# lyclyc52/SANeRF-HQ

Hardware: AMD Instinct MI355X
Metric: rays/s full render (800x800, hashgrid L=16 + 2x64 MLP) (higher is better)
Workload: dtype f32 arithmetic / f16 tables

## Files before the change

include/sanerf_hip.h:

```cpp
#ifndef SANERF_HIP_H
#define SANERF_HIP_H

#include <stddef.h>
#include <stdint.h>

#ifdef __cplusplus
extern "C" {
#endif

#define SN_MAX_LEVELS 32
#define SN_MAX_LAYERS 8
#define SN_MAX_STAGES 4
#define SN_ABI_VERSION 12

typedef void *sn_stream_t;

typedef enum {
    SN_OK = 0,
    SN_ERR_INVALID = -1,
    SN_ERR_UNSUPPORTED = -2,
    SN_ERR_HIP = -3,
    SN_ERR_WORKSPACE = -4,
    SN_ERR_WINDOW = -5
} sn_status;
// ... 111 lines not shown

int sn_rm_mask_eval_accumulate(const float *logits, const int64_t *labels, uint32_t N, uint32_t K, uint32_t C, float eps, sn_eval_record *record,
                               void *workspace, sn_stream_t stream);

int sn_rm_image_sqerr_accumulate(const float *pred, uint32_t pred_stride, const float *truth, uint32_t truth_stride, uint32_t N,
                                 sn_eval_record *record, void *workspace, sn_stream_t stream);

typedef struct sn_ssim_record {
    double ssim_sum;
    double last;
    uint64_t images;
} sn_ssim_record;

#define SN_SSIM_WORKSPACE_BYTES 8192

int sn_rm_image_ssim_accumulate(const float *pred, uint32_t pred_stride, const float *truth, uint32_t truth_stride, uint32_t H, uint32_t W,
                                float data_range , sn_ssim_record *record, void *workspace, sn_stream_t stream);

#define SN_DISTILL_WORKSPACE_FIXED_BYTES 8256
size_t sn_rm_feature_distill_workspace_bytes(uint32_t h, uint32_t w, uint32_t C, uint32_t Ho, uint32_t Wo);
int sn_rm_feature_distill_loss(const float *feat, uint32_t feat_stride, uint32_t h, uint32_t w, uint32_t C, const float *target, uint32_t Ho,
                               uint32_t Wo, float scale, const float *scale_dev, float *loss, float *grad_feat, float *resized, void *workspace,
                               size_t workspace_bytes, sn_stream_t stream);
int sn_rm_feature_map(const float *feat, uint32_t feat_stride, uint32_t h, uint32_t w, uint32_t C, uint32_t Ho, uint32_t Wo, float *out,
                      sn_stream_t stream);

typedef struct sn_rgb_loss_record { float total, mse, entropy, reserved; } sn_rgb_loss_record;
#define SN_RGB_LOSS_MAX_WORKGROUPS 512
#define SN_RGB_LOSS_WORKSPACE_BYTES 8256
int sn_rm_rgb_loss(const float *image, uint32_t image_stride, const float *weights_sum, const float *truth, uint32_t truth_stride,
                   uint32_t truth_channels, uint32_t N, float bg_value, const float *bg, uint32_t bg_rows, int image_has_bg,
                   float lambda_entropy, const float *extra0, float coef0, const float *extra1, float coef1, float *pred_rgb, float *gt_rgb,
                   sn_rgb_loss_record *record, float *grad_image, float *grad_weights_sum, void *workspace, sn_stream_t stream);

#define SN_PROMPT_MAX_POINTS 1024

int sn_rm_points_lift(const int32_t *pixels, uint32_t M, const float *rays_o, const float *rays_d, const float *depth, uint32_t depth_stride,
                      uint32_t H, uint32_t W, float *point_3d, sn_stream_t stream);

int sn_rm_point_store_update(float *xyz, int32_t *labels, int32_t *crucial, int32_t *count, uint32_t cap, const float *point, const int32_t *label,
                             float dist_thresh, int32_t *status, sn_stream_t stream);

int sn_rm_points_project(const float *points, const int32_t *labels, const int32_t *crucial, uint32_t N, const int32_t *n_points, const float *poses,
                         uint32_t V, const float *intrinsics, uint32_t n_intr, const float *depth, uint32_t depth_stride, uint32_t H, uint32_t W,
                         float depth_tol, int32_t crucial_count, int32_t valid_threshold, double resize_ratio ,
                         int32_t *coords, int32_t *labels_out, int32_t *kept_index, int32_t *sam_coords, int32_t *overlay_coords, float *cam,
                         float *uv, int32_t *state, int32_t *counts, sn_stream_t stream);

int sn_rm_prompt_overlay(const float *image, uint32_t image_stride, uint32_t H, uint32_t W, const uint8_t *masks, uint32_t M, const float *scores,
                         int32_t mask_index, const int32_t *coords, const int32_t *labels, uint32_t N, const int32_t *count, int32_t radius, double alpha,
                         float *rgb, uint8_t *rgb8, uint8_t *pred_mask, int32_t *selected, sn_stream_t stream);

#define SN_DRAW_MAX_CELLS 65536

int sn_rm_weighted_draw(const float *weights, const float *expo, uint32_t R, uint32_t C, uint32_t n, const float *row_u, const int64_t *row_index,
                        uint32_t M, int64_t *out, int32_t *status, sn_stream_t stream);

enum { SN_COLLATE_UNIFORM = 0, SN_COLLATE_ERROR_MAP = 1 };
typedef struct sn_collate_desc {
    const float   *poses, *intrinsics;
    const uint8_t *images;
    const void    *masks;
    const float   *error_map, *cam_near_far;
    uint32_t       M, n_intrinsics, H, W, image_channels, mask_channels, mask_elem_bytes, S, coarse_size;
    uint32_t       N;
    int32_t        mode, index;
    const int64_t *index_dev;
    const float   *u;
    const int64_t *cells;
    uint32_t       L, p;
    const float   *ul;
    const int64_t *centres;
    float         *rays_o, *rays_d;
    int64_t       *index_out, *i_out, *j_out, *inds_coarse;
    float         *images_out;
    void          *masks_out;
    float         *error_maps_out, *cam_near_far_out, *poses_out, *intrinsics_out;
    uint32_t       rays_o_stride, rays_d_stride, index_stride, i_stride, j_stride, inds_coarse_stride, images_stride, masks_stride,
                   error_maps_stride, cam_near_far_stride, poses_stride, intrinsics_stride;
} sn_collate_desc;
int sn_rm_collate_gather(const sn_collate_desc *desc, sn_stream_t stream);

int sn_rm_sample_positions(const float *rays_o, const float *rays_d, const float *nears, const float *fars, const float *bins,
                           uint32_t N, uint32_t T, int contract, float *real_bins, float *rays_t, float *xyzs, sn_stream_t stream);

int sn_rm_sample_positions_ex(const float *rays_o, const float *rays_d, const float *nears, const float *fars, const float *bins,
                              uint32_t N, uint32_t T, int contract, float grid_bound, float *real_bins, float *rays_t, float *xyzs,
                              sn_stream_t stream);

int sn_rm_jitter(const float *uniform, uint32_t N, uint32_t T, int kind, float *out, sn_stream_t stream);

int sn_rm_jitter_tables(uint64_t *state, uint32_t N, uint32_t ray_base, uint32_t num_stages, const uint32_t *num_steps, float *bins0,
                        float *const *u, int32_t advance, sn_stream_t stream);

int sn_rm_ray_composite(const float *weights, const float *rays_t, const float *raw, const float *rays_d, uint32_t N, uint32_t T,
                        float *weights_sum, float *depth, float *f_image, sn_stream_t stream);
int sn_rm_ray_composite_backward(const float *weights, const float *rays_t, const float *raw, const float *rays_d, const float *grad_weights_sum,
                                 const float *grad_depth, const float *grad_f_image, uint32_t N, uint32_t T, float *grad_weights, float *grad_raw,
                                 sn_stream_t stream);

int sn_rm_proposal_loss_scaled(const float *bins, const float *weights, const float *ref_bins, const float *ref_weights, uint32_t N, uint32_t T,
                               uint32_t Tr, float scale, const float *scale_dev, float *loss_per_ray, float *grad_weights, sn_stream_t stream);

size_t sn_rm_proposal_loss_workspace_bytes(uint32_t N, uint32_t T, uint32_t Tr, int backward);
int sn_rm_proposal_loss_long(const float *bins, const float *weights, const float *ref_bins, const float *ref_weights, uint32_t N, uint32_t T,
                             uint32_t Tr, float scale, const float *scale_dev, float *loss_per_ray, float *grad_weights, void *workspace,
                             size_t workspace_bytes, sn_stream_t stream);

int sn_zero(void *ptr, size_t bytes, sn_stream_t stream);

int sn_rm_composite(const float *weights, const float *values, uint32_t N, uint32_t T, uint32_t K,
                    float *out, sn_stream_t stream);
int sn_rm_composite_backward(const float *weights, const float *grad_out, uint32_t N, uint32_t T, uint32_t K,
                             float *grad_values, sn_stream_t stream);

typedef struct sn_grid_desc {
    const void *embeddings;
    int32_t     table_dtype;
    int32_t     offsets[SN_MAX_LEVELS + 1];
    uint32_t    D, C, L;
    float       S;
    uint32_t    H;
    uint32_t    gridtype, align_corners, interp;
} sn_grid_desc;

typedef struct sn_mlp_desc {
    const float *weight[SN_MAX_LAYERS];
    const float *bias[SN_MAX_LAYERS];
    uint32_t     dims[SN_MAX_LAYERS + 1];
    uint32_t     num_layers;
    uint32_t     activation;
    uint32_t     skip_mask;
} sn_mlp_desc;

enum { SN_MLP_AUTO = 0, SN_MLP_F16X3 = 1, SN_MLP_MFMA32 = 2, SN_MLP_VALU = 3, SN_MLP_F16X1 = 5 };
enum { SN_EXP_NONE = 0, SN_EXP_ROLE_SPLIT = 1, SN_EXP_LDS_LEVEL0 = 2, SN_EXP_FINAL_ONE_WG = 3,
       SN_EXP_MATRIX_CLUMPED = 4,
       SN_EXP_GATHER_CANONICAL = 5    };
typedef struct sn_render_tuning {
    int32_t mlp_mode;
    int32_t per_sample_form;
    int32_t densify;
    int32_t linear_tile_order;
    int32_t prop_sp_max_rays;
    int32_t final_sp_max_rays;
    int32_t feat_levels;
    int32_t band_streams;
    int32_t exact_early_out;
    int32_t wave_tile;
    int32_t prop_sp_lanes;
    int32_t feat_patch;
    int32_t prop_pair;
    int32_t experiment;
} sn_render_tuning;

typedef struct sn_render_cfg {
    uint32_t     num_stages;
    uint32_t     num_steps[SN_MAX_STAGES];
    sn_grid_desc prop_grid[SN_MAX_STAGES];
    sn_mlp_desc  prop_mlp[SN_MAX_STAGES];
    sn_grid_desc grid;
    sn_mlp_desc  grid_mlp;
    sn_mlp_desc  view_mlp;
    uint32_t     sh_degree;
    float        aabb[6];
    float        min_near;
    float        bound;
    int32_t      contract;
    int32_t      last_sample_opaque;
    float        bg_color;
    sn_grid_desc feat_grid;
    int32_t      with_feat;
    float        early_stop_eps;
    int32_t      mlp_exact_fp32;
    int32_t      compact_live;
    sn_render_tuning tuning;
} sn_render_cfg;

typedef struct sn_render_io {
    const float *rays_o, *rays_d;
    const float *cam_near_far;
    uint32_t     N;
    uint32_t     tile_w;
    const float *bins0_table;
    const float *u_table[SN_MAX_STAGES];
    uint32_t     bins0_ray_stride;
    uint32_t     u_ray_stride[SN_MAX_STAGES];
    int32_t      skip_final;
    float       *image;
    float       *depth;
    float       *weights_sum;
    uint32_t     out_stride;
    float       *bins[SN_MAX_STAGES];
    float       *weights[SN_MAX_STAGES];
    float       *sigmas[SN_MAX_STAGES];
    int32_t     *inds[SN_MAX_STAGES];
    float       *xyzs_last;
    float       *geo_feat_last;
    float       *f_image;
    float       *f_feat;
    uint32_t     head_stride;
    int32_t      pack_valid;
    void        *workspace;
    size_t       workspace_bytes;
} sn_render_io;

#define SN_PACK_VALID 0x50414b31

size_t sn_rm_render_workspace_bytes(const sn_render_cfg *cfg, uint32_t N, uint32_t tile_w);
int sn_rm_render_rays(const sn_render_cfg *cfg, const sn_render_io *io, sn_stream_t stream);
typedef struct sn_launch_info {
    char     final_kernel[64];
    uint32_t workgroups, lds_bytes, dense_levels, gathers_per_wave_sample, launches;
} sn_launch_info;
int sn_rm_last_launch_info(sn_launch_info *info);
int sn_rm_render_route_info(const sn_render_cfg *cfg, const sn_render_io *io, sn_launch_info *out);

typedef struct sn_tile_order_info {
    uint32_t workgroups, tile_id, tile_w, tile_h;
    int32_t  x[4], y[4];
} sn_tile_order_info;
int sn_rm_tile_order_info(uint32_t W, uint32_t rows, int32_t wave_tile, int32_t order, uint32_t workgroup, sn_tile_order_info *out);

int sn_rm_grid_composite(const float *xyzs, const float *weights, uint32_t N, uint32_t T, float bound,
                         const sn_grid_desc *grid, uint32_t tile_w, float *out, sn_stream_t stream);

size_t sn_mlp_wide_workspace_bytes(const sn_mlp_desc *mlp);
int sn_mlp_wide_overflow(int32_t *flag);
int sn_mlp_wide_forward(const sn_mlp_desc *mlp, const float *ln_weight, const float *ln_bias, float ln_eps,
                        const float *x, uint32_t N, float *out, void *workspace, size_t workspace_bytes,
                        sn_stream_t stream);

size_t sn_rm_mask_head_workspace_bytes(const sn_mlp_desc *mlp);
int sn_rm_mask_head(const float *xyzs, const float *extra, const float *weights, uint32_t N, uint32_t T, uint32_t E,
                    float bound, const sn_grid_desc *grid, const sn_mlp_desc *mlp, float *out,
                    void *workspace, size_t workspace_bytes, sn_stream_t stream);

int sn_rm_mask_point_labels(const float *xyzs, const float *extra, const float *live, uint32_t N, uint32_t T, uint32_t E,
                            float bound, const sn_grid_desc *grid, const sn_mlp_desc *mlp, uint8_t *labels, float *logits,
                            void *workspace, size_t workspace_bytes, sn_stream_t stream);
int sn_rm_object_composite(const uint8_t *labels, const float *sigmas, const float *real_bins, const float *geo_feat, const float *rays_d,
                           uint32_t N, uint32_t T, uint32_t keep_mask, int32_t invert, int32_t last_sample_opaque, float *weights_sum,
                           float *depth, float *f_image, float *weights, sn_stream_t stream);

int sn_rm_vertex_probe_points(const float *vertices, const float *normals, uint32_t V_total, uint32_t first, uint32_t count, uint32_t K,
                              float h, int32_t contract, float *xyz, float *dirs, sn_stream_t stream);
int sn_rm_vertex_probe_composite(const uint8_t *labels, const float *sigmas, const float *geo_feat, const float *dirs, uint32_t V, uint32_t K,
                                 float h, uint32_t keep_mask, int32_t invert, float *f, float *coverage, uint8_t *vertex_label,
                                 sn_stream_t stream);

int sn_rm_lattice_points(const float *origin, const float *step, uint32_t nx, uint32_t ny, uint32_t nz, uint32_t first, uint32_t count,
                         int32_t contract, float *xyz, sn_stream_t stream);
size_t sn_rm_isosurface_workspace_bytes(uint32_t nx, uint32_t ny, uint32_t nz);
int sn_rm_isosurface_count(const float *volume, uint32_t nx, uint32_t ny, uint32_t nz, float iso, void *workspace, size_t workspace_bytes,
                           uint32_t *counts, sn_stream_t stream);
int sn_rm_isosurface_emit(const float *volume, uint32_t nx, uint32_t ny, uint32_t nz, float iso, const float *origin, const float *step,
                          const void *workspace, size_t workspace_bytes, float *vertices, float *normals, int32_t *triangles,
                          uint32_t cap_v, uint32_t cap_t, sn_stream_t stream);

size_t sn_rm_mesh_clean_workspace_bytes(uint32_t V, uint32_t T);
int sn_rm_mesh_components_init(uint32_t V, int32_t *labels, sn_stream_t stream);
int sn_rm_mesh_components_sweep(const int32_t *triangles, uint32_t T, uint32_t V, int32_t *labels, uint32_t rounds, uint32_t *changed,
                                sn_stream_t stream);
int sn_rm_mesh_component_stats(const int32_t *triangles, uint32_t T, uint32_t V, const int32_t *labels, int32_t *triangle_counts,
                               int32_t *vertex_counts, uint32_t *counts, sn_stream_t stream);
int sn_rm_mesh_filter_count(const int32_t *triangles, uint32_t T, uint32_t V, const int32_t *labels, const int32_t *triangle_counts,
                            uint32_t min_triangles, const uint64_t *min_key, void *workspace, size_t workspace_bytes, uint32_t *counts,
                            sn_stream_t stream);
int sn_rm_mesh_filter_emit(const int32_t *triangles, uint32_t T, uint32_t V, const float *vertices, const float *normals,
                           const void *workspace, size_t workspace_bytes, float *out_vertices, float *out_normals, int32_t *out_triangles,
                           int32_t *source_vertex, uint32_t cap_v, uint32_t cap_t, sn_stream_t stream);

#define SN_MESH_SPLIT_PARTS 33
size_t sn_rm_mesh_split_workspace_bytes(uint32_t V, uint32_t T);
int sn_rm_mesh_split_count(const int32_t *triangles, uint32_t T, uint32_t V, const uint8_t *vertex_labels, void *workspace,
                           size_t workspace_bytes, int32_t *part_triangle_offsets, int32_t *part_vertex_offsets, uint32_t *counts,
                           sn_stream_t stream);
int sn_rm_mesh_split_emit(const int32_t *triangles, uint32_t T, uint32_t V, const float *vertices, const float *normals, void *workspace,
                          size_t workspace_bytes, float *out_vertices, float *out_normals, int32_t *out_triangles, int32_t *source_vertex,
                          int32_t *source_triangle, uint32_t cap_v, uint32_t cap_t, sn_stream_t stream);

size_t sn_rm_mesh_simplify_workspace_bytes(uint32_t V, uint32_t T, uint32_t cells);
int sn_rm_mesh_simplify_count(const float *vertices, const float *normals, const int32_t *triangles, uint32_t V, uint32_t T,
                              const float *origin, const float *cell, const uint32_t *dims, void *workspace, size_t workspace_bytes,
                              uint32_t *counts, sn_stream_t stream);
int sn_rm_mesh_simplify_emit(const float *vertices, const float *normals, const int32_t *triangles, uint32_t V, uint32_t T,
                             const float *origin, const float *cell, const uint32_t *dims, const void *workspace, size_t workspace_bytes,
                             float *out_vertices, float *out_normals, int32_t *out_triangles, int32_t *vertex_cluster, uint32_t cap_v,
                             uint32_t cap_t, sn_stream_t stream);

size_t sn_rm_mesh_smooth_workspace_bytes(uint32_t V, uint32_t T);
int sn_rm_mesh_smooth_build(const float *vertices, const int32_t *triangles, uint32_t V, uint32_t T, const float *origin, float quantum,
                            void *workspace, size_t workspace_bytes, sn_stream_t stream);
int sn_rm_mesh_smooth_steps(uint32_t V, uint32_t T, uint32_t iterations, float lambda, float mu, int pin_open, void *workspace,
                            size_t workspace_bytes, sn_stream_t stream);
int sn_rm_mesh_smooth_emit(const float *vertices, uint32_t V, uint32_t T, const float *origin, float quantum, const void *workspace,
                           size_t workspace_bytes, float *out_vertices, float *out_normals, uint8_t *vertex_flags, sn_stream_t stream);

size_t sn_rm_mesh_raster_workspace_bytes(uint32_t V, uint32_t T, uint32_t H, uint32_t W);
int sn_rm_mesh_raster_project(const float *vertices, uint32_t V, uint32_t T, const float *pose, const float *intrinsics, uint32_t H, uint32_t W,
                              float near_plane, void *workspace, size_t workspace_bytes, int32_t *counts, sn_stream_t stream);
int sn_rm_mesh_raster_draw(const int32_t *triangles, uint32_t V, uint32_t T, uint32_t H, uint32_t W, int cull, uint32_t small_max_pixels,
                           void *workspace, size_t workspace_bytes, int32_t *counts, sn_stream_t stream);
int sn_rm_mesh_raster_resolve(const int32_t *triangles, uint32_t V, uint32_t T, uint32_t H, uint32_t W, const float *colors,
                              const float *normals, const uint8_t *labels, float bg_color, const void *workspace, size_t workspace_bytes,
                              int32_t *triangle_id, float *depth, uint8_t *mask, float *image, float *normal, uint8_t *label,
                              sn_stream_t stream);
int sn_rm_mesh_raster_draw_clip(const float *vertices, const int32_t *triangles, uint32_t V, uint32_t T, const float *pose, const float *intrinsics,
                                uint32_t H, uint32_t W, float near_plane, int cull, uint32_t small_max_pixels, void *workspace,
                                size_t workspace_bytes, int32_t *counts, int32_t *clip_counts, sn_stream_t stream);
int sn_rm_mesh_raster_resolve_clip(const float *vertices, const int32_t *triangles, uint32_t V, uint32_t T, const float *pose,
                                   const float *intrinsics, uint32_t H, uint32_t W, float near_plane, const float *colors, const float *normals,
                                   const uint8_t *labels, float bg_color, const void *workspace, size_t workspace_bytes, int32_t *triangle_id,
                                   float *depth, uint8_t *mask, float *image, float *normal, uint8_t *label, sn_stream_t stream);

int sn_mlp_wide_forward_train(const sn_mlp_desc *mlp, const float *x, uint32_t N, float *const *hidden, float *out, sn_stream_t stream);

int sn_mlp_wide_forward_train_f16x3(const sn_mlp_desc *mlp, const float *x, uint32_t N, float *const *hidden, uint32_t *const *sign_bits,
                                    float *out, void *workspace, size_t workspace_bytes, sn_stream_t stream);

size_t sn_mlp_wide_backward_workspace_bytes(const sn_mlp_desc *mlp);
int sn_mlp_wide_backward_bits(const sn_mlp_desc *mlp, const float *grad_out, const uint32_t *const *sign_bits, uint32_t N,
                              float *grad_in, float *const *grad_hidden, void *workspace, size_t workspace_bytes, sn_stream_t stream);
int sn_mlp_wide_backward(const sn_mlp_desc *mlp, const float *grad_out, const float *const *hidden, uint32_t N,
                         float *grad_in, float *const *grad_hidden, void *workspace, size_t workspace_bytes, sn_stream_t stream);

enum { SN_SMALL_ACT_NONE = 0, SN_SMALL_ACT_TRUNC_EXP0 = 1, SN_SMALL_ACT_SIGMOID_BG = 2 };
int sn_mlp_small_supported(const sn_mlp_desc *mlp);
int sn_mlp_small_forward_train(const sn_mlp_desc *mlp, const float *x, uint32_t N, float *const *hidden, float *out, int32_t act,
                               const float *aux_in, float bg, float *aux_out, sn_stream_t stream);
int sn_mlp_small_backward(const sn_mlp_desc *mlp, const float *grad_out, const float *grad_aux, int32_t act, const float *out_raw, float bg,
                          const float *const *hidden, uint32_t N, float *grad_in, float *const *grad_hidden, float *grad_last, float *grad_aux_in,
                          sn_stream_t stream);

int sn_gemm_f32(const float *a, int64_t a_row, int64_t a_col, const float *b, int64_t b_row, int64_t b_col, const float *bias, int32_t act,
                uint32_t M, uint32_t N, uint32_t K, float *c, int64_t c_row, sn_stream_t stream);

size_t sn_linear_wgrad_workspace_bytes(uint32_t M, uint32_t K, uint32_t N);
int sn_linear_wgrad(const float *x, const float *dy, uint32_t M, uint32_t K, uint32_t N, float *dw,
                    void *workspace, size_t workspace_bytes, sn_stream_t stream);

#define SN_ADAM_ZERO_GRAD 1
#define SN_ADAM_LAZY 2
int sn_adam_step(float *param, float *grad, float *exp_avg, float *exp_avg_sq, uint64_t n, double lr, double beta1, double beta2,
                 double eps, double weight_decay, uint32_t step, const float *step_device, int maximize, int flags, sn_stream_t stream);

#define SN_ADAM_MULTI_MAX_TENSORS 32
#define SN_ADAM_MULTI_MAX_GROUPS 8
typedef struct sn_adam_tensor {
    float *param, *grad, *exp_avg, *exp_avg_sq;
    uint64_t n;
    float *step_device;
    uint32_t step;
    uint32_t group;
} sn_adam_tensor;
typedef struct sn_adam_group {
    double lr, beta1, beta2, eps, weight_decay;
    int32_t maximize;
    int32_t flags;
} sn_adam_group;
int sn_adam_step_multi(const sn_adam_tensor *tensors, uint32_t n_tensors, const sn_adam_group *groups, uint32_t n_groups,
                       const float *lr_scale_device, uint32_t *ticket, sn_stream_t stream);

#define SN_EMA_MULTI_MAX_TENSORS 32
#define SN_EMA_ADVANCE 1
typedef struct sn_ema_tensor {
    float *shadow;
    const float *param;
    uint64_t n;
// ... 15 lines not shown
```

sanerf-hq_amd/_lib.py:

```python
from __future__ import annotations

import ctypes as C
import os
import subprocess
from typing import Optional

import torch

_PKG = os.path.dirname(os.path.abspath(__file__))
LIB_PATH = os.environ.get("SN_LIB") or os.path.join(_PKG, "libsanerf_hip.so")
CSRC = os.path.join(_PKG, "csrc")

MAX_LEVELS, MAX_LAYERS, MAX_STAGES = 32, 8, 4
SN_F32, SN_F16 = 0, 1
LAYOUT_LBC, LAYOUT_BLC = 0, 1


class GridDesc(C.Structure):
    _fields_ = [("embeddings", C.c_void_p), ("table_dtype", C.c_int32), ("offsets", C.c_int32 * (MAX_LEVELS + 1)),
                ("D", C.c_uint32), ("C", C.c_uint32), ("L", C.c_uint32), ("S", C.c_float), ("H", C.c_uint32),
                ("gridtype", C.c_uint32), ("align_corners", C.c_uint32), ("interp", C.c_uint32)]


class MlpDesc(C.Structure):
    _fields_ = [("weight", C.c_void_p * MAX_LAYERS), ("bias", C.c_void_p * MAX_LAYERS),
                ("dims", C.c_uint32 * (MAX_LAYERS + 1)), ("num_layers", C.c_uint32),
                ("activation", C.c_uint32), ("skip_mask", C.c_uint32)]


MLP_AUTO, MLP_F16X3, MLP_MFMA32, MLP_VALU, MLP_F16X1 = 0, 1, 2, 3, 5
EXP_NONE, EXP_ROLE_SPLIT, EXP_LDS_LEVEL0, EXP_FINAL_ONE_WG, EXP_MATRIX_CLUMPED, EXP_GATHER_CANONICAL = 0, 1, 2, 3, 4, 5
BUILD_EXPERIMENTS, BUILD_POISON_LDS = 1, 2
ADAM_ZERO_GRAD, ADAM_LAZY = 1, 2
ADAM_MULTI_MAX_TENSORS, ADAM_MULTI_MAX_GROUPS = 32, 8
EMA_MULTI_MAX_TENSORS, EMA_ADVANCE = 32, 1
MASK_MAX_CLASSES, MASK_EVAL_WORKSPACE_BYTES = 32, 8192
MASK_OUT_MODES = {"none": 0, "heatmap": 1, "composition": 2, "mask": 3}
SSIM_WORKSPACE_BYTES, SSIM_MAX_STRIDE, SSIM_WINDOW = 8192, 64, 11
DISTILL_WORKSPACE_FIXED_BYTES = 8256
RGB_LOSS_WORKSPACE_BYTES, RGB_LOSS_MAX_WORKGROUPS = 8256, 512
PROMPT_MAX_POINTS = 1024
DRAW_MAX_CELLS = 65536
COLLATE_UNIFORM, COLLATE_ERROR_MAP = 0, 1


class AdamTensor(C.Structure):
    _fields_ = [("param", C.c_void_p), ("grad", C.c_void_p), ("exp_avg", C.c_void_p), ("exp_avg_sq", C.c_void_p), ("n", C.c_uint64),
                ("step_device", C.c_void_p), ("step", C.c_uint32), ("group", C.c_uint32)]


class AdamGroup(C.Structure):
    _fields_ = [("lr", C.c_double), ("beta1", C.c_double), ("beta2", C.c_double), ("eps", C.c_double), ("weight_decay", C.c_double),
                ("maximize", C.c_int32), ("flags", C.c_int32)]


class EmaTensor(C.Structure):
    _fields_ = [("shadow", C.c_void_p), ("param", C.c_void_p), ("n", C.c_uint64)]


class EvalRecord(C.Structure):
    _fields_ = [("nll_mean_sum", C.c_double), ("miou_sum", C.c_double), ("mse_sum", C.c_double), ("psnr_sum", C.c_double),
                ("images", C.c_uint64), ("rgb_images", C.c_uint64), ("inter", C.c_uint64 * MASK_MAX_CLASSES),
                ("pred", C.c_uint64 * MASK_MAX_CLASSES), ("truth", C.c_uint64 * MASK_MAX_CLASSES)]


class SsimRecord(C.Structure):
    _fields_ = [("ssim_sum", C.c_double), ("last", C.c_double), ("images", C.c_uint64)]


class CollateDesc(C.Structure):
    _fields_ = ([(n, C.c_void_p) for n in ("poses", "intrinsics", "images", "masks", "error_map", "cam_near_far")]
                + [(n, C.c_uint32) for n in ("M", "n_intrinsics", "H", "W", "image_channels", "mask_channels", "mask_elem_bytes", "S", "coarse_size", "N")]
                + [("mode", C.c_int32), ("index", C.c_int32), ("index_dev", C.c_void_p), ("u", C.c_void_p), ("cells", C.c_void_p),
                   ("L", C.c_uint32), ("p", C.c_uint32), ("ul", C.c_void_p), ("centres", C.c_void_p)]
                + [(n, C.c_void_p) for n in ("rays_o", "rays_d", "index_out", "i_out", "j_out", "inds_coarse", "images_out", "masks_out",
                                             "error_maps_out", "cam_near_far_out", "poses_out", "intrinsics_out")]
                + [(n + "_stride", C.c_uint32) for n in ("rays_o", "rays_d", "index", "i", "j", "inds_coarse", "images", "masks", "error_maps",
                                                         "cam_near_far", "poses", "intrinsics")])


class RenderTuning(C.Structure):
    _fields_ = [("mlp_mode", C.c_int32), ("per_sample_form", C.c_int32), ("densify", C.c_int32), ("linear_tile_order", C.c_int32),
                ("prop_sp_max_rays", C.c_int32), ("final_sp_max_rays", C.c_int32), ("feat_levels", C.c_int32), ("band_streams", C.c_int32), ("exact_early_out", C.c_int32), ("wave_tile", C.c_int32), ("prop_sp_lanes", C.c_int32), ("feat_patch", C.c_int32), ("prop_pair", C.c_int32), ("experiment", C.c_int32)]


class LaunchInfo(C.Structure):
    _fields_ = [("final_kernel", C.c_char * 64), ("workgroups", C.c_uint32), ("lds_bytes", C.c_uint32), ("dense_levels", C.c_uint32),
                ("gathers_per_wave_sample", C.c_uint32), ("launches", C.c_uint32)]


class TileOrderInfo(C.Structure):
    _fields_ = [("workgroups", C.c_uint32), ("tile_id", C.c_uint32), ("tile_w", C.c_uint32), ("tile_h", C.c_uint32),
                ("x", C.c_int32 * 4), ("y", C.c_int32 * 4)]


PACK_VALID = 0x50414B31


class RenderCfg(C.Structure):
    _fields_ = [("num_stages", C.c_uint32), ("num_steps", C.c_uint32 * MAX_STAGES),
                ("prop_grid", GridDesc * MAX_STAGES), ("prop_mlp", MlpDesc * MAX_STAGES),
                ("grid", GridDesc), ("grid_mlp", MlpDesc), ("view_mlp", MlpDesc),
                ("sh_degree", C.c_uint32), ("aabb", C.c_float * 6), ("min_near", C.c_float), ("bound", C.c_float),
                ("contract", C.c_int32), ("last_sample_opaque", C.c_int32), ("bg_color", C.c_float),
                ("feat_grid", GridDesc), ("with_feat", C.c_int32), ("early_stop_eps", C.c_float), ("mlp_exact_fp32", C.c_int32),
                ("compact_live", C.c_int32), ("tuning", RenderTuning)]


class RenderIO(C.Structure):
    _fields_ = [("rays_o", C.c_void_p), ("rays_d", C.c_void_p), ("cam_near_far", C.c_void_p),
                ("N", C.c_uint32), ("tile_w", C.c_uint32),
                ("bins0_table", C.c_void_p), ("u_table", C.c_void_p * MAX_STAGES),
                ("bins0_ray_stride", C.c_uint32), ("u_ray_stride", C.c_uint32 * MAX_STAGES), ("skip_final", C.c_int32),
                ("image", C.c_void_p), ("depth", C.c_void_p), ("weights_sum", C.c_void_p), ("out_stride", C.c_uint32),
                ("bins", C.c_void_p * MAX_STAGES), ("weights", C.c_void_p * MAX_STAGES),
                ("sigmas", C.c_void_p * MAX_STAGES), ("inds", C.c_void_p * MAX_STAGES),
                ("xyzs_last", C.c_void_p), ("geo_feat_last", C.c_void_p), ("f_image", C.c_void_p), ("f_feat", C.c_void_p), ("head_stride", C.c_uint32), ("pack_valid", C.c_int32),
                ("workspace", C.c_void_p), ("workspace_bytes", C.c_size_t)]


_u32, _f32, _i32, _vp, _int = C.c_uint32, C.c_float, C.c_int32, C.c_void_p, C.c_int
ABI_VERSION = 12

_SIGNATURES = {
    "sn_abi_version": (_int, []),
    "sn_build_flags": (_int, []),
    "sn_debug_set": (_int, [C.c_char_p, _int]),
    "sn_last_error": (C.c_char_p, []),
    "sn_device_count": (_int, []),
    "sn_grid_encode_forward": (_int, [_vp, _vp, _int, _vp, _vp, _u32, _u32, _u32, _u32, _u32, _f32, _u32, _vp, _u32, _int, _u32, _int, _vp]),
    "sn_grid_encode_forward_cat": (_int, [_vp, _vp, _int, _vp, _vp, _u32, _vp, _u32, _u32, _u32, _f32, _u32, _u32, _int, _u32, _vp]),
    "sn_grid_encode_backward": (_int, [_vp, _vp, _vp, _int, _vp, _vp, _u32, _u32, _u32, _u32, _u32, _f32, _u32, _vp, _vp, _u32, _int, _u32, _int, _vp]),
    "sn_grid_backward_binned_workspace_bytes": (C.c_size_t, [_u32, _u32, _u32, _u32, _u32, _vp]),
    "sn_grid_encode_backward_binned": (_int, [_vp, _vp, _vp, _vp, _u32, _u32, _u32, _u32, _u32, _f32, _u32, _u32, _int, _u32, _int, _vp, C.c_size_t, _vp]),
    "sn_grid_encode_backward_binned_rows": (_int, [_vp, _u32, _vp, _vp, _vp, _u32, _u32, _u32, _u32, _u32, _f32, _u32, _u32, _int, _u32, _int, _vp, C.c_size_t, _vp]),
    "sn_grad_total_variation": (_int, [_vp, _vp, _vp, _vp, _f32, _u32, _u32, _u32, _u32, _f32, _u32, _u32, _int, _vp]),
    "sn_grad_weight_decay": (_int, [_vp, _vp, _vp, _f32, _u32, _u32, _u32, _vp]),
    "sn_sh_encode_forward": (_int, [_vp, _vp, _u32, _u32, _u32, _vp, _vp]),
    "sn_sh_encode_backward": (_int, [_vp, _vp, _u32, _u32, _u32, _vp, _vp, _vp]),
    "sn_freq_encode_forward": (_int, [_vp, _u32, _u32, _u32, _u32, _vp, _vp]),
    "sn_freq_encode_backward": (_int, [_vp, _vp, _u32, _u32, _u32, _u32, _vp, _vp]),
    "sn_rm_generate_rays": (_int, [_vp, _f32, _f32, _f32, _f32, _u32, _u32, _u32, _u32, _vp, _vp, _vp]),
    "sn_rm_rays_from_pixels": (_int, [_vp, _u32, _vp, _u32, _vp, _u32, _u32, _vp, _vp, _vp]),
    "sn_rm_near_far_from_aabb": (_int, [_vp, _vp, _vp, _f32, _u32, _vp, _vp, _vp]),
    "sn_rm_contract": (_int, [_vp, _u32, _vp, _vp]),
    "sn_rm_sample_pdf": (_int, [_vp, _vp, _u32, _u32, _u32, _vp, _u32, _vp, _vp, _vp]),
    "sn_rm_weights_from_sigma": (_int, [_vp, _vp, _u32, _u32, _int, _vp, _vp]),
    "sn_rm_weights_from_sigma_backward": (_int, [_vp, _vp, _vp, _u32, _u32, _int, _vp, _vp]),
    "sn_rm_distort_loss": (_int, [_vp, _vp, _u32, _u32, _vp, _vp, _vp]),
    "sn_rm_proposal_loss": (_int, [_vp, _vp, _vp, _vp, _u32, _u32, _u32, _vp, _vp, _vp]),
    "sn_rm_sample_positions": (_int, [_vp, _vp, _vp, _vp, _vp, _u32, _u32, _int, _vp, _vp, _vp, _vp]),
    "sn_rm_sample_positions_ex": (_int, [_vp, _vp, _vp, _vp, _vp, _u32, _u32, _int, _f32, _vp, _vp, _vp, _vp]),
    "sn_rm_jitter": (_int, [_vp, _u32, _u32, _int, _vp, _vp]),
    "sn_rm_jitter_tables": (_int, [_vp, _u32, _u32, _u32, C.POINTER(_u32), _vp, C.POINTER(_vp), _i32, _vp]),
    "sn_rm_ray_composite": (_int, [_vp, _vp, _vp, _vp, _u32, _u32, _vp, _vp, _vp, _vp]),
    "sn_rm_ray_composite_backward": (_int, [_vp, _vp, _vp, _vp, _vp, _vp, _vp, _u32, _u32, _vp, _vp, _vp]),
    "sn_rm_proposal_loss_scaled": (_int, [_vp, _vp, _vp, _vp, _u32, _u32, _u32, _f32, _vp, _vp, _vp, _vp]),
    "sn_gemm_f32": (_int, [_vp, C.c_int64, C.c_int64, _vp, C.c_int64, C.c_int64, _vp, C.c_int32, _u32, _u32, _u32, _vp, C.c_int64, _vp]),
    "sn_rm_proposal_loss_workspace_bytes": (C.c_size_t, [_u32, _u32, _u32, _int]),
    "sn_rm_proposal_loss_long": (_int, [_vp, _vp, _vp, _vp, _u32, _u32, _u32, _f32, _vp, _vp, _vp, _vp, C.c_size_t, _vp]),
    "sn_zero": (_int, [_vp, C.c_size_t, _vp]),
    "sn_mlp_small_supported": (_int, [C.POINTER(MlpDesc)]),
    "sn_mlp_small_forward_train": (_int, [C.POINTER(MlpDesc), _vp, _u32, _vp, _vp, _i32, _vp, _f32, _vp, _vp]),
    "sn_mlp_small_backward": (_int, [C.POINTER(MlpDesc), _vp, _vp, _i32, _vp, _f32, _vp, _u32, _vp, _vp, _vp, _vp, _vp]),
    "sn_rm_composite": (_int, [_vp, _vp, _u32, _u32, _u32, _vp, _vp]),
    "sn_rm_composite_backward": (_int, [_vp, _vp, _u32, _u32, _u32, _vp, _vp]),
    "sn_rm_grid_composite": (_int, [_vp, _vp, _u32, _u32, _f32, C.POINTER(GridDesc), _u32, _vp, _vp]),
    "sn_mlp_wide_workspace_bytes": (C.c_size_t, [C.POINTER(MlpDesc)]),
    "sn_mlp_wide_forward": (_int, [C.POINTER(MlpDesc), _vp, _vp, _f32, _vp, _u32, _vp, _vp, C.c_size_t, _vp]),
    "sn_mlp_wide_overflow": (_int, [_vp]),
    "sn_mlp_wide_forward_train": (_int, [C.POINTER(MlpDesc), _vp, _u32, _vp, _vp, _vp]),
    "sn_mlp_wide_forward_train_f16x3": (_int, [C.POINTER(MlpDesc), _vp, _u32, _vp, _vp, _vp, _vp, C.c_size_t, _vp]),
    "sn_mlp_wide_backward_bits": (_int, [C.POINTER(MlpDesc), _vp, _vp, _u32, _vp, _vp, _vp, C.c_size_t, _vp]),
    "sn_mlp_wide_backward_workspace_bytes": (C.c_size_t, [C.POINTER(MlpDesc)]),
    "sn_mlp_wide_backward": (_int, [C.POINTER(MlpDesc), _vp, _vp, _u32, _vp, _vp, _vp, C.c_size_t, _vp]),
    "sn_rm_mask_head_workspace_bytes": (C.c_size_t, [C.POINTER(MlpDesc)]),
    "sn_rm_mask_head": (_int, [_vp, _vp, _vp, _u32, _u32, _u32, _f32, C.POINTER(GridDesc), C.POINTER(MlpDesc), _vp, _vp, C.c_size_t, _vp]),
    "sn_rm_mask_point_labels": (_int, [_vp, _vp, _vp, _u32, _u32, _u32, _f32, C.POINTER(GridDesc), C.POINTER(MlpDesc), _vp, _vp, _vp, C.c_size_t, _vp]),
    "sn_rm_object_composite": (_int, [_vp, _vp, _vp, _vp, _vp, _u32, _u32, _u32, _i32, _i32, _vp, _vp, _vp, _vp, _vp]),
    "sn_rm_vertex_probe_points": (_int, [_vp, _vp, _u32, _u32, _u32, _u32, _f32, _i32, _vp, _vp, _vp]),
    "sn_rm_vertex_probe_composite": (_int, [_vp, _vp, _vp, _vp, _u32, _u32, _f32, _u32, _i32, _vp, _vp, _vp, _vp]),
    "sn_rm_lattice_points": (_int, [C.POINTER(_f32), C.POINTER(_f32), _u32, _u32, _u32, _u32, _u32, _i32, _vp, _vp]),
    "sn_rm_isosurface_workspace_bytes": (C.c_size_t, [_u32, _u32, _u32]),
    "sn_rm_isosurface_count": (_int, [_vp, _u32, _u32, _u32, _f32, _vp, C.c_size_t, _vp, _vp]),
    "sn_rm_isosurface_emit": (_int, [_vp, _u32, _u32, _u32, _f32, C.POINTER(_f32), C.POINTER(_f32), _vp, C.c_size_t, _vp, _vp, _vp, _u32, _u32, _vp]),
    "sn_rm_mesh_clean_workspace_bytes": (C.c_size_t, [_u32, _u32]),
    "sn_rm_mesh_components_init": (_int, [_u32, _vp, _vp]),
    "sn_rm_mesh_components_sweep": (_int, [_vp, _u32, _u32, _vp, _u32, _vp, _vp]),
    "sn_rm_mesh_component_stats": (_int, [_vp, _u32, _u32, _vp, _vp, _vp, _vp, _vp]),
    "sn_rm_mesh_filter_count": (_int, [_vp, _u32, _u32, _vp, _vp, _u32, _vp, _vp, C.c_size_t, _vp, _vp]),
    "sn_rm_mesh_filter_emit": (_int, [_vp, _u32, _u32, _vp, _vp, _vp, C.c_size_t, _vp, _vp, _vp, _vp, _u32, _u32, _vp]),
    "sn_rm_mesh_split_workspace_bytes": (C.c_size_t, [_u32, _u32]),
    "sn_rm_mesh_split_count": (_int, [_vp, _u32, _u32, _vp, _vp, C.c_size_t, _vp, _vp, _vp, _vp]),
    "sn_rm_mesh_split_emit": (_int, [_vp, _u32, _u32, _vp, _vp, _vp, C.c_size_t, _vp, _vp, _vp, _vp, _vp, _u32, _u32, _vp]),
    "sn_rm_mesh_simplify_workspace_bytes": (C.c_size_t, [_u32, _u32, _u32]),
    "sn_rm_mesh_simplify_count": (_int, [_vp, _vp, _vp, _u32, _u32, _vp, _vp, _vp, _vp, C.c_size_t, _vp, _vp]),
    "sn_rm_mesh_simplify_emit": (_int, [_vp, _vp, _vp, _u32, _u32, _vp, _vp, _vp, _vp, C.c_size_t, _vp, _vp, _vp, _vp, _u32, _u32, _vp]),
    "sn_rm_mesh_smooth_workspace_bytes": (C.c_size_t, [_u32, _u32]),
    "sn_rm_mesh_smooth_build": (_int, [_vp, _vp, _u32, _u32, C.POINTER(_f32), _f32, _vp, C.c_size_t, _vp]),
    "sn_rm_mesh_smooth_steps": (_int, [_u32, _u32, _u32, _f32, _f32, _i32, _vp, C.c_size_t, _vp]),
    "sn_rm_mesh_smooth_emit": (_int, [_vp, _u32, _u32, C.POINTER(_f32), _f32, _vp, C.c_size_t, _vp, _vp, _vp, _vp]),
    "sn_rm_mesh_raster_workspace_bytes": (C.c_size_t, [_u32, _u32, _u32, _u32]),
    "sn_rm_mesh_raster_project": (_int, [_vp, _u32, _u32, _vp, _vp, _u32, _u32, _f32, _vp, C.c_size_t, _vp, _vp]),
    "sn_rm_mesh_raster_draw": (_int, [_vp, _u32, _u32, _u32, _u32, _i32, _u32, _vp, C.c_size_t, _vp, _vp]),
    "sn_rm_mesh_raster_resolve": (_int, [_vp, _u32, _u32, _u32, _u32, _vp, _vp, _vp, _f32, _vp, C.c_size_t, _vp, _vp, _vp, _vp, _vp, _vp, _vp]),
    "sn_rm_mesh_raster_draw_clip": (_int, [_vp, _vp, _u32, _u32, _vp, _vp, _u32, _u32, _f32, _i32, _u32, _vp, C.c_size_t, _vp, _vp, _vp]),
    "sn_rm_mesh_raster_resolve_clip": (_int, [_vp, _vp, _u32, _u32, _vp, _vp, _u32, _u32, _f32, _vp, _vp, _vp, _f32, _vp, C.c_size_t, _vp, _vp, _vp,
                                              _vp, _vp, _vp, _vp]),
    "sn_adam_step": (_int, [_vp, _vp, _vp, _vp, C.c_uint64, C.c_double, C.c_double, C.c_double, C.c_double, C.c_double, _u32, _vp, _int, _int, _vp]),
    "sn_adam_step_multi": (_int, [C.POINTER(AdamTensor), _u32, C.POINTER(AdamGroup), _u32, _vp, _vp, _vp]),
    "sn_ema_update_multi": (_int, [C.POINTER(EmaTensor), _u32, C.c_double, _vp, _vp, _int, _vp]),
    "sn_linear_wgrad_workspace_bytes": (C.c_size_t, [_u32, _u32, _u32]),
    "sn_linear_wgrad": (_int, [_vp, _vp, _u32, _u32, _u32, _vp, _vp, C.c_size_t, _vp]),
    "sn_rm_render_workspace_bytes": (C.c_size_t, [C.POINTER(RenderCfg), _u32, _u32]),
    "sn_rm_render_rays": (_int, [C.POINTER(RenderCfg), C.POINTER(RenderIO), _vp]),
    "sn_rm_profile_enable": (None, [_int]),
    "sn_rm_profile_read": (_int, [_vp, _vp, _int]),
    "sn_rm_profile_shader_clock": (_int, [_vp, _vp]),
    "sn_rm_mask_nll": (_int, [_vp, _vp, _u32, _u32, _f32, _vp, _vp, _vp]),
    "sn_rm_ray_pair_select": (_int, [_vp, _vp, _u32, _u32, _u32, _vp, _vp]),
    "sn_rm_ray_pair_rgb_loss": (_int, [_vp, _vp, _int, _vp, _u32, _u32, _u32, _u32, _f32, _f32, _f32, _int, _f32, _vp, _vp, _vp, _vp, _vp]),
    "sn_rm_mask_error": (_int, [_vp, _int, _vp, _u32, _u32, _f32, _f32, _vp, _vp]),
    "sn_rm_error_map_update": (_int, [_vp, _int, _vp, _vp, _u32, _vp, _u32, _u32, _f32, _f32, _u32, _u32, _vp, _vp, _vp, _vp]),
    "sn_rm_mask_output": (_int, [_vp, _u32, _u32, _vp, _u32, _vp, _u32, _int, _int, _f32, _vp, _vp, _vp, _vp, _vp, _vp, _vp]),
    "sn_rm_mask_eval_accumulate": (_int, [_vp, _vp, _u32, _u32, _u32, _f32, _vp, _vp, _vp]),
    "sn_rm_image_sqerr_accumulate": (_int, [_vp, _u32, _vp, _u32, _u32, _vp, _vp, _vp]),
    "sn_rm_image_ssim_accumulate": (_int, [_vp, _u32, _vp, _u32, _u32, _u32, _f32, _vp, _vp, _vp]),
    "sn_rm_feature_distill_workspace_bytes": (C.c_size_t, [_u32, _u32, _u32, _u32, _u32]),
    "sn_rm_feature_distill_loss": (_int, [_vp, _u32, _u32, _u32, _u32, _vp, _u32, _u32, _f32, _vp, _vp, _vp, _vp, _vp, C.c_size_t, _vp]),
    "sn_rm_feature_map": (_int, [_vp, _u32, _u32, _u32, _u32, _u32, _u32, _vp, _vp]),
    "sn_rm_rgb_loss": (_int, [_vp, _u32, _vp, _vp, _u32, _u32, _u32, _f32, _vp, _u32, _int, _f32, _vp, _f32, _vp, _f32, _vp, _vp, _vp, _vp, _vp, _vp, _vp]),
    "sn_rm_points_lift": (_int, [_vp, _u32, _vp, _vp, _vp, _u32, _u32, _u32, _vp, _vp]),
    "sn_rm_point_store_update": (_int, [_vp, _vp, _vp, _vp, _u32, _vp, _vp, _f32, _vp, _vp]),
    "sn_rm_points_project": (_int, [_vp, _vp, _vp, _u32, _vp, _vp, _u32, _vp, _u32, _vp, _u32, _u32, _u32, _f32, _i32, _i32, C.c_double,
                                    _vp, _vp, _vp, _vp, _vp, _vp, _vp, _vp, _vp, _vp]),
    "sn_rm_prompt_overlay": (_int, [_vp, _u32, _u32, _u32, _vp, _u32, _vp, _i32, _vp, _vp, _u32, _vp, _i32, C.c_double, _vp, _vp, _vp, _vp, _vp]),
    "sn_rm_weighted_draw": (_int, [_vp, _vp, _u32, _u32, _u32, _vp, _vp, _u32, _vp, _vp, _vp]),
    "sn_rm_collate_gather": (_int, [C.POINTER(CollateDesc), _vp]),
    "sn_rm_debug_occupancy": (_int, [_vp, _vp, _int]),
    "sn_rm_last_launch_info": (_int, [_vp]),
    "sn_rm_render_route_info": (_int, [C.POINTER(RenderCfg), C.POINTER(RenderIO), _vp]),
    "sn_rm_tile_order_info": (_int, [_u32, _u32, _i32, _i32, _u32, C.POINTER(TileOrderInfo)]),
    "sn_debug_eval": (_int, [_int, _vp, _vp, _u32, _vp, _vp]),
}

EXPORTED_SYMBOLS = tuple(_SIGNATURES)

_lib = None


def build(force: bool = False) -> str:
    srcs = [os.path.join(CSRC, f) for f in os.listdir(CSRC) if f.endswith((".hip", ".h", ".inc"))]
    srcs.append(os.path.join(os.path.dirname(_PKG), "include", "sanerf_hip.h"))
    stale = force or not os.path.exists(LIB_PATH) or os.path.getmtime(LIB_PATH) < max(os.path.getmtime(s) for s in srcs)
    if stale:
        subprocess.check_call(["make", "-C", CSRC, "-j4"] + (["-B"] if force else []))
    return LIB_PATH


def lib():
    global _lib
    if _lib is None:
        if not os.path.exists(LIB_PATH):
            raise ImportError(
                f"{LIB_PATH} is missing: build it with `python -c 'import __graft_entry__ as g; g.build()'` "
                "(hipcc --offload-arch=gfx950). There is no CPU / eager fallback for these operators.")
        l = C.CDLL(LIB_PATH)
        for name, (res, args) in _SIGNATURES.items():
            try:
                fn = getattr(l, name)
            except AttributeError:
                if os.environ.get("SN_LIB"):
                    continue
                raise ImportError(f"{LIB_PATH} does not export {name}: rebuild it")
            fn.restype, fn.argtypes = res, args
        if l.sn_abi_version() != ABI_VERSION:
            raise ImportError(f"{LIB_PATH} has ABI version {l.sn_abi_version()}, this package expects {ABI_VERSION}: rebuild it")
        _lib = l
    return _lib


def check(rc: int, what: str = "") -> None:
    if rc != 0:
        msg = lib().sn_last_error().decode()
        raise RuntimeError(f"{what}: {msg}" if what else msg)


def stream() -> int:
    return torch.cuda.current_stream().cuda_stream


def dev(t: Optional[torch.Tensor], name: str, dtype=torch.float32):
    if t is None:
        return None
    if not t.is_cuda:
        raise RuntimeError(f"{name} must be a CUDA tensor")
    if not t.is_contiguous():
        raise RuntimeError(f"{name} must be a contiguous tensor")
    if dtype is not None and t.dtype != dtype:
        raise RuntimeError(f"{name} must be a {dtype} tensor, got {t.dtype}")
    return t.data_ptr()


def host_i32(values):
    arr = (C.c_int32 * len(values))(*[int(v) for v in values])
    return arr


def host_f32(values):
    return (C.c_float * len(values))(*[float(v) for v in values])
```

sanerf-hq_amd/csrc/render.hip:

```cpp
#include "sn_common.h"
#include "sh_basis.inc"

#include <float.h>
#include <stdlib.h>
#include <string.h>
#include <cstdio>
#include <map>
#include <mutex>
#include <type_traits>
#include <vector>

namespace sn {

typedef float floatx16 __attribute__((ext_vector_type(16)));

struct RayCommon {
    const float *rays_o, *rays_d, *cnf;
    uint32_t N;
    uint32_t W;
    uint32_t rows;
    uint32_t Npad;
    float aabb[6];
    float min_near, bound;
    int contract, last_opaque;
    float bg;
    int xcd_swizzle;
    uint32_t st_w, st_h;
    uint32_t tlw;
    float inv_den;
};

__host__ __device__ __forceinline__ uint32_t xcd_tile_id(uint32_t b, uint32_t nwg) {
    const uint32_t xcd = b & 7u, q = nwg >> 3, r = nwg & 7u;
    return (xcd < r ? xcd * (q + 1u) : r * (q + 1u) + (xcd - r) * q) + (b >> 3);
}
__device__ __forceinline__ uint32_t tile_id_x(const RayCommon &rc, uint32_t b, uint32_t nwg) { return rc.xcd_swizzle ? xcd_tile_id(b, nwg) : b; }
__device__ __forceinline__ uint32_t tile_id(const RayCommon &rc) { return tile_id_x(rc, blockIdx.x, gridDim.x); }

__host__ __device__ __forceinline__ void wave_tile_of(uint32_t g, uint32_t tx8, uint32_t ty8, uint32_t sw, uint32_t sh, uint32_t &wx, uint32_t &wy) {
    const uint32_t P = ty8 >> 1, pair = 2u * tx8, paired = P * pair;
    if (g >= paired) { wx = g - paired; wy = ty8 & ~1u; return; }
    if (sw == 0u) { const uint32_t p = g / pair, i = g - p * pair; wx = i >> 1; wy = 2u * p + (i & 1u); return; }
    const uint32_t u = g >> 1;
    const uint32_t nsy = (P + sh - 1u) / sh, base = P / nsy, extra = P - base * nsy;
    const uint32_t big = (base + 1u) * tx8;
    uint32_t sy, r0, h, y0;
    if (u < extra * big) { sy = u / big; r0 = u - sy * big; h = base + 1u; y0 = sy * h; }
    else { const uint32_t v = u - extra * big, row = base * tx8, s = v / row; r0 = v - s * row; sy = extra + s; h = base; y0 = extra * (base + 1u) + s * base; }
    const uint32_t full = sw * h, sx = r0 / full, r1 = r0 - sx * full;
    const uint32_t left = tx8 - sx * sw, w = left < sw ? left : sw;
    const uint32_t ry = r1 / w, rx = r1 - ry * w;
    const uint32_t x = sx * sw + rx;
    wx = (sy & 1u) ? tx8 - 1u - x : x;
    wy = 2u * (y0 + ry) + (g & 1u);
}

__device__ __forceinline__ bool ray_of_lane(const RayCommon &rc, uint32_t wg, uint32_t &n) {
    const uint32_t tid = threadIdx.x;
    if (rc.W) {
        const uint32_t tlw = rc.tlw, tlh = 6u - tlw, tw = 1u << tlw, th = 1u << tlh;
        const uint32_t tx8 = (rc.W + tw - 1u) >> tlw, ty8 = (rc.rows + th - 1u) >> tlh;
        const uint32_t wave = __builtin_amdgcn_readfirstlane(tid >> 6), lane = tid & 63u;
        const uint32_t g = wg * 4u + wave;
        uint32_t wx, wy;
        wave_tile_of(g, tx8, ty8, rc.st_w, rc.st_h, wx, wy);
        const uint32_t py = (wy << tlh) + (lane >> tlw);
        const uint32_t px = (wx << tlw) + (lane & (tw - 1u));
        const bool ok = wx < tx8 && px < rc.W && py < rc.rows;
        n = ok ? py * rc.W + px : 0u;
        return ok;
    }
    n = wg * 256u + tid;
    const bool ok = n < rc.N;
    if (!ok) n = 0;
    return ok;
}

struct RaySetup {
    float o[3], d[3];
    float s_near, s_far;
};

__device__ __forceinline__ void setup_ray(const RayCommon &rc, uint32_t n, RaySetup &rs) {
#pragma unroll
    for (int k = 0; k < 3; ++k) { rs.o[k] = rc.rays_o[(size_t)n * 3 + k]; rs.d[k] = rc.rays_d[(size_t)n * 3 + k]; }
    float near, far;
    near_far_one(rs.o, rs.d, rc.aabb, rc.min_near, near, far);
    if (rc.cnf) {
        const float cn = rc.cnf[(size_t)n * 2], cf = rc.cnf[(size_t)n * 2 + 1];
        near = cn > near ? cn : near;
        far = cf < far ? cf : far;
    }
    rs.s_near = spacing_fn(near);
    rs.s_far = spacing_fn(far);
}

__device__ __forceinline__ float real_bin(const RaySetup &rs, float b) {
    const float a = rs.s_near * (1.0f - b);
    const float c = rs.s_far * b;
    return spacing_inv(a + c);
}

__device__ __forceinline__ void sample_x01(const RayCommon &rc, const RaySetup &rs, float tmid, float (&p)[3], float (&x01)[3]) {
#pragma unroll
    for (int k = 0; k < 3; ++k) { const float m = rs.d[k] * tmid; p[k] = rs.o[k] + m; }
    if (rc.contract) contract3(p[0], p[1], p[2]);
    const float den = 2.0f * rc.bound;
    if (rc.inv_den != 0.0f) {
#pragma unroll
        for (int k = 0; k < 3; ++k) x01[k] = (p[k] + rc.bound) * rc.inv_den;
    } else {
#pragma unroll
        for (int k = 0; k < 3; ++k) x01[k] = (p[k] + rc.bound) / den;
    }
}

template <int I, int N, typename F>
__device__ __forceinline__ void static_for(F &&f) {
    if constexpr (I < N) {
        f(std::integral_constant<int, I>{});
        static_for<I + 1, N>(f);
    }
}

template <typename T, int C>
struct Corner { float v[C]; };

template <typename T, int C>
__device__ __forceinline__ void corner_set_half2(Corner<T, C> &c, uint32_t bits) {
    static_assert(C == 2 && sizeof(T) == 2, "packed rows: fp16 tables with two features per level");
    c.v[0] = __uint_as_float(bits); c.v[1] = 0.0f;
}
__device__ __forceinline__ float fma_mix_lo(float w, uint32_t packed, float acc) {
    float d;
    asm("v_fma_mix_f32 %0, %1, %2, %3 op_sel_hi:[0,1,0]" : "=v"(d) : "v"(w), "v"(packed), "v"(acc));
    return d;
}
__device__ __forceinline__ float fma_mix_hi(float w, uint32_t packed, float acc) {
    float d;
    asm("v_fma_mix_f32 %0, %1, %2, %3 op_sel:[0,1,0] op_sel_hi:[0,1,0]" : "=v"(d) : "v"(w), "v"(packed), "v"(acc));
    return d;
}

#ifndef SN_PROP_GROUP
#define SN_PROP_GROUP 2
#endif
#ifndef SN_PROP_GROUP_H
#define SN_PROP_GROUP_H 2
#endif
template <typename T, int KIND, int l>
constexpr bool xswap_level() {
    return KIND == 1 && l >= 0;
}
#ifndef SN_XSWAP_MODE
#define SN_XSWAP_MODE 0
#endif
#ifndef SN_PARITY_FIRST
#define SN_PARITY_FIRST 12
#endif
#ifndef SN_PARITY_AXES
#define SN_PARITY_AXES 2
#endif
template <typename T, int AXIS, int l>
constexpr bool parity_level() {
    return l >= SN_PARITY_FIRST && (AXIS == 2 || (AXIS == 1 && SN_PARITY_AXES == 2));
}
__device__ __forceinline__ float parity_tag(float frac, uint32_t cell) {
    return __uint_as_float(__float_as_uint(frac) | (cell << 31));
}
__device__ __forceinline__ bool parity_of(float tagged) { return (__float_as_uint(tagged) >> 31) != 0u; }
#ifndef SN_PARITY_UNDO
#define SN_PARITY_UNDO 1
#endif
__device__ __forceinline__ void swap_if(bool odd, uint32_t &a, uint32_t &b) {
#if SN_PARITY_UNDO == 1
    const uint64_t m = __builtin_amdgcn_ballot_w64(odd);
    uint64_t sv;
    asm("s_and_saveexec_b64 %[sv], %[m]\n\tv_swap_b32 %[a], %[b]\n\ts_mov_b64 exec, %[sv]" : [a] "+v"(a), [b] "+v"(b), [sv] "=&s"(sv) : [m] "s"(m) : "scc");
#else
    const uint32_t t = a;
    a = odd ? b : a; b = odd ? t : b;
#endif
}
__device__ __forceinline__ void swap_if4(bool odd, uint32_t &a0, uint32_t &b0, uint32_t &a1, uint32_t &b1, uint32_t &a2, uint32_t &b2, uint32_t &a3, uint32_t &b3) {
#if SN_PARITY_UNDO == 1
    const uint64_t m = __builtin_amdgcn_ballot_w64(odd);
    uint64_t sv;
    asm("s_and_saveexec_b64 %[sv], %[m]\n\t"
        "v_swap_b32 %[a0], %[b0]\n\tv_swap_b32 %[a1], %[b1]\n\tv_swap_b32 %[a2], %[b2]\n\tv_swap_b32 %[a3], %[b3]\n\t"
        "s_mov_b64 exec, %[sv]"
        : [a0] "+v"(a0), [b0] "+v"(b0), [a1] "+v"(a1), [b1] "+v"(b1), [a2] "+v"(a2), [b2] "+v"(b2), [a3] "+v"(a3), [b3] "+v"(b3), [sv] "=&s"(sv)
        : [m] "s"(m)
        : "scc");
#else
    uint32_t t;
    t = a0; a0 = odd ? b0 : a0; b0 = odd ? t : b0;
    t = a1; a1 = odd ? b1 : a1; b1 = odd ? t : b1;
    t = a2; a2 = odd ? b2 : a2; b2 = odd ? t : b2;
    t = a3; a3 = odd ? b3 : a3; b3 = odd ? t : b3;
#endif
}

__device__ __forceinline__ void half_wave_swap(uint32_t &a, uint32_t &b) {
#if SN_XSWAP_MODE == 0
    auto r = __builtin_amdgcn_permlane32_swap(a, b, false, false);
    a = r[0]; b = r[1];
#elif SN_XSWAP_MODE == 1
    const uint32_t nb = (uint32_t)__builtin_amdgcn_update_dpp(0, (int)b, 0xB1, 0xF, 0xF, true);
    const uint32_t na = (uint32_t)__builtin_amdgcn_update_dpp(0, (int)a, 0xB1, 0xF, 0xF, true);
    const bool odd = (threadIdx.x & 1u) != 0u;
    a = odd ? nb : a; b = odd ? b : na;
#else
    auto r = __builtin_amdgcn_permlane16_swap(a, b, false, false);
    a = r[0]; b = r[1];
#endif
}

struct PairTab {
    const void *base;
    uint32_t off[8];
};

template <typename T, int C, int KIND, bool PAIRA, bool XSWAP = false>
__device__ __forceinline__ void issue_level(const T *__restrict__ table, const GridLevels &g, int l, const float (&x01)[3],
                                            float (&pos)[3], Corner<T, C> (&cv)[8], const PairTab *pt = nullptr) {
    const uint32_t res = g.res[l], size = g.size[l], mode = g.mode[l];
    const T *tab = table + (size_t)g.off[l] * C;
    uint32_t cell[3], offs[8];
// ... 1270 lines not shown
    return dot32_sum(s01, s23);
}

template <bool SW>
__device__ __forceinline__ void grid_mlp_mfma16_l12_spread(const uint4 *__restrict__ pk, const uint32_t *__restrict__ slab_hi,
                                                           const uint32_t *__restrict__ slab_lo, const float *__restrict__ w3,
                                                           float (&xh)[2][32], float (&part)[2]) {
    const uint32_t lane = threadIdx.x & 63u;
    const uint32_t lo = lane & 31u, hi = lane >> 5;
    const floatx16 zero16 = {0, 0, 0, 0, 0, 0, 0, 0, 0, 0, 0, 0, 0, 0, 0, 0};
    uint4 W[2][2];
    uint4 B[2][2];
    uint32_t bb[4][2][4];
    floatx16 h1[2], h2[2][2];
    float4 ww[2][8];
    f2v s01[2] = {{0.0f, 0.0f}, {0.0f, 0.0f}}, s23[2] = {{0.0f, 0.0f}, {0.0f, 0.0f}};
    const uint32_t oz1 = opaque_zero();
    const uint4 *const pkT[2] = {pk, pk + oz1};
    const float *const w3T[2] = {w3, w3 + oz1};
    auto rdW = [&](int S, int im) { W[S & 1][im] = pkT[S / 12][((S % 12) * 2 + im) * 64 + lane]; };
    auto rdB = [&](int t, int st, int im) {
        const uint32_t off = slab_dword<SW>((uint32_t)t * 32u + lo, 4u * hi + 8u * (uint32_t)st);
        B[st][im] = *reinterpret_cast<const uint4 *>((im ? slab_lo : slab_hi) + off);
    };
    auto rdw3 = [&](int t, int i4) { ww[t][i4] = *reinterpret_cast<const float4 *>(w3T[t] + 4 * i4); };
    auto S_ = [&](int q, int p) {
        const floatx16 &v = h1[q >> 1];
        const int i = 8 * (q & 1) + 2 * p;
        split2(relu_ieee(v[i]), relu_ieee(v[i + 1]), bb[q][0][p], bb[q][1][p]);
    };
    auto X_ = [&](int t, int i4) {
        const floatx16 &v = h2[t][i4 >> 2];
        const int r = 4 * (i4 & 3);
        float (&x)[32] = xh[t];
        x[4 * i4 + 0] = relu_ieee(v[r + 0]); x[4 * i4 + 1] = relu_ieee(v[r + 1]);
        x[4 * i4 + 2] = relu_ieee(v[r + 2]); x[4 * i4 + 3] = relu_ieee(v[r + 3]);
        dot32_step(ww[t][i4], x[4 * i4 + 0], x[4 * i4 + 1], x[4 * i4 + 2], x[4 * i4 + 3], s01[t], s23[t]);
    };
    rdW(0, 1); rdB(0, 0, 0); rdW(0, 0); rdB(0, 0, 1); rdB(0, 1, 0); rdB(0, 1, 1);
    __builtin_amdgcn_sched_barrier(0);
    static_for<0, 2>([&](auto tt) {
        constexpr int t = decltype(tt)::value;
        static_for<0, 36>([&](auto mm) {
            constexpr int m = decltype(mm)::value, s = m / 3, k = m % 3, S = 12 * t + s;
            uint4 bh, bl;
            if constexpr (s < 4) { bh = B[s & 1][0]; bl = B[s & 1][1]; }
            else {
                constexpr int q = s & 3;
                bh = uint4{bb[q][0][0], bb[q][0][1], bb[q][0][2], bb[q][0][3]};
                bl = uint4{bb[q][1][0], bb[q][1][1], bb[q][1][2], bb[q][1][3]};
            }
            floatx16 &acc = s < 4 ? h1[(s >> 1) & 1] : h2[t][s < 4 ? 0 : (s - 4) >> 2];
            if constexpr (k == 0 && (s == 0 || s == 2 || s == 4 || s == 8)) acc = zero16;
            const half8_t Ah = __builtin_bit_cast(half8_t, W[S & 1][0]), Al = __builtin_bit_cast(half8_t, W[S & 1][1]);
            const half8_t Bh = __builtin_bit_cast(half8_t, bh), Bl = __builtin_bit_cast(half8_t, bl);
            if constexpr (k == 0) acc = __builtin_amdgcn_mfma_f32_32x32x16_f16(Al, Bh, acc, 0, 0, 0);
            if constexpr (k == 1) acc = __builtin_amdgcn_mfma_f32_32x32x16_f16(Ah, Bl, acc, 0, 0, 0);
            if constexpr (k == 2) acc = __builtin_amdgcn_mfma_f32_32x32x16_f16(Ah, Bh, acc, 0, 0, 0);
            if constexpr (k == 0 && S + 1 < 24) rdW(S + 1, 1);
            if constexpr (k == 2 && S + 1 < 24) rdW(S + 1, 0);
            if constexpr (t == 1) {
                if constexpr (m == 0) { X_(0, 4); rdw3(0, 5); }
                if constexpr (m == 1) { rdw3(0, 6); rdw3(0, 7); }
                if constexpr (m == 3) X_(0, 5);
                if constexpr (m == 4) X_(0, 6);
                if constexpr (m == 5) { X_(0, 7); part[0] = dot32_sum(s01[0], s23[0]); }
            }
            if constexpr (m >= 6 && m < 14) S_((m - 6) >> 2, (m - 6) & 3);
            if constexpr (m == 14) S_(2, 0);
            if constexpr (m == 15) S_(2, 1);
            if constexpr (m == 16) { S_(2, 2); S_(2, 3); }
            if constexpr (m == 17) S_(3, 0);
            if constexpr (m == 18) S_(3, 1);
            if constexpr (m == 19) { S_(3, 2); S_(3, 3); }
            if constexpr (t == 0) {
                if constexpr (m == 30) rdB(1, 0, 0);
                if constexpr (m == 32) rdB(1, 0, 1);
                if constexpr (m == 33) rdB(1, 1, 0);
                if constexpr (m == 34) rdB(1, 1, 1);
            }
            if constexpr (m == 24) rdw3(t, 0);
            if constexpr (m == 26) rdw3(t, 1);
            if constexpr (m == 28) rdw3(t, 2);
            if constexpr (m == 30) rdw3(t, 3);
            if constexpr (m == 32) rdw3(t, 4);
            if constexpr (m == 26) X_(t, 0);
            if constexpr (m == 28) X_(t, 1);
            if constexpr (m == 30) X_(t, 2);
            if constexpr (m == 32) X_(t, 3);
            if constexpr (t == 1) {
                if constexpr (m == 33) rdw3(1, 5);
                if constexpr (m == 34) rdw3(1, 6);
                if constexpr (m == 35) rdw3(1, 7);
            }
            __builtin_amdgcn_sched_barrier(0);
        });
    });
    X_(1, 4); X_(1, 5); X_(1, 6); X_(1, 7);
    part[1] = dot32_sum(s01[1], s23[1]);
}

template <typename T, int L, int GROUP, int K>
__device__ __forceinline__ void encode_levels_split(const T *__restrict__ table, const GridLevels &g, const float (&x01)[3],
                                                    uint32_t *__restrict__ row_hi, uint32_t *__restrict__ row_lo) {
    const bool oob = encode_grouped<T, L, 2, GROUP, K, false>(table, g, x01, [&](int l, const float (&acc)[2]) {
        uint32_t ph, pl;
        split2(acc[0], acc[1], ph, pl);
        row_hi[l] = ph;
        row_lo[l] = pl;
    });
    if (__builtin_expect(__any(oob), 0)) {
        if (oob) for (int l = 0; l < L; ++l) { row_hi[l] = 0u; row_lo[l] = 0u; }
    }
}

template <int IN, int OUT, int ACT>
__device__ __forceinline__ void dense_lds(const float *__restrict__ W, const float *__restrict__ xin, float *__restrict__ yout, uint32_t stride) {
    float x[IN];
#pragma unroll
    for (int k = 0; k < IN; ++k) x[k] = xin[k * stride];
#pragma unroll 1
    for (int o = 0; o < OUT; ++o) {
        float acc = 0.0f;
#pragma unroll
        for (int k = 0; k < IN; ++k) acc = __builtin_fmaf(W[o * IN + k], x[k], acc);
        if (ACT == 1) acc = relu_ieee(acc);
        yout[o * stride] = acc;
    }
}

template <typename T, int L, int C, int GROUP, int K, bool PAIRX = false>
__device__ __forceinline__ void encode_levels_lds(const T *__restrict__ table, const GridLevels &g, const float (&x01)[3],
                                                  float *__restrict__ fe, uint32_t stride) {
    const bool oob = encode_grouped<T, L, C, GROUP, K, PAIRX>(table, g, x01, [&](int l, const float (&acc)[C]) {
#pragma unroll
        for (int c = 0; c < C; ++c) fe[(l * C + c) * stride] = acc[c];
    });
    if (__builtin_expect(__any(oob), 0)) {
        if (oob) for (int i = 0; i < L * C; ++i) fe[i * stride] = 0.0f;
    }
}

enum { MLP_VALU = 0, MLP_F32 = 1, MLP_F16X3 = 2 };
#ifndef SN_RS_SPANS_H
#define SN_RS_SPANS_H 6
#endif
#ifndef SN_FINAL_WAVES
#ifndef SN_FINAL_SP_MIN_BLOCKS
#define SN_FINAL_SP_MIN_BLOCKS 256u
#endif
#define SN_FINAL_WAVES 2
#endif

template <typename TT, int L, int C, int H1, int H2, int NOUT, int VH, int MODE, int K, bool AUX = false, bool LT = false, bool L0L = false, bool EO = false, int NP = 3, bool PORD = false,
          bool CANON = false>
__global__ __launch_bounds__(256, MODE == MLP_VALU ? 1 : SN_FINAL_WAVES) void k_final_stage(FinalArgs a) {
    SN_POISON_ALL();
    static_assert(NP == 3 || (LT && !L0L && !AUX), "reduced-product MLP forms: plain linear-tail instantiations only");
    static_assert(!LT || (MODE == MLP_F16X3 && K >= 4 && K <= 8), "linear tail: split-fp16 MLP on the FinalLv path");
    static_assert(!L0L || (LT && sizeof(TT) == 2), "LDS-resident level 0: fp16 tables, linear-tail instantiation (80 KiB: 32 packed weights + 4 x 8 swizzled slabs + 16 level 0)");
    constexpr int SLAB_DW = L0L ? 16 : SLAB_STRIDE;
    constexpr bool MFMA = MODE != MLP_VALU;
    constexpr int IN = L * C;
    constexpr int GEO = NOUT - 1;
    constexpr int NSH = 16;
    constexpr int NCOL = GEO + NSH;
    static_assert(!MFMA || (IN == 32 && H1 == 64 && H2 == 64 && NOUT == 16), "MFMA path is the 32-64-64-16 MLP");
    extern __shared__ __attribute__((aligned(16))) float lds[];
    float *fe;
    uint32_t fstride;
    float *actB = nullptr;
    constexpr int VW0 = VH * PadIn<NCOL>::value, VW1 = VH * PadIn<VH>::value;
    float *lds_vw;
    uint32_t *slab_hi = nullptr, *slab_lo = nullptr;
    if constexpr (MODE == MLP_F16X3) {
        static_assert(PACK16_U4 * 4 == PACK_FLOATS, "both packings fill the same 32 KiB");
        for (uint32_t i = threadIdx.x; i < (uint32_t)PACK16_U4; i += 256u)
            reinterpret_cast<uint4 *>(lds)[i] = reinterpret_cast<const uint4 *>(a.mlp_pack)[i];
        if constexpr (LT) { __syncthreads(); stage_w3p(lds + W3P_OFFSET, a.w[2]); }
        constexpr int WAVE_SLAB = 2 * 64 * SLAB_DW;
        float *wave_base = lds + PACK_FLOATS + (threadIdx.x >> 6) * WAVE_SLAB;
        slab_hi = reinterpret_cast<uint32_t *>(wave_base);
        slab_lo = slab_hi + 64 * SLAB_DW;
        if constexpr (L0L) {
            uint32_t *l0w = reinterpret_cast<uint32_t *>(lds + PACK_FLOATS + 4 * WAVE_SLAB);
            const uint32_t rows0 = a.g.res[0] * a.g.res[0] * a.g.res[0];
            const uint32_t *src = reinterpret_cast<const uint32_t *>(a.table) + a.g.off[0];
            for (uint32_t i = threadIdx.x; i < rows0; i += 256u) l0w[i] = src[i];
        }
        fe = wave_base + (threadIdx.x & 63u);
        fstride = 64u;
        lds_vw = lds;
    } else if constexpr (MODE == MLP_F32) {
        for (uint32_t i = threadIdx.x; i < (uint32_t)PACK_FLOATS / 4u; i += 256u)
            reinterpret_cast<float4 *>(lds)[i] = reinterpret_cast<const float4 *>(a.mlp_pack)[i];
        fe = lds + PACK_FLOATS + (threadIdx.x >> 6) * (IN * 64) + (threadIdx.x & 63u);
        fstride = 64u;
        lds_vw = lds;
    } else {
        fe = lds + threadIdx.x;
        actB = lds + 64 * 256 + threadIdx.x;
        fstride = 256u;
        lds_vw = lds + 2 * 64 * 256;
    }
    if constexpr (!MFMA) {
        stage_weights<NCOL, VH>(lds_vw, a.vw[0]);
        stage_weights<VH, VH>(lds_vw + VW0, a.vw[1]);
        stage_weights<VH, 3>(lds_vw + VW0 + VW1, a.vw[2]);
    }
    __syncthreads();
    clock_probe(0);
    const uint32_t *l0tab = reinterpret_cast<const uint32_t *>(lds + PACK_FLOATS + 4 * 2 * 64 * SLAB_DW);

    uint32_t n;
    const uint32_t wg = tile_id(a.rc);
    const bool ok = ray_of_lane(a.rc, wg, n);
    const uint32_t r = wg * 256u + threadIdx.x;
    const uint32_t Npad = a.rc.Npad;
    RaySetup rs;
    setup_ray(a.rc, n, rs);
    const uint32_t T = a.T;
    const float b0step = 1.0f / (float)T;
    auto bin_at = [&](uint32_t j) -> float {
        if (a.bins_in) return a.bins_in[(size_t)j * Npad + r];
        if (a.bins0_tab) return a.bins0_tab[(size_t)n * a.bins0_stride + j];
        return linspace_at(0.0f, 1.0f, b0step, T + 1u, j);
    };

    float dirn[3] = {rs.d[0], rs.d[1], rs.d[2]};
#pragma unroll
    for (int pass = 0; pass < 2; ++pass) {
        const float aa = dirn[0] * dirn[0], bb = dirn[1] * dirn[1], cc = dirn[2] * dirn[2];
        const float nrm = sqrtf((aa + bb) + cc);
        dirn[0] = dirn[0] / nrm; dirn[1] = dirn[1] / nrm; dirn[2] = dirn[2] / nrm;
    }

    float fimg[NCOL];
#pragma unroll
    for (int c = 0; c < NCOL; ++c) fimg[c] = 0.0f;
    float dep = 0.0f;
    double cum = 0.0, wsum = 0.0;
    float tr_seen = 1.0f;
    uint32_t j_stop = a.T;
    const bool per_sample_export = a.dbg_bins || a.dbg_w || a.dbg_sigma || a.dbg_xyz || a.dbg_geo;
    const TT *table = reinterpret_cast<const TT *>(a.table);
    float hacc[LT ? 2 : 1][LT ? 32 : 1];
    if constexpr (LT) {
#pragma unroll
        for (int t = 0; t < 2; ++t)
#pragma unroll
            for (int i = 0; i < 32; ++i) hacc[t][i] = 0.0f;
    }
    const float *w3p = lds + W3P_OFFSET + (threadIdx.x & 32u) * 16u;

    float bprev = bin_at(0);
    float rb_prev = real_bin(rs, bprev);
    if (ok && a.dbg_bins) a.dbg_bins[(size_t)n * (T + 1)] = bprev;
    constexpr int PG = 4;
    constexpr bool LV = MODE == MLP_F16X3 && K >= PG && K <= 8;
    using SP = FinalSpans<LV ? (LT ? (sizeof(TT) == 2 ? SN_FINAL_SPANS_LT_H : SN_FINAL_SPANS_LT) : 0) : 0>;
    constexpr int G0 = LV ? SP::B[1] : PG;
    static_assert(!LV || (L == 16 && SP::B[SP::N] == L && G0 <= K), "spans cover the 16 levels; span 0 is dense");
    GroupRegs<TT, 2, G0> g0;
    float bnext_n = bin_at(1);
    float rb_next_n = real_bin(rs, bnext_n);
    float tmid_n = (rb_next_n + rb_prev) / 2.0f;
    float p_n[3], x01_n[3];
    sample_x01(a.rc, rs, tmid_n, p_n, x01_n);
    bool fast_n = false;
    if constexpr (LV) {
        fast_n = all_interior(a.lv, x01_n);
        if constexpr (L0L) {
            issue_level0_lds<0>(a.lv, l0tab, x01_n, g0.pos[0], g0.cv[0]);
            static_for<1, G0>([&](auto kk) { constexpr int k = decltype(kk)::value; issue_level_lv<TT, true, false, false, k>(a.lv, x01_n, g0.pos[k], g0.cv[k]); });
        } else issue_span_lv<TT, 0, G0, K, false>(a.lv, x01_n, g0);
        __builtin_amdgcn_sched_barrier(0);
    } else if constexpr (MODE == MLP_F16X3) {
        issue_group<TT, 2, PG, K, 0>(table, a.g, x01_n, g0, a.pairs);
        __builtin_amdgcn_sched_barrier(0);
    }
    for (uint32_t j = 0; j < T; ++j) {
        const float bnext = bnext_n;
        const float rb_next = rb_next_n;
        const float tmid = tmid_n;
        float p[3] = {p_n[0], p_n[1], p_n[2]}, x01[3] = {x01_n[0], x01_n[1], x01_n[2]};
        float h[NOUT];
        if constexpr (MODE == MLP_F16X3) {
            const uint32_t lane = threadIdx.x & 63u;
            uint32_t *row_hi = slab_hi + lane * SLAB_STRIDE, *row_lo = slab_lo + lane * SLAB_STRIDE;
            auto emit = [&](int l, const float (&acc)[2]) {
                if constexpr (NP < 3) { row_hi[l] = pack_h2(acc[0], acc[1]); return; }
                uint32_t ph, pl;
                split2(acc[0], acc[1], ph, pl);
                if constexpr (L0L) { const uint32_t o = slab_dword<true>(lane, (uint32_t)l); slab_hi[o] = ph; slab_lo[o] = pl; }
                else { row_hi[l] = ph; row_lo[l] = pl; }
            };
            if constexpr (LV) blend_span<TT, 0, G0, K>(g0, emit);
            else blend_group<TT, 2, PG, K, 0>(g0, emit);
            __builtin_amdgcn_sched_barrier(0);
            auto zero_oob = [&]() {
                const bool oob = (x01[0] < 0.0f || x01[0] > 1.0f) || (x01[1] < 0.0f || x01[1] > 1.0f) || (x01[2] < 0.0f || x01[2] > 1.0f);
                if (__builtin_expect(__any(oob), 0)) {
                    if (oob) for (int l = 0; l < L; ++l) {
                        if constexpr (L0L) { const uint32_t o = slab_dword<true>(lane, (uint32_t)l); slab_hi[o] = 0u; slab_lo[o] = 0u; }
                        else { row_hi[l] = 0u; row_lo[l] = 0u; }
                    }
                }
            };
            if constexpr (LV) {
                auto rest = [&](auto fast_tag) {
                    constexpr bool FAST = decltype(fast_tag)::value;
                    static_for<1, SP::N>([&](auto gg) {
                        constexpr int SPAN = decltype(gg)::value, L0 = SP::B[SPAN], G = SP::B[SPAN + 1] - L0;
                        GroupRegs<TT, 2, G> gr;
                        issue_span_lv<TT, L0, G, K, FAST, !CANON>(a.lv, x01, gr);
                        __builtin_amdgcn_sched_barrier(0);
                        blend_span<TT, L0, G, K, !CANON>(gr, emit);
                        __builtin_amdgcn_sched_barrier(0);
                    });
                };
                if (__builtin_expect(fast_n, 1)) rest(std::true_type{});
                else { rest(std::false_type{}); zero_oob(); }
            } else {
                static_for<1, L / PG>([&](auto gg) {
                    constexpr int GRP = decltype(gg)::value;
                    GroupRegs<TT, 2, PG> gr;
                    issue_group<TT, 2, PG, K, GRP>(table, a.g, x01, gr, a.pairs);
                    __builtin_amdgcn_sched_barrier(0);
                    blend_group<TT, 2, PG, K, GRP>(gr, emit);
                    __builtin_amdgcn_sched_barrier(0);
                });
                zero_oob();
            }
            {
                const uint32_t jn = j + 2u <= T ? j + 2u : T;
                bnext_n = bin_at(jn);
                rb_next_n = real_bin(rs, bnext_n);
                const float rbp = j + 2u <= T ? rb_next : rb_prev;
                tmid_n = (rb_next_n + rbp) / 2.0f;
                sample_x01(a.rc, rs, tmid_n, p_n, x01_n);
                if constexpr (LV) {
                    fast_n = all_interior(a.lv, x01_n);
                    if constexpr (L0L) {
                        issue_level0_lds<0>(a.lv, l0tab, x01_n, g0.pos[0], g0.cv[0]);
                        static_for<1, G0>([&](auto kk) { constexpr int k = decltype(kk)::value; issue_level_lv<TT, true, false, false, k>(a.lv, x01_n, g0.pos[k], g0.cv[k]); });
                    } else issue_span_lv<TT, 0, G0, K, false>(a.lv, x01_n, g0);
                } else {
                    issue_group<TT, 2, PG, K, 0>(table, a.g, x01_n, g0, a.pairs);
                }
                __builtin_amdgcn_sched_barrier(0);
            }
            __builtin_amdgcn_wave_barrier();
            if constexpr (!LT) grid_mlp_mfma16(reinterpret_cast<const uint4 *>(lds) + opaque_zero(), slab_hi, slab_lo, h);
            __builtin_amdgcn_wave_barrier();
        } else if constexpr (MODE == MLP_F32) {
            encode_levels_lds<TT, L, C, 2, K>(table, a.g, x01, fe, fstride);
            __builtin_amdgcn_wave_barrier();
            grid_mlp_mfma(lds + opaque_zero(), fe - (threadIdx.x & 63u), h);
            __builtin_amdgcn_wave_barrier();
        } else {
            encode_levels_lds<TT, L, C, 2, K>(table, a.g, x01, fe, fstride);
            dense_lds<IN, H1, 1>(a.w[0], fe, actB, fstride);
            dense_lds<H1, H2, 1>(a.w[1], actB, fe, fstride);
            dense_lds<H2, NOUT, 0>(a.w[2], fe, actB, fstride);
#pragma unroll
            for (int k = 0; k < NOUT; ++k) h[k] = actB[k * fstride];
        }
        if constexpr (LT && (sizeof(TT) == 2 ? 0 : 0)) {
            const float delta = rb_next - rb_prev;
            const uint32_t oz = opaque_zero();
            const uint32_t my_half = (threadIdx.x >> 5) & 1u;
            static_for<0, 2>([&](auto tt) {
                constexpr int t = decltype(tt)::value;
                float x[32];
                grid_mlp_mfma16_l12<L0L>(reinterpret_cast<const uint4 *>(lds) + oz, slab_hi, slab_lo, t, x);
                const float part = dot32_lds(w3p + oz, x);
                auto pr = __builtin_amdgcn_permlane32_swap(__float_as_uint(part), __float_as_uint(part), false, false);
                const float h0 = __uint_as_float(pr[0]) + __uint_as_float(pr[1]);
                float wv = 0.0f;
                if (my_half == (uint32_t)t) {
                    const float sigma = expf_det(h0);
                    float ds = delta * sigma;
                    if (a.rc.last_opaque && j == T - 1u) ds = __builtin_inff();
                    const float alpha = 1.0f - expf_det(-ds);
                    const float tr = expf_det(-(float)cum);
                    tr_seen = tr;
                    float w = alpha * tr;
                    if (w != w) w = 0.0f;
                    cum += (double)ds;
                    wsum += (double)w;
                    dep = __builtin_fmaf(w, tmid, dep);
                    if constexpr (AUX) { if (a.w_out) a.w_out[(size_t)j * Npad + r] = w; }
                    wv = w;
                }
                auto ww = __builtin_amdgcn_permlane32_swap(__float_as_uint(wv), __float_as_uint(wv), false, false);
                const float wt = __uint_as_float(ww[t]);
#pragma unroll
                for (int i = 0; i < 32; i += 2) {
                    const f2v r = __builtin_elementwise_fma(f2v{wt, wt}, f2v{x[i], x[i + 1]}, f2v{hacc[t][i], hacc[t][i + 1]});
                    hacc[t][i] = r.x; hacc[t][i + 1] = r.y;
                }
                __builtin_amdgcn_sched_barrier(0);
            });
            if constexpr (AUX) { if (a.stop_cum > 0.0f && __all((float)cum > a.stop_cum)) break; }
            if constexpr (EO) { if (!per_sample_export && __all(tr_seen == 0.0f)) { j_stop = j + 1u; break; } }
            rb_prev = rb_next;
            continue;
        }
        float xh[LT ? 2 : 1][LT ? 32 : 1];
        if constexpr (LT) {
            const uint32_t oz = opaque_zero();
            float part[2];
            if constexpr (NP == 3 && !PORD) {
                grid_mlp_mfma16_l12_spread<L0L>(reinterpret_cast<const uint4 *>(lds) + oz, slab_hi, slab_lo, w3p + oz, xh, part);
            } else {
#pragma unroll
                for (int t = 0; t < 2; ++t) {
                    grid_mlp_mfma16_l12<L0L, NP>(reinterpret_cast<const uint4 *>(lds) + oz, slab_hi, slab_lo, t, xh[t]);
                    part[t] = dot32_lds(w3p + oz, xh[t]);
                }
            }
            __builtin_amdgcn_wave_barrier();
            auto pr = __builtin_amdgcn_permlane32_swap(__float_as_uint(part[0]), __float_as_uint(part[1]), false, false);
            h[0] = __uint_as_float(pr[0]) + __uint_as_float(pr[1]);
        }
        const float sigma = expf_det(h[0]);
        const float delta = rb_next - rb_prev;
        float ds = delta * sigma;
        if (a.rc.last_opaque && j == T - 1u) ds = __builtin_inff();
        const float alpha = 1.0f - expf_det(-ds);
        const float tr = expf_det(-(float)cum);
        tr_seen = tr;
        float w = alpha * tr;
        if (w != w) w = 0.0f;
        cum += (double)ds;
        wsum += (double)w;
        dep = __builtin_fmaf(w, tmid, dep);
        if constexpr (LT) {
            auto ww = __builtin_amdgcn_permlane32_swap(__float_as_uint(w), __float_as_uint(w), false, false);
            const float w0 = __uint_as_float(ww[0]), w1 = __uint_as_float(ww[1]);
#pragma unroll
            for (int i = 0; i < 32; i += 2) {
                const f2v r0 = __builtin_elementwise_fma(f2v{w0, w0}, f2v{xh[0][i], xh[0][i + 1]}, f2v{hacc[0][i], hacc[0][i + 1]});
                const f2v r1 = __builtin_elementwise_fma(f2v{w1, w1}, f2v{xh[1][i], xh[1][i + 1]}, f2v{hacc[1][i], hacc[1][i + 1]});
                hacc[0][i] = r0.x; hacc[0][i + 1] = r0.y; hacc[1][i] = r1.x; hacc[1][i + 1] = r1.y;
            }
        } else {
#pragma unroll
            for (int c = 0; c < GEO; ++c) fimg[c] = __builtin_fmaf(w, h[1 + c], fimg[c]);
        }
        if constexpr (AUX) { if (a.w_out) a.w_out[(size_t)j * Npad + r] = w; }
        if constexpr (!LT) if (ok) {
            if (a.dbg_bins) a.dbg_bins[(size_t)n * (T + 1) + j + 1] = bnext;
            if (a.dbg_sigma) a.dbg_sigma[(size_t)n * T + j] = sigma;
            if (a.dbg_w) a.dbg_w[(size_t)n * T + j] = w;
            if (a.dbg_xyz) { float *q = a.dbg_xyz + ((size_t)n * T + j) * 3; q[0] = p[0]; q[1] = p[1]; q[2] = p[2]; }
            if (a.dbg_geo) { float *q = a.dbg_geo + ((size_t)n * T + j) * GEO;
#pragma unroll
                for (int c = 0; c < GEO; ++c) q[c] = h[1 + c]; }
        }
        if constexpr (AUX) { if (a.stop_cum > 0.0f && __all((float)cum > a.stop_cum)) break; }
        if constexpr (EO) { if (!per_sample_export && __all(tr_seen == 0.0f)) { j_stop = j + 1u; break; } }
        rb_prev = rb_next;
        if constexpr (MODE != MLP_F16X3) {
            const uint32_t jn = j + 2u <= T ? j + 2u : T;
            bnext_n = bin_at(jn);
            rb_next_n = real_bin(rs, bnext_n);
            tmid_n = (rb_next_n + (j + 2u <= T ? rb_next : rb_prev)) / 2.0f;
            sample_x01(a.rc, rs, tmid_n, p_n, x01_n);
        }
    }

    clock_probe(1);
    if constexpr (AUX) {
        if (a.w_out) for (uint32_t jj = j_stop; jj < T; ++jj) a.w_out[(size_t)jj * Npad + r] = 0.0f;
    }
    if constexpr (LT) {
#pragma unroll 1
        for (int c = 0; c < GEO; ++c) {
            const float *wr = w3p + (1 + c) * 32;
            const float q0 = dot32_lds(wr, hacc[0]), q1 = dot32_lds(wr, hacc[1]);
            auto qq = __builtin_amdgcn_permlane32_swap(__float_as_uint(q0), __float_as_uint(q1), false, false);
            const float v = __uint_as_float(qq[0]) + __uint_as_float(qq[1]);
            switch (c) {
#define SN_FIMG_CASE(I) case I: fimg[I] = v; break;
                SN_FIMG_CASE(0) SN_FIMG_CASE(1) SN_FIMG_CASE(2) SN_FIMG_CASE(3) SN_FIMG_CASE(4) SN_FIMG_CASE(5) SN_FIMG_CASE(6) SN_FIMG_CASE(7)
                SN_FIMG_CASE(8) SN_FIMG_CASE(9) SN_FIMG_CASE(10) SN_FIMG_CASE(11) SN_FIMG_CASE(12) SN_FIMG_CASE(13) SN_FIMG_CASE(14)
#undef SN_FIMG_CASE
                default: break;
            }
        }
    }
    static_assert(VH <= IN && NCOL <= IN && IN * 64 <= 2 * 64 * SLAB_DW, "view MLP activations reuse the feature column / slab");
    if constexpr (MFMA) {
        __syncthreads();
        stage_weights<NCOL, VH>(lds_vw, a.vw[0]);
        stage_weights<VH, VH>(lds_vw + VW0, a.vw[1]);
        stage_weights<VH, 3>(lds_vw + VW0 + VW1, a.vw[2]);
        __syncthreads();
    }
    __builtin_amdgcn_wave_barrier();
    float rgb[3];
    const float ws = (float)wsum;
    {
        float sh[NSH];
        sh_degree4(dirn[0], dirn[1], dirn[2], sh);
#pragma unroll
        for (int c = 0; c < NSH; ++c) fimg[GEO + c] = sh[c] * ws;
    }
#pragma unroll
    for (int c = 0; c < NCOL; ++c) fe[c * fstride] = fimg[c];
    dense_ldsw_col<NCOL, VH, 1>(lds_vw, fe, fe, fstride);
    dense_ldsw_col<VH, VH, 1>(lds_vw + VW0, fe, fe, fstride);
    {
        float v2[VH];
#pragma unroll
        for (int k = 0; k < VH; ++k) v2[k] = fe[k * fstride];
        dense_ldsw<VH, 3, 0>(lds_vw + VW0 + VW1, v2, rgb);
    }
    if (ok) {
#pragma unroll
        for (int c = 0; c < 3; ++c) {
            const float sg = 1.0f / (1.0f + expf_det(-rgb[c]));
            const float bgm = (1.0f - ws) * a.rc.bg;
            a.image[(size_t)n * a.istride + c] = sg + bgm;
        }
        a.depth[(size_t)n * a.sstride] = dep;
        a.wsum[(size_t)n * a.sstride] = ws;
        if (a.dbg_fimg) {
#pragma unroll
            for (int c = 0; c < NCOL; ++c) a.dbg_fimg[(size_t)n * a.fimg_stride + c] = fimg[c];
        }
        if (a.head_rgbd) {
            float *q = a.head_rgbd + (size_t)n * a.fimg_stride;
#pragma unroll
            for (int c = 0; c < 3; ++c) q[c] = a.image[(size_t)n * a.istride + c];
            q[3] = dep;
        }
    }
}

struct AnyShape {
    uint32_t ng, nv;
    uint32_t dg[5], dv[5];
    const float *wg[4], *wv[4];
    uint32_t rows;
};
constexpr uint32_t ANY_W = 64, ANY_GEO = 31, ANY_LAYERS = 4;

template <int INB>
__device__ __forceinline__ void dense_any_b(const float *__restrict__ W, uint32_t in, uint32_t out, bool relu, const float *xin, float *yout) {
    float x[INB];
#pragma unroll
    for (int k = 0; k < INB; ++k) {
        const float t = xin[(uint32_t)k * 256u];
        x[k] = (uint32_t)k < in ? t : 0.0f;
    }
    for (uint32_t o0 = 0; o0 < out; o0 += 4u) {
        const float *w[4];
        float acc[4] = {0.0f, 0.0f, 0.0f, 0.0f};
#pragma unroll
        for (uint32_t q = 0; q < 4u; ++q) w[q] = W + (size_t)umin(o0 + q, out - 1u) * in;
#pragma unroll
        for (int g = 0; g < INB / 8; ++g) {
            if (8u * (uint32_t)g < in) {
                if (8u * (uint32_t)g + 8u <= in) {
#pragma unroll
                    for (int j = 0; j < 8; ++j)
#pragma unroll
                        for (uint32_t q = 0; q < 4u; ++q) acc[q] = __builtin_fmaf(w[q][8 * g + j], x[8 * g + j], acc[q]);
                } else {
#pragma unroll
                    for (int j = 0; j < 8; ++j) {
                        const uint32_t kk = 8u * (uint32_t)g + (uint32_t)j;
#pragma unroll
                        for (uint32_t q = 0; q < 4u; ++q) {
                            const float wk = w[q][kk < in ? kk : in - 1u];
                            acc[q] = __builtin_fmaf(kk < in ? wk : 0.0f, x[8 * g + j], acc[q]);
                        }
                    }
                }
            }
        }
#pragma unroll
        for (uint32_t q = 0; q < 4u; ++q) {
            if (o0 + q < out) yout[(o0 + q) * 256u] = relu ? relu_ieee(acc[q]) : acc[q];
        }
    }
}
__device__ __forceinline__ void dense_any(const float *__restrict__ W, uint32_t in, uint32_t out, bool relu, const float *xin, float *yout) {
    if (in <= 16u) dense_any_b<16>(W, in, out, relu, xin, yout);
    else if (in <= 32u) dense_any_b<32>(W, in, out, relu, xin, yout);
    else dense_any_b<64>(W, in, out, relu, xin, yout);
}

template <typename TT>
__global__ __launch_bounds__(256) void k_final_stage_any(FinalArgs a, AnyShape s) {
    SN_POISON_ALL();
    extern __shared__ __attribute__((aligned(16))) float lds[];
    const uint32_t rows = s.rows;
    float *bufA = lds + threadIdx.x, *bufB = lds + rows * 256u + threadIdx.x, *accf = lds + 2u * rows * 256u + threadIdx.x;
    uint32_t n;
    const uint32_t wg = tile_id(a.rc);
    const bool ok = ray_of_lane(a.rc, wg, n);
    const uint32_t r = wg * 256u + threadIdx.x;
    const uint32_t Npad = a.rc.Npad;
    RaySetup rs;
    setup_ray(a.rc, n, rs);
    const uint32_t T = a.T, L = a.g.L, GEO = s.dg[s.ng] - 1u, NCOL = GEO + 16u;
    const float b0step = 1.0f / (float)T;
    auto bin_at = [&](uint32_t j) -> float {
        if (a.bins_in) return a.bins_in[(size_t)j * Npad + r];
        if (a.bins0_tab) return a.bins0_tab[(size_t)n * a.bins0_stride + j];
        return linspace_at(0.0f, 1.0f, b0step, T + 1u, j);
    };
    float dirn[3] = {rs.d[0], rs.d[1], rs.d[2]};
#pragma unroll
    for (int pass = 0; pass < 2; ++pass) {
        const float aa = dirn[0] * dirn[0], bb = dirn[1] * dirn[1], cc = dirn[2] * dirn[2];
        const float nrm = sqrtf((aa + bb) + cc);
        dirn[0] = dirn[0] / nrm; dirn[1] = dirn[1] / nrm; dirn[2] = dirn[2] / nrm;
    }
    for (uint32_t c = 0; c < GEO; ++c) accf[c * 256u] = 0.0f;
    float dep = 0.0f;
    double cum = 0.0, wsum = 0.0;
    const TT *table = reinterpret_cast<const TT *>(a.table);
    float bprev = bin_at(0);
    float rb_prev = real_bin(rs, bprev);
    if (ok && a.dbg_bins) a.dbg_bins[(size_t)n * (T + 1)] = bprev;
    for (uint32_t j = 0; j < T; ++j) {
        const float bnext = bin_at(j + 1u);
        const float rb_next = real_bin(rs, bnext);
        const float tmid = (rb_next + rb_prev) / 2.0f;
        float p[3], x01[3];
        sample_x01(a.rc, rs, tmid, p, x01);
        const bool oob = (x01[0] < 0.0f || x01[0] > 1.0f) || (x01[1] < 0.0f || x01[1] > 1.0f) || (x01[2] < 0.0f || x01[2] > 1.0f);
        for (uint32_t l0 = 0; l0 < L; l0 += 4u) {
            float pos[4][3], v[4][8][2];
#pragma unroll
            for (uint32_t gi = 0; gi < 4u; ++gi) {
                const uint32_t l = umin(l0 + gi, L - 1u);
                const uint32_t res = a.g.res[l], size = a.g.size[l], mode = a.g.mode[l];
                const TT *tab = table + (size_t)a.g.off[l] * 2u;
                float deriv[3];
                uint32_t cell[3];
                grid_locate<3>(x01, res, a.g.align_corners != 0, a.g.interp, pos[gi], deriv, cell);
#pragma unroll
                for (uint32_t idx = 0; idx < 8u; ++idx) {
                    uint32_t q[3];
#pragma unroll
                    for (uint32_t d = 0; d < 3u; ++d) q[d] = (idx & (1u << d)) ? umin(cell[d] + 1u, res - 1u) : cell[d];
                    load_row<TT, 2>(tab + (size_t)grid_row<3>(q, res, size, mode) * 2u, v[gi][idx]);
                }
            }
#pragma unroll
            for (uint32_t gi = 0; gi < 4u; ++gi) {
                float acc[2] = {0.0f, 0.0f};
#pragma unroll
                for (uint32_t idx = 0; idx < 8u; ++idx) {
                    float w = 1.0f;
#pragma unroll
                    for (uint32_t d = 0; d < 3u; ++d) w *= (idx & (1u << d)) ? pos[gi][d] : 1.0f - pos[gi][d];
                    acc[0] = __builtin_fmaf(w, v[gi][idx][0], acc[0]);
                    acc[1] = __builtin_fmaf(w, v[gi][idx][1], acc[1]);
                }
                if (l0 + gi < L) {
                    bufA[(2u * (l0 + gi)) * 256u] = oob ? 0.0f : acc[0];
                    bufA[(2u * (l0 + gi) + 1u) * 256u] = oob ? 0.0f : acc[1];
                }
            }
        }
        float *xin = bufA, *xout = bufB;
        for (uint32_t i = 0; i < s.ng; ++i) {
            dense_any(s.wg[i], s.dg[i], s.dg[i + 1u], i + 1u < s.ng, xin, xout);
            float *t = xin; xin = xout; xout = t;
        }
        const float sigma = expf_det(xin[0]);
        const float delta = rb_next - rb_prev;
        float ds = delta * sigma;
        if (a.rc.last_opaque && j == T - 1u) ds = __builtin_inff();
        const float alpha = 1.0f - expf_det(-ds);
        const float tr = expf_det(-(float)cum);
        float w = alpha * tr;
        if (w != w) w = 0.0f;
        cum += (double)ds;
        wsum += (double)w;
        dep = __builtin_fmaf(w, tmid, dep);
        for (uint32_t c = 0; c < GEO; ++c) accf[c * 256u] = __builtin_fmaf(w, xin[(1u + c) * 256u], accf[c * 256u]);
        if (a.w_out) a.w_out[(size_t)j * Npad + r] = w;
        if (ok) {
            if (a.dbg_bins) a.dbg_bins[(size_t)n * (T + 1) + j + 1] = bnext;
            if (a.dbg_sigma) a.dbg_sigma[(size_t)n * T + j] = sigma;
// ... 824 lines not shown
    const auto key = std::make_pair(dev, caller);
    auto it = streams.find(key);
    if (it != streams.end()) return it->second;
    hipStream_t s = nullptr;
    if (hipStreamCreateWithFlags(&s, hipStreamNonBlocking) != hipSuccess) s = nullptr;
    streams[key] = s;
    return s;
}

struct BandFork {
    hipStream_t main_st, side = nullptr;
    hipEvent_t ev_fork = nullptr, ev_join = nullptr;
    BandFork(hipStream_t m, bool want) : main_st(m) {
        if (!want) return;
        hipStream_t s = band_side_stream(m);
        if (!s) return;
        if (hipEventCreateWithFlags(&ev_fork, hipEventDisableTiming) != hipSuccess) { ev_fork = nullptr; return; }
        if (hipEventCreateWithFlags(&ev_join, hipEventDisableTiming) != hipSuccess) { (void)hipEventDestroy(ev_fork); ev_fork = ev_join = nullptr; return; }
        if (hipEventRecord(ev_fork, main_st) != hipSuccess || hipStreamWaitEvent(s, ev_fork, 0) != hipSuccess) {
            (void)hipEventDestroy(ev_fork); (void)hipEventDestroy(ev_join); ev_fork = ev_join = nullptr; return;
        }
        side = s;
    }
    ~BandFork() {
        if (!side) return;
        (void)hipEventRecord(ev_join, side);
        (void)hipStreamWaitEvent(main_st, ev_join, 0);
        (void)hipEventDestroy(ev_fork); (void)hipEventDestroy(ev_join);
    }
};
}

using namespace sn;

extern "C" {

int sn_build_flags(void) {
    int f = 0;
#ifdef SN_EXPERIMENTS
    f |= SN_BUILD_EXPERIMENTS;
#endif
#ifdef SN_POISON_LDS
    f |= SN_BUILD_POISON_LDS;
#endif
    return f;
}

int sn_rm_last_launch_info(sn_launch_info *info) {
    SN_REQUIRE(info, "last_launch_info: NULL output");
    *info = g_launch;
    return SN_OK;
}

void sn_rm_profile_enable(int on) {
    g_prof_on = on != 0;
    {
        const int flag = g_prof_on ? 1 : 0;
        const unsigned long long zero[4] = {0, 0, 0, 0};
        if (g_prof_on) (void)hipMemcpyToSymbol(HIP_SYMBOL(g_clk_buf), zero, sizeof(zero));
        (void)hipMemcpyToSymbol(HIP_SYMBOL(g_clk_on), &flag, sizeof(flag));
    }
    if (!g_prof_on) {
        for (auto &sp : g_prof) { (void)hipEventDestroy(sp.a); (void)hipEventDestroy(sp.b); }
        g_prof.clear();
    }
}

int sn_rm_profile_shader_clock(float *shader_mhz, float *probe_ms) {
    SN_REQUIRE(shader_mhz, "profile_shader_clock: NULL output");
    *shader_mhz = 0.0f;
    if (probe_ms) *probe_ms = 0.0f;
    unsigned long long h[4];
    SN_HIP_OK(hipDeviceSynchronize());
    SN_HIP_OK(hipMemcpyFromSymbol(h, HIP_SYMBOL(g_clk_buf), sizeof(h)));
    int dev = 0, wall_khz = 0;
    SN_HIP_OK(hipGetDevice(&dev));
    SN_HIP_OK(hipDeviceGetAttribute(&wall_khz, hipDeviceAttributeWallClockRate, dev));
    if (h[3] <= h[1] || h[2] <= h[0] || wall_khz <= 0) return SN_OK;
    const double wall_s = (double)(h[3] - h[1]) / ((double)wall_khz * 1e3);
    *shader_mhz = (float)((double)(h[2] - h[0]) / wall_s / 1e6);
    if (probe_ms) *probe_ms = (float)(wall_s * 1e3);
    return SN_OK;
}

int sn_rm_profile_read(float *ms_per_class, int32_t *launches_per_class, int n_classes) {
    SN_REQUIRE(ms_per_class && launches_per_class && n_classes >= PK_CLASSES, "profile_read: need %d classes", (int)PK_CLASSES);
    for (int i = 0; i < n_classes; ++i) { ms_per_class[i] = 0.0f; launches_per_class[i] = 0; }
    for (auto &sp : g_prof) {
        SN_HIP_OK(hipEventSynchronize(sp.b));
        float ms = 0.0f;
        SN_HIP_OK(hipEventElapsedTime(&ms, sp.a, sp.b));
        ms_per_class[sp.cls] += ms; launches_per_class[sp.cls] += 1;
        (void)hipEventDestroy(sp.a); (void)hipEventDestroy(sp.b);
    }
    g_prof.clear();
    return SN_OK;
}

int sn_rm_debug_occupancy(int32_t *out, int32_t *lds, int n) {
    SN_REQUIRE(out && lds && n >= 3, "debug_occupancy: need 3 slots");
    int v = 0;
    SN_HIP_OK(hipOccupancyMaxActiveBlocksPerMultiprocessor(&v, k_prop_stage<float, 5, 2, 16, 3>, 256, 0));
    out[0] = v; lds[0] = 0;
    size_t l1 = (size_t)(PACK_FLOATS + 4 * 2 * 64 * SLAB_STRIDE) * sizeof(float);
    SN_HIP_OK(hipFuncSetAttribute(reinterpret_cast<const void *>(&k_final_stage<float, 16, 2, 64, 64, 16, 32, MLP_F16X3, 5>), hipFuncAttributeMaxDynamicSharedMemorySize, (int)l1));
    SN_HIP_OK(hipOccupancyMaxActiveBlocksPerMultiprocessor(&v, k_final_stage<float, 16, 2, 64, 64, 16, 32, MLP_F16X3, 5>, 256, l1));
    out[1] = v; lds[1] = (int32_t)l1;
    size_t l2 = (size_t)(PACK_FLOATS + 4 * 32 * 64) * sizeof(float);
    SN_HIP_OK(hipFuncSetAttribute(reinterpret_cast<const void *>(&k_final_stage<float, 16, 2, 64, 64, 16, 32, MLP_F32, -1>), hipFuncAttributeMaxDynamicSharedMemorySize, (int)l2));
    SN_HIP_OK(hipOccupancyMaxActiveBlocksPerMultiprocessor(&v, k_final_stage<float, 16, 2, 64, 64, 16, 32, MLP_F32, -1>, 256, l2));
    out[2] = v; lds[2] = (int32_t)l2;
    return SN_OK;
}

}

namespace sn {

constexpr uint64_t DENSIFY_MIN_SAMPLES = 64ull << 20;
constexpr uint64_t DENSIFY_MAX_VERTICES = 6ull << 20;
static int densify_levels(const GridLevels &g, int K, uint64_t samples, bool f16, int mode) {
    if (K != 5 || g.L != 16 || g.C != 2) return K;
    const bool want = mode == 2 || (mode == 0 && samples >= DENSIFY_MIN_SAMPLES && f16);
    if (!want) return K;
    uint64_t v = 0;
    for (int l = 0; l < K + 2; ++l) {
        if ((uint64_t)g.res[l] * g.res[l] * 16u >= (1u << 24)) return K;
        v += (uint64_t)g.res[l] * g.res[l] * g.res[l];
    }
    return v <= DENSIFY_MAX_VERTICES ? K + 2 : K;
}

static size_t pair_floats_of(const sn_grid_desc *d, uint64_t densify_samples = 0, int densify_mode = 1) {
    GridLevels g;
    if (d->D != 3 || d->C != 2 || build_grid_levels(&g, d->offsets, d->D, d->C, d->L, d->S, d->H, d->gridtype, (int)d->align_corners, d->interp) != SN_OK) return 0;
    if (!levels_fast(g)) return 0;
    uint32_t off[8];
    const int K = dense_prefix(g);
    return (size_t)pair_layout(g, densify_samples ? densify_levels(g, K, densify_samples, d->table_dtype == SN_F16, densify_mode) : K, off) * 4u;
}

static bool final_lv_fits(const GridLevels &g, int K, uint32_t row_bytes) {
    FinalLv probe;
    PairTab pt;
    pt.base = &probe;
    for (int l = 0; l < 8; ++l) pt.off[l] = 0;
    return build_final_lv(g, K, pt, &probe, row_bytes, probe);
}


constexpr int VIEW_W = 32 * 32 + 32 * 32 + 3 * 32;
static_assert(VIEW_W <= PACK_FLOATS, "view weights overlay the packed MLP weights");
constexpr size_t LDS_F16X3 = (size_t)(PACK_FLOATS + 4 * 2 * 64 * SLAB_STRIDE) * sizeof(float);
constexpr size_t LDS_F16X3_L0 = (size_t)(PACK_FLOATS + 4 * 2 * 64 * 16 + L0_MAX_ROWS) * sizeof(float);
constexpr size_t LDS_MFMA32 = (size_t)(PACK_FLOATS + 4 * 32 * 64) * sizeof(float);
constexpr size_t LDS_VALU = (size_t)(2 * 64 * 256 + VIEW_W) * sizeof(float);

static int experiment_of(const sn_render_cfg *cfg) {
#ifdef SN_EXPERIMENTS
    return cfg->tuning.experiment;
#else
    (void)cfg;
    return SN_EXP_NONE;
#endif
}

struct FinalRoute {
    enum Family { NONE, ANY, SP, CMP, RS, LT, LT_L0, PER_SAMPLE, MFMA32, VALU };
    Family family = NONE;
    bool f16 = false;
    int K = -1;
    bool aux = false, eo = false;
    int np = 3;
    bool clumped = false;
    bool canon = false;
    uint32_t grid = 0, block = 256;
    size_t lds = 0;
    const char *name = "";
    int dense = 0;
    uint32_t gathers = 0;
    uint32_t lpr_log2 = 0, spl_log2 = 0;
};
struct PropRoute {
    int K = -1;
    bool f16 = false, sp = false, pair = false;
    uint32_t lanes = 32, grid = 0;
};
struct FeatRoute {
    uint32_t C = 0, lg = 2, patch_levels = 0;
    bool f16 = false;
};
struct ChunkRoute {
    uint32_t n = 0, nblk = 0, Npad = 0;
    PropRoute prop[SN_MAX_STAGES];
    FinalRoute fin;
};
struct WorkspacePlan {
    BandPlan bands;
    size_t pair_main = 0, pair_prop[SN_MAX_STAGES] = {};
    size_t pair_floats = 0, slot_floats = 0;
    size_t head_floats() const { return (size_t)PACK_FLOATS + pair_floats; }
    size_t bytes() const { return ((size_t)bands.slots * slot_floats + head_floats()) * sizeof(float); }
};
struct RenderRoute {
    GridLevels gl_prop[SN_MAX_STAGES], gl_main, gl_feat;
    bool is_main = false, is_any = false;
    AnyShape any;
    int mlp_mode = MLP_F16X3, mlp_np = 3;
    bool use_cmp = false;
    int Kmain = -1;
    int Kv_main = 0;
    float stop_cum = 0.0f;
    WorkspacePlan ws;
    FinalRoute fin;
    FeatRoute feat;
    uint32_t chunks = 0;
    ChunkRoute full, last;
};

static WorkspacePlan plan_workspace(const sn_render_cfg *cfg, uint32_t N, uint32_t W) {
    WorkspacePlan w;
    w.bands = band_plan(cfg, N, W);
    const uint32_t nc = w.bands.chunk < N ? w.bands.chunk : N;
    w.slot_floats = stage_scratch_floats(cfg, blocks_for(nc, W, tile_log2w(cfg)) * 256u);
    w.pair_floats = w.pair_main = pair_floats_of(&cfg->grid, (uint64_t)N * cfg->num_steps[cfg->num_stages - 1], cfg->tuning.densify);
    for (uint32_t k = 0; k + 1 < cfg->num_stages; ++k) w.pair_floats += w.pair_prop[k] = pair_floats_of(&cfg->prop_grid[k]);
    return w;
}

static int check_io_pointers(const sn_render_cfg *cfg, const sn_render_io *io) {
    SN_REQUIRE(io->rays_o && io->rays_d, "render_rays: rays must be device pointers");
    if (io->skip_final) SN_REQUIRE(cfg->num_stages >= 2 && (cfg->num_stages > SN_MAX_STAGES  || io->bins[cfg->num_stages - 1]) && !cfg->with_feat,
                                   "render_rays: skip_final needs >= 2 stages, io->bins[last] for the resampled bins, and no feature stage");
    else SN_REQUIRE(io->image && io->depth && io->weights_sum, "render_rays: outputs must be device pointers");
    return SN_OK;
}

static void plan_final(const sn_render_cfg *cfg, const sn_render_io *io, RenderRoute *r) {
    const uint32_t S = cfg->num_stages;
    const bool f16 = cfg->grid.table_dtype == SN_F16;
    const int dp = dense_prefix(r->gl_main);
    const uint64_t main_samples = (uint64_t)io->N * cfg->num_steps[S - 1];
    r->Kv_main = r->is_any ? 0 : dp;
    const bool have_pairs = !r->is_any && dp > 0 && r->ws.pair_main != 0;
    r->Kmain = have_pairs && final_lv_fits(r->gl_main, dp, 2u * (f16 ? 2u : 4u)) ? dp : -1;
    if (cfg->compact_live && r->mlp_mode == MLP_F16X3 && !cfg->with_feat && !io->xyzs_last && !io->geo_feat_last && !io->skip_final &&
        io->bins0_ray_stride == 0) {
        bool any_dbg = false;
        for (uint32_t k = 1; k < S; ++k) any_dbg = any_dbg || io->u_ray_stride[k] != 0;
        for (uint32_t k = 0; k < S; ++k) any_dbg = any_dbg || io->bins[k] || io->weights[k] || io->sigmas[k] || io->inds[k];
        r->use_cmp = !any_dbg && dp == 5 && r->Kmain == 5;
    }
    if (io->skip_final) return;
    const bool dbg_last = io->bins[S - 1] || io->weights[S - 1] || io->sigmas[S - 1] || io->xyzs_last || io->geo_feat_last;
    const bool per_sample_out = dbg_last || cfg->with_feat;
    r->stop_cum = (cfg->early_stop_eps > 0.0f && cfg->early_stop_eps < 1.0f && !per_sample_out) ? -logf(cfg->early_stop_eps) : 0.0f;
    auto lv_gathers = [&](int kd) -> uint32_t { return (uint32_t)kd * (f16 ? 2u : 4u) + (uint32_t)(16 - kd) * 8u; };
    FinalRoute &f = r->fin;
    f.f16 = f16;
    f.aux = cfg->with_feat || r->stop_cum > 0.0f;
    f.eo = cfg->tuning.exact_early_out == 2;
    const int xp = experiment_of(cfg);
    const bool f16x3 = r->mlp_mode == MLP_F16X3;
    f.canon = xp == SN_EXP_GATHER_CANONICAL;
    if (r->is_any) {
        f.family = FinalRoute::ANY; f.name = "k_final_stage_any";
        f.lds = (size_t)(2u * r->any.rows + (r->any.dg[r->any.ng] - 1u)) * 256u * sizeof(float);
        f.dense = 0; f.gathers = cfg->grid.L * 8u;
    } else if (r->use_cmp) {
        f.family = FinalRoute::CMP; f.name = "k_final_stage_cmp"; f.K = 5; f.lds = LDS_F16X3; f.dense = 5; f.gathers = lv_gathers(5);
    } else if (f16x3 && r->Kmain == 5 && !f.aux && !per_sample_out && xp == SN_EXP_ROLE_SPLIT) {
        f.family = FinalRoute::RS; f.name = "k_final_stage_rs"; f.K = 5; f.dense = 5; f.gathers = lv_gathers(5);
    } else if (f16x3 && r->Kmain == 5 && !dbg_last && lt_enabled(cfg)) {
        const bool l0 = f16 && (uint64_t)r->gl_main.res[0] * r->gl_main.res[0] * r->gl_main.res[0] <= (uint64_t)L0_MAX_ROWS && xp == SN_EXP_LDS_LEVEL0;
        if (!f.aux && !cfg->compact_live) r->Kv_main = densify_levels(r->gl_main, 5, main_samples, f16, cfg->tuning.densify);
        const bool dens = r->Kv_main == 7 && !l0 && final_lv_fits(r->gl_main, 7, 2u * (f16 ? 2u : 4u));
        f.family = l0 ? FinalRoute::LT_L0 : FinalRoute::LT;
        f.K = dens ? 7 : 5;
        f.name = l0 ? "k_final_stage<lt,K=5,lds-level0>" : dens ? "k_final_stage<lt,K=7>" : f.aux ? "k_final_stage<lt,K=5,aux>" : "k_final_stage<lt,K=5>";
        f.dense = f.K; f.gathers = lv_gathers(f.K) - (l0 ? 2u : 0u);
        if (f16 && !f.eo && r->mlp_np == 1 && !f.aux && !l0) f.np = 1;
        f.clumped = xp == SN_EXP_MATRIX_CLUMPED && f.np == 3 && !l0;
        f.lds = l0 ? LDS_F16X3_L0 : (xp == SN_EXP_FINAL_ONE_WG && !dens && f.np == 3) ? (size_t)(84 * 1024) : LDS_F16X3;
    } else if (f16x3) {
        f.family = FinalRoute::PER_SAMPLE; f.K = r->Kmain == 5 ? 5 : -1; f.lds = LDS_F16X3;
        f.name = r->Kmain == 5 ? "k_final_stage<per-sample,K=5>" : "k_final_stage<per-sample,generic>";
        f.dense = r->Kmain; f.gathers = r->Kmain == 5 ? lv_gathers(5) : (uint32_t)dp * 4u + (16u - (uint32_t)dp) * 8u;
    } else if (r->mlp_mode == MLP_F32) {
        f.family = FinalRoute::MFMA32; f.name = "k_final_stage<mfma32>"; f.aux = true; f.lds = LDS_MFMA32; f.dense = -1; f.gathers = 16u * 8u;
    } else {
        f.family = FinalRoute::VALU; f.name = "k_final_stage<valu>"; f.aux = true; f.lds = LDS_VALU; f.dense = -1; f.gathers = 16u * 8u;
    }
}

static ChunkRoute plan_chunk(const sn_render_cfg *cfg, const sn_render_io *io, const RenderRoute &r, uint32_t n) {
    const uint32_t S = cfg->num_stages, W = io->tile_w;
    ChunkRoute c;
    c.n = n; c.nblk = blocks_for(n, W, tile_log2w(cfg)); c.Npad = c.nblk * 256u;
    for (uint32_t k = 0; k + 1 < S; ++k) {
        PropRoute &p = c.prop[k];
        const int K = dense_prefix(r.gl_prop[k]);
        p.K = (K == 3 || K == 2) ? K : -1;
        p.f16 = cfg->prop_grid[k].table_dtype != SN_F32;
        p.sp = W == 0 && n <= prop_sp_max_rays(cfg) && cfg->num_steps[k] <= SP_MAX_T;
        p.lanes = 32u;
        if (cfg->tuning.prop_sp_lanes == 8 || cfg->tuning.prop_sp_lanes == 16 || cfg->tuning.prop_sp_lanes == 32) p.lanes = (uint32_t)cfg->tuning.prop_sp_lanes;
        p.pair = cfg->tuning.prop_pair == 2 ||
                 (cfg->tuning.prop_pair == 0 && prop_pair_auto(r.ws.bands.slots == 2u ? blocks_for(io->N, W, tile_log2w(cfg)) : c.nblk));
        p.grid = p.sp ? c.Npad / (256u / p.lanes) : c.nblk;
    }
    c.fin = r.fin;
    FinalRoute &f = c.fin;
    f.grid = c.nblk;
    const uint32_t T = cfg->num_steps[S - 1];
#ifdef SN_EXPERIMENTS
    if (f.family == FinalRoute::RS) {
        f.grid = W ? ((W + 31u) >> 5) * ((n / W + 15u) >> 4) : div_up(n, (uint32_t)(RS_PROD * 64));
        f.block = RS_THREADS; f.lds = (size_t)RS_LDS_FLOATS * sizeof(float);
    }
#endif
    if (f.family != FinalRoute::NONE && f.family != FinalRoute::ANY && W == 0 && r.mlp_mode == MLP_F16X3 && r.stop_cum == 0.0f && !r.use_cmp &&
        n <= final_sp_max_rays(cfg) && T <= 64u * FSP_MAX_SPL) {
        auto lpr_log2_of = [&](uint32_t sl) { const uint32_t need = div_up(T, 1u << sl); uint32_t l2 = 0; while ((1u << l2) < need) ++l2; return l2; };
        uint32_t spl_log2 = 2;
        while (spl_log2 > 0 && div_up(T, 1u << (spl_log2 - 1)) <= 64u && (((size_t)c.Npad << lpr_log2_of(spl_log2)) >> 8) < SN_FINAL_SP_MIN_BLOCKS) --spl_log2;
        FinalRoute sp;
        sp.family = FinalRoute::SP; sp.name = "k_final_stage_sp"; sp.f16 = f.f16; sp.K = r.Kmain == 5 ? 5 : -1;
        sp.spl_log2 = spl_log2; sp.lpr_log2 = lpr_log2_of(spl_log2);
        sp.grid = (uint32_t)(((size_t)c.Npad << sp.lpr_log2) >> 8);
        sp.lds = final_sp_lds_floats(1u << spl_log2) * sizeof(float);
        sp.dense = r.Kmain; sp.gathers = r.Kmain == 5 ? (uint32_t)5 * (f.f16 ? 2u : 4u) + 11u * 8u : 16u * 8u;
        f = sp;
    }
    return c;
}

static void plan_chunks(const sn_render_cfg *cfg, const sn_render_io *io, RenderRoute *r) {
    const uint32_t chunk = r->ws.bands.chunk;
    r->chunks = div_up(io->N, chunk);
    r->full = plan_chunk(cfg, io, *r, io->N < chunk ? io->N : chunk);
    const uint32_t n_last = io->N - (r->chunks - 1u) * chunk;
    r->last = n_last == r->full.n ? r->full : plan_chunk(cfg, io, *r, n_last);
}

static int plan_render(const sn_render_cfg *cfg, const sn_render_io *io, RenderRoute *r) {
    SN_REQUIRE(io->out_stride == 0u || io->out_stride >= 5u, "render_rays: out_stride %u must be 0 (dense outputs) or at least 5 floats (rgb | depth | weights_sum per row)", io->out_stride);
    SN_REQUIRE(io->head_stride == 0u || (io->f_image && io->head_stride >= 31u + 4u && !io->skip_final),
               "render_rays: head_stride %u needs f_image and room for f_image | rgb | depth (>= 35 floats per row)", io->head_stride);
    SN_REQUIRE(cfg->tuning.wave_tile >= 0 && cfg->tuning.wave_tile <= 5, "render_rays: tuning.wave_tile %d outside 0..5", cfg->tuning.wave_tile);
    SN_REQUIRE(!(experiment_of(cfg) == SN_EXP_ROLE_SPLIT && cfg->tuning.wave_tile != 0 && cfg->tuning.wave_tile != 3), "render_rays: the role-split experiment is built for 8x8 wave tiles (tuning.wave_tile 0 or 3)");
    const uint32_t S = cfg->num_stages;
    SN_REQUIRE(S >= 1 && S <= SN_MAX_STAGES, "render_rays: num_stages=%u outside 1..%d", S, SN_MAX_STAGES);
    for (uint32_t k = 0; k < S; ++k) SN_REQUIRE(cfg->num_steps[k] >= 1, "render_rays: num_steps[%u] must be >= 1", k);
    SN_REQUIRE(cfg->sh_degree == 4, "render_rays: fused path is built for SH degree 4 (network.py:97), got %u", cfg->sh_degree);
    if (io->tile_w) SN_REQUIRE(io->N % io->tile_w == 0, "render_rays: N=%u is not a multiple of tile_w=%u", io->N, io->tile_w);
    SN_REQUIRE(io->bins0_ray_stride == 0 || (io->bins0_table && io->bins0_ray_stride >= cfg->num_steps[0] + 1u),
               "render_rays: bins0_ray_stride=%u needs bins0_table and at least num_steps[0]+1=%u values per ray", io->bins0_ray_stride, cfg->num_steps[0] + 1u);
    for (uint32_t k = 1; k < S; ++k)
        SN_REQUIRE(io->u_ray_stride[k] == 0 || (io->u_table[k] && io->u_ray_stride[k] >= cfg->num_steps[k] + 1u),
                   "render_rays: u_ray_stride[%u]=%u needs u_table[%u] and at least num_steps[%u]+1=%u values per ray", k, io->u_ray_stride[k], k, k, cfg->num_steps[k] + 1u);

    static const uint32_t d_prop[3] = {10, 16, 1};
    static const uint32_t d_main[4] = {32, 64, 64, 16};
    static const uint32_t d_view[4] = {31, 32, 32, 3};
    for (uint32_t k = 0; k + 1 < S; ++k) {
        int rc = to_levels(&r->gl_prop[k], &cfg->prop_grid[k]);
        if (rc) return rc;
        if (!(cfg->prop_grid[k].L == 5 && cfg->prop_grid[k].C == 2 && mlp_is(&cfg->prop_mlp[k], 2, d_prop) && levels_fast(r->gl_prop[k]))) {
            set_error("render_rays: proposal stage %u is not the L=5,F=2 grid + 10-16-1 bias-free ReLU MLP this build fuses (network.py:135-143)", k);
            return SN_ERR_UNSUPPORTED;
        }
    }
    {
        int rc = to_levels(&r->gl_main, &cfg->grid);
        if (rc) return rc;
    }
    r->is_main = cfg->grid.L == 16 && cfg->grid.C == 2 && mlp_is(&cfg->grid_mlp, 3, d_main) && mlp_is(&cfg->view_mlp, 3, d_view) && levels_fast(r->gl_main);
    memset(&r->any, 0, sizeof(r->any));
    if (!r->is_main) {
        const sn_mlp_desc *gm = &cfg->grid_mlp, *vm = &cfg->view_mlp;
        auto plain = [](const sn_mlp_desc *m) {
            if (m->num_layers < 1u || m->num_layers > ANY_LAYERS || m->activation != 0u || m->skip_mask != 0u) return false;
            for (uint32_t l = 0; l < m->num_layers; ++l) if (m->bias[l] != nullptr || m->weight[l] == nullptr) return false;
            for (uint32_t l = 0; l <= m->num_layers; ++l) if (m->dims[l] < 1u || m->dims[l] > ANY_W) return false;
            return true;
        };
        r->is_any = cfg->grid.D == 3 && cfg->grid.C == 2 && cfg->grid.L >= 1 && cfg->grid.L * 2u <= ANY_W && plain(gm) && plain(vm) &&
                    gm->dims[0] == cfg->grid.L * 2u && gm->dims[gm->num_layers] >= 2u && gm->dims[gm->num_layers] - 1u <= ANY_GEO &&
                    cfg->sh_degree == 4u && vm->dims[0] == gm->dims[gm->num_layers] - 1u + 16u && vm->dims[vm->num_layers] == 3u;
        if (r->is_any) {
            AnyShape &a = r->any;
            a.ng = gm->num_layers; a.nv = vm->num_layers;
            for (uint32_t l = 0; l <= gm->num_layers; ++l) a.dg[l] = gm->dims[l];
            for (uint32_t l = 0; l <= vm->num_layers; ++l) a.dv[l] = vm->dims[l];
            for (uint32_t l = 0; l < gm->num_layers; ++l) a.wg[l] = gm->weight[l];
            for (uint32_t l = 0; l < vm->num_layers; ++l) a.wv[l] = vm->weight[l];
            uint32_t wmax = 0;
            for (uint32_t l = 0; l <= gm->num_layers; ++l) wmax = gm->dims[l] > wmax ? gm->dims[l] : wmax;
            for (uint32_t l = 0; l <= vm->num_layers; ++l) wmax = vm->dims[l] > wmax ? vm->dims[l] : wmax;
            a.rows = wmax <= 16u ? 16u : wmax <= 32u ? 32u : 64u;
        }
    }
    if (!r->is_main && !r->is_any) {
        set_error("render_rays: the field is neither the L=16,F=2 grid + 32-64-64-16 / 31-32-32-3 MLPs (network.py:93-98) nor of the shape the "
                  "size-agnostic final stage takes (3-D grid with level_dim 2 and <= 32 levels' worth of 64 features, bias-free ReLU MLPs of "
                  "<= 4 layers and <= 64 neurons, <= 31 geometry channels, degree-4 SH)");
        return SN_ERR_UNSUPPORTED;
    }
    if (r->is_any && (cfg->compact_live || cfg->with_feat)) {
        set_error("render_rays: compact_live / the in-render feature stage are instantiated for the reference network's sizes only");
        return SN_ERR_UNSUPPORTED;
    }
    if (cfg->with_feat) {
        SN_REQUIRE(io->f_feat, "render_rays: with_feat is set but io->f_feat is NULL");
        SN_REQUIRE(cfg->feat_grid.embeddings && table_aligned(cfg->feat_grid.embeddings) && table_aligned(io->f_feat),
                   "render_rays: feature grid table / f_feat must be 16-byte aligned device pointers");
        int rc = to_levels(&r->gl_feat, &cfg->feat_grid);
        if (rc) return rc;
        const GridLevels &gf = r->gl_feat;
        if (!levels_fast(gf) || !(gf.C == 2 || gf.C == 4 || gf.C == 8)) {
            set_error("render_rays: feature grid must be a hash grid with level_dim 2/4/8, align_corners=False, linear "
                      "interpolation (network.py:103); use sn_rm_grid_composite for other grids");
            return SN_ERR_UNSUPPORTED;
        }
        int lg = 2;
        if (cfg->tuning.feat_levels) lg = cfg->tuning.feat_levels;
        if (lg != 1 && lg != 2 && lg != 4) lg = 2;
        while (gf.L % (uint32_t)lg) lg >>= 1;
        FeatRoute &ft = r->feat;
        ft.C = gf.C; ft.lg = (uint32_t)lg; ft.f16 = cfg->feat_grid.table_dtype == SN_F16;
        uint32_t n_dense = 0;
        while (n_dense < gf.L && (gf.mode[n_dense] & 1u) == 0u) ++n_dense;
        const uint32_t whole = ((n_dense + ft.lg - 1u) / ft.lg) * ft.lg;
        ft.patch_levels = cfg->tuning.feat_patch != 1 ? 0u : whole > gf.L ? gf.L : whole;
    }
    r->mlp_mode = cfg->mlp_exact_fp32 ? MLP_F32 : MLP_F16X3;
    r->mlp_np = 3;
    switch (cfg->tuning.mlp_mode) {
        case SN_MLP_F16X1: r->mlp_mode = MLP_F16X3; r->mlp_np = 1; break;
        case SN_MLP_AUTO: break;
        case SN_MLP_F16X3: r->mlp_mode = MLP_F16X3; break;
        case SN_MLP_MFMA32: r->mlp_mode = MLP_F32; break;
        case SN_MLP_VALU: r->mlp_mode = MLP_VALU; break;
        default: set_error("render_rays: unknown tuning.mlp_mode=%d", cfg->tuning.mlp_mode); return SN_ERR_INVALID;
    }
    if (cfg->tuning.experiment != SN_EXP_NONE && !(sn_build_flags() & SN_BUILD_EXPERIMENTS)) {
        set_error("render_rays: tuning.experiment=%d needs a library built with -DSN_EXPERIMENTS (make exp)", cfg->tuning.experiment);
        return SN_ERR_UNSUPPORTED;
    }
    r->ws = plan_workspace(cfg, io->N, io->tile_w);
    plan_final(cfg, io, r);
    plan_chunks(cfg, io, r);
    return SN_OK;
}

static void note_final(const FinalRoute &f, sn_launch_info *info) {
    snprintf(info->final_kernel, sizeof(info->final_kernel), "%s", f.name);
    info->workgroups = f.grid; info->lds_bytes = (uint32_t)f.lds; info->dense_levels = (uint32_t)(f.dense < 0 ? 0 : f.dense);
    info->gathers_per_wave_sample = f.gathers; info->launches += 1u;
}

template <typename... P, typename... A>
static int launch(void (*kern)(P...), dim3 grid, dim3 block, size_t lds, hipStream_t st, const A &...args) {
    if (lds) SN_HIP_OK(hipFuncSetAttribute(reinterpret_cast<const void *>(kern), hipFuncAttributeMaxDynamicSharedMemorySize, (int)lds));
    hipLaunchKernelGGL(kern, grid, block, lds, st, args...);
    return SN_OK;
}

using PropKern = void (*)(PropArgs);
template <typename TT, int K> static PropKern prop_kernel_of(const PropRoute &p) {
    if (p.sp) {
        if (p.lanes == 8u) return k_prop_stage_sp<TT, 5, 2, 16, K, 8>;
        if (p.lanes == 16u) return k_prop_stage_sp<TT, 5, 2, 16, K, 16>;
        return k_prop_stage_sp<TT, 5, 2, 16, K, 32>;
    }
    if (p.pair) return k_prop_stage<TT, 5, 2, 16, K, 2>;
    return k_prop_stage<TT, 5, 2, 16, K>;
}
static PropKern prop_kernel(const PropRoute &p) {
    switch (p.K) {
        case 3: return p.f16 ? prop_kernel_of<__half, 3>(p) : prop_kernel_of<float, 3>(p);
        case 2: return p.f16 ? prop_kernel_of<__half, 2>(p) : prop_kernel_of<float, 2>(p);
        default: return p.f16 ? prop_kernel_of<__half, -1>(p) : prop_kernel_of<float, -1>(p);
    }
}

using FinalKern = void (*)(FinalArgs);
template <typename TT, int MODE, int K, bool AUX = false, bool LT = false, bool L0L = false, bool EO = false, int NP = 3, bool PORD = false, bool CANON = false>
static FinalKern fs() { return k_final_stage<TT, 16, 2, 64, 64, 16, 32, MODE, K, AUX, LT, L0L, EO, NP, PORD, CANON>; }
template <typename TT> static FinalKern final_kernel_of(const FinalRoute &f) {
    constexpr bool half = std::is_same<TT, __half>::value;
    switch (f.family) {
#ifdef SN_EXPERIMENTS
        case FinalRoute::CMP: return f.canon ? k_final_stage_cmp<TT, 5, true> : k_final_stage_cmp<TT, 5>;
#else
        case FinalRoute::CMP: return k_final_stage_cmp<TT, 5>;
#endif
#ifdef SN_EXPERIMENTS
        case FinalRoute::RS: return k_final_stage_rs<TT, 5>;
        case FinalRoute::LT_L0:
            if constexpr (half) return f.aux ? fs<__half, MLP_F16X3, 5, true, true, true>() : fs<__half, MLP_F16X3, 5, false, true, true>();
            return nullptr;
#endif
        case FinalRoute::LT:
            if constexpr (half) {
                if (f.np == 1) return f.K == 7 ? fs<__half, MLP_F16X3, 7, false, true, false, false, 1>() : fs<__half, MLP_F16X3, 5, false, true, false, false, 1>();
            }
#ifdef SN_EXPERIMENTS
            if (f.clumped) {
                if (f.K == 7) return f.eo ? fs<TT, MLP_F16X3, 7, false, true, false, true, 3, true>() : fs<TT, MLP_F16X3, 7, false, true, false, false, 3, true>();
                if (f.aux) return f.eo ? fs<TT, MLP_F16X3, 5, true, true, false, true, 3, true>() : fs<TT, MLP_F16X3, 5, true, true, false, false, 3, true>();
                return f.eo ? fs<TT, MLP_F16X3, 5, false, true, false, true, 3, true>() : fs<TT, MLP_F16X3, 5, false, true, false, false, 3, true>();
            }
            if (f.canon && f.np == 3) {
                if (f.K == 7) return f.eo ? fs<TT, MLP_F16X3, 7, false, true, false, true, 3, false, true>() : fs<TT, MLP_F16X3, 7, false, true, false, false, 3, false, true>();
                if (f.aux) return f.eo ? fs<TT, MLP_F16X3, 5, true, true, false, true, 3, false, true>() : fs<TT, MLP_F16X3, 5, true, true, false, false, 3, false, true>();
                return f.eo ? fs<TT, MLP_F16X3, 5, false, true, false, true, 3, false, true>() : fs<TT, MLP_F16X3, 5, false, true, false, false, 3, false, true>();
            }
#endif
            if (f.K == 7) return f.eo ? fs<TT, MLP_F16X3, 7, false, true, false, true>() : fs<TT, MLP_F16X3, 7, false, true, false, false>();
            if (f.aux) return f.eo ? fs<TT, MLP_F16X3, 5, true, true, false, true>() : fs<TT, MLP_F16X3, 5, true, true, false, false>();
            return f.eo ? fs<TT, MLP_F16X3, 5, false, true, false, true>() : fs<TT, MLP_F16X3, 5, false, true, false, false>();
        case FinalRoute::PER_SAMPLE:
#ifdef SN_EXPERIMENTS
            if (f.canon && f.K == 5) return f.aux ? fs<TT, MLP_F16X3, 5, true, false, false, false, 3, false, true>() : fs<TT, MLP_F16X3, 5, false, false, false, false, 3, false, true>();
#endif
            if (f.K == 5) return f.aux ? fs<TT, MLP_F16X3, 5, true>() : fs<TT, MLP_F16X3, 5, false>();
            return f.aux ? fs<TT, MLP_F16X3, -1, true>() : fs<TT, MLP_F16X3, -1, false>();
        case FinalRoute::MFMA32: return fs<TT, MLP_F32, -1, true>();
        case FinalRoute::VALU: return fs<TT, MLP_VALU, -1, true>();
        default: return nullptr;
    }
}

static int launch_final(const FinalRoute &f, hipStream_t st, const FinalArgs &fa, const AnyShape &any) {
    const dim3 grid(f.grid), block(f.block);
    switch (f.family) {
        case FinalRoute::ANY:
            return f.f16 ? launch(k_final_stage_any<__half>, grid, block, f.lds, st, fa, any) : launch(k_final_stage_any<float>, grid, block, f.lds, st, fa, any);
        case FinalRoute::SP:
            if (f.K == 5) return f.f16 ? launch(k_final_stage_sp<__half, 5>, grid, block, f.lds, st, fa, f.lpr_log2, f.spl_log2) : launch(k_final_stage_sp<float, 5>, grid, block, f.lds, st, fa, f.lpr_log2, f.spl_log2);
            return f.f16 ? launch(k_final_stage_sp<__half, -1>, grid, block, f.lds, st, fa, f.lpr_log2, f.spl_log2) : launch(k_final_stage_sp<float, -1>, grid, block, f.lds, st, fa, f.lpr_log2, f.spl_log2);
        default: {
            const FinalKern kern = f.f16 ? final_kernel_of<__half>(f) : final_kernel_of<float>(f);
            if (!kern) { set_error("render_rays: no kernel for the last-stage route %s", f.name); return SN_ERR_UNSUPPORTED; }
            return launch(kern, grid, block, f.lds, st, fa);
        }
    }
}

using FeatKern = void (*)(FeatArgs);
template <typename TT, int C> static FeatKern feat_kernel_of(uint32_t lg, bool patch) {
    if (patch) {
        if (lg == 4u) return k_feat_stage<TT, C, 4, true>;
        if (lg == 2u) return k_feat_stage<TT, C, 2, true>;
        return k_feat_stage<TT, C, 1, true>;
    }
    if (lg == 4u) return k_feat_stage<TT, C, 4>;
    if (lg == 2u) return k_feat_stage<TT, C, 2>;
    return k_feat_stage<TT, C, 1>;
}
static FeatKern feat_kernel(const FeatRoute &ft, bool patch) {
    switch (ft.C) {
        case 8: return ft.f16 ? feat_kernel_of<__half, 8>(ft.lg, patch) : feat_kernel_of<float, 8>(ft.lg, patch);
        case 4: return ft.f16 ? feat_kernel_of<__half, 4>(ft.lg, patch) : feat_kernel_of<float, 4>(ft.lg, patch);
        default: return ft.f16 ? feat_kernel_of<__half, 2>(ft.lg, patch) : feat_kernel_of<float, 2>(ft.lg, patch);
    }
}
}

extern "C" {

size_t sn_rm_render_workspace_bytes(const sn_render_cfg *cfg, uint32_t N, uint32_t tile_w) {
    if (!cfg || N == 0 || cfg->num_stages < 1 || cfg->num_stages > SN_MAX_STAGES) return (size_t)PACK_FLOATS * sizeof(float);
    return plan_workspace(cfg, N, tile_w).bytes();
}

int sn_rm_render_route_info(const sn_render_cfg *cfg, const sn_render_io *io, sn_launch_info *out) {
    SN_REQUIRE(cfg && io && out, "render_route_info: cfg/io/out is NULL");
    *out = sn_launch_info{};
    if (io->N == 0) return SN_OK;
    int rc = check_io_pointers(cfg, io);
    if (rc) return rc;
    RenderRoute route;
    rc = plan_render(cfg, io, &route);
    if (rc) return rc;
    if (io->skip_final) return SN_OK;
    note_final(route.last.fin, out);
    out->launches = route.chunks;
    return SN_OK;
}

static_assert(sizeof(sn_render_io) == 312 && offsetof(sn_render_io, pack_valid) == 292 && offsetof(sn_render_io, workspace) == 296,
              "sn_render_io.pack_valid sits in the padding after head_stride: the struct's layout is ABI 12's");

int sn_rm_tile_order_info(uint32_t W, uint32_t rows, int32_t wave_tile, int32_t order, uint32_t workgroup, sn_tile_order_info *out) {
    SN_REQUIRE(out, "tile_order_info: out is NULL");
    SN_REQUIRE(W >= 1u && rows >= 1u && (uint64_t)W * rows <= 0xffffffffull, "tile_order_info: W=%u rows=%u is not an image of 1..2^32-1 rays", W, rows);
    SN_REQUIRE(wave_tile >= 0 && wave_tile <= 5, "tile_order_info: wave_tile %d outside 0..5", wave_tile);
    const uint32_t tlw = wave_tile ? (uint32_t)wave_tile : 3u, tlh = 6u - tlw, tw = 1u << tlw, th = 1u << tlh;
    const uint32_t nwg = blocks_for(W * rows, W, tlw);
    SN_REQUIRE(workgroup < nwg, "tile_order_info: workgroup %u outside the launch of %u", workgroup, nwg);
    const TileOrder to = tile_order_of(order, tlw);
    const uint32_t tx8 = (W + tw - 1u) >> tlw, ty8 = (rows + th - 1u) >> tlh;
    *out = sn_tile_order_info{};
    out->workgroups = nwg;
    out->tile_id = to.xcd ? xcd_tile_id(workgroup, nwg) : workgroup;
    out->tile_w = tw; out->tile_h = th;
    for (uint32_t wave = 0; wave < 4u; ++wave) {
        uint32_t wx, wy;
        wave_tile_of(out->tile_id * 4u + wave, tx8, ty8, to.st_w, to.st_h, wx, wy);
        const bool ok = wx < tx8 && (wy << tlh) < rows;
        out->x[wave] = ok ? (int32_t)(wx << tlw) : -1;
        out->y[wave] = ok ? (int32_t)(wy << tlh) : -1;
    }
    return SN_OK;
}

int sn_rm_render_rays(const sn_render_cfg *cfg, const sn_render_io *io, sn_stream_t stream) {
    SN_REQUIRE(cfg && io, "render_rays: cfg/io is NULL");
    if (io->N == 0) return SN_OK;
    g_launch = sn_launch_info{};
    int rc = check_io_pointers(cfg, io);
    if (rc) return rc;
    RenderRoute route;
    rc = plan_render(cfg, io, &route);
    if (rc) return rc;
    SN_REQUIRE(io->workspace != nullptr, "render_rays: workspace is NULL");
    SN_REQUIRE(table_aligned(io->workspace), "render_rays: workspace must be 16-byte aligned");
    if (io->workspace_bytes / sizeof(float) < route.ws.bytes() / sizeof(float)) {
        set_error("render_rays: workspace too small (%zu bytes, need %zu)", io->workspace_bytes, route.ws.bytes());
        return SN_ERR_WORKSPACE;
    }
    const uint32_t S = cfg->num_stages, W = io->tile_w;
    const hipStream_t st_main = (hipStream_t)stream;
    const GridLevels &gl_main = route.gl_main;
    float *pack = reinterpret_cast<float *>(io->workspace);
    float *pair_mem = pack + PACK_FLOATS;
    float *scratch = pair_mem + route.ws.pair_floats;

    const bool packed_before = io->pack_valid == SN_PACK_VALID;
    if (route.mlp_mode != MLP_VALU && !route.is_any && !packed_before) {
        ProfScope ps(st_main, PK_PACK);
        if (route.mlp_mode == MLP_F16X3)
            rc = launch(k_pack_grid_mlp_f16, dim3(PACK16_VECS * 64 / 256), dim3(256), 0, st_main, cfg->grid_mlp.weight[0], cfg->grid_mlp.weight[1],
                        cfg->grid_mlp.weight[2], reinterpret_cast<uint4 *>(pack));
        else
            rc = launch(k_pack_grid_mlp, dim3(PACK_FLOATS / 256), dim3(256), 0, st_main, cfg->grid_mlp.weight[0], cfg->grid_mlp.weight[1], cfg->grid_mlp.weight[2], pack);
        if (rc) return rc;
        SN_LAUNCH_CHECK("k_pack_grid_mlp");
    }
    PairTab pairs, prop_pairs[SN_MAX_STAGES];
    {
        float *cursor = pair_mem;
        auto pack_pairs = [&](const sn_grid_desc *d, const GridLevels &gl, PairTab &pt, int Kp, size_t fl) -> int {
            pt.base = nullptr;
            for (int l = 0; l < 8; ++l) pt.off[l] = 0;
            if (fl == 0 || Kp <= 0) return SN_OK;
            pair_layout(gl, Kp, pt.off);
            pt.base = cursor;
            cursor += fl;
            if (packed_before) return SN_OK;
            uint32_t max_rows = 0;
            for (int l = 0; l < Kp; ++l) { const uint32_t r3 = gl.res[l] * gl.res[l] * gl.res[l]; if (r3 > max_rows) max_rows = r3; }
            const dim3 gp(div_up(max_rows, 256), (uint32_t)Kp);
            const int rcl = d->table_dtype == SN_F16 ? launch(k_pack_pairs<__half>, gp, dim3(256), 0, st_main, (const __half *)d->embeddings, gl, pt, (uint32_t)Kp)
                                                     : launch(k_pack_pairs<float>, gp, dim3(256), 0, st_main, (const float *)d->embeddings, gl, pt, (uint32_t)Kp);
            if (rcl) return rcl;
            SN_LAUNCH_CHECK("k_pack_pairs");
            return SN_OK;
        };
        ProfScope ps(st_main, PK_PACK);
        rc = pack_pairs(&cfg->grid, gl_main, pairs, route.Kv_main, route.ws.pair_main);
        if (rc) return rc;
        for (uint32_t k = 0; k + 1 < S; ++k) {
            rc = pack_pairs(&cfg->prop_grid[k], route.gl_prop[k], prop_pairs[k], dense_prefix(route.gl_prop[k]), route.ws.pair_prop[k]);
            if (rc) return rc;
        }
    }

    BandFork fork(st_main, route.ws.bands.slots == 2u);
    if (route.ws.bands.slots == 2u && !fork.side) {
        route.ws.bands.slots = 1u;
        plan_chunks(cfg, io, &route);
    }
    const uint32_t chunk = route.ws.bands.chunk;
    for (uint32_t ci = 0; ci < route.chunks; ++ci) {
        const uint32_t first = ci * chunk;
        const ChunkRoute &cr = ci + 1u < route.chunks ? route.full : route.last;
        const uint32_t n = cr.n, Npad = cr.Npad;
        const uint32_t slot = fork.side ? (ci & 1u) : 0u;
        const hipStream_t st = slot ? fork.side : st_main;
        RayCommon rays;
        rays.rays_o = io->rays_o + (size_t)first * 3; rays.rays_d = io->rays_d + (size_t)first * 3;
        rays.cnf = io->cam_near_far ? io->cam_near_far + (size_t)first * 2 : nullptr;
        rays.N = n; rays.W = W; rays.rows = W ? n / W : 0; rays.Npad = Npad;
        for (int i = 0; i < 6; ++i) rays.aabb[i] = cfg->aabb[i];
        rays.min_near = cfg->min_near; rays.bound = cfg->bound; rays.contract = cfg->contract;
        rays.last_opaque = cfg->last_sample_opaque; rays.bg = cfg->bg_color;
        {
            int e = 0;
            const float m = frexpf(2.0f * cfg->bound, &e);
            rays.inv_den = (m == 0.5f && e > -100 && e < 100) ? 1.0f / (2.0f * cfg->bound) : 0.0f;
        }
        {
            rays.tlw = tile_log2w(cfg);
            const TileOrder to = tile_order_of(cfg->tuning.linear_tile_order, rays.tlw);
            rays.xcd_swizzle = to.xcd; rays.st_w = to.st_w; rays.st_h = to.st_h;
            if (route.use_cmp) rays.xcd_swizzle = 0;
            if (cr.fin.family == FinalRoute::RS) rays.st_w = rays.st_h = 0;
        }

        float *w_scr[SN_MAX_STAGES] = {nullptr}, *b_scr[SN_MAX_STAGES] = {nullptr};
        float *cur = scratch + (size_t)slot * route.ws.slot_floats;
        for (uint32_t k = 0; k + 1 < S; ++k) { w_scr[k] = cur; cur += (size_t)cfg->num_steps[k] * Npad; }
        for (uint32_t k = 1; k < S; ++k) { b_scr[k] = cur; cur += (size_t)(cfg->num_steps[k] + 1) * Npad; }
        if (cfg->with_feat) { w_scr[S - 1] = cur; cur += (size_t)cfg->num_steps[S - 1] * Npad; }

        for (uint32_t k = 0; k + 1 < S; ++k) {
            PropArgs pa;
            pa.rc = rays; pa.g = route.gl_prop[k]; pa.table = cfg->prop_grid[k].embeddings;
            pa.w0 = cfg->prop_mlp[k].weight[0]; pa.w1 = cfg->prop_mlp[k].weight[1];
            pa.T = cfg->num_steps[k]; pa.Tn = cfg->num_steps[k + 1];
            pa.bins_in = b_scr[k];
            pa.bins0_stride = io->bins0_ray_stride; pa.u_stride = io->u_ray_stride[k + 1];
            pa.bins0_tab = (k == 0 && io->bins0_table) ? io->bins0_table + (size_t)first * pa.bins0_stride : nullptr;
            pa.u_tab = io->u_table[k + 1] ? io->u_table[k + 1] + (size_t)first * pa.u_stride : nullptr;
            pa.dbg_bins_next = (io->skip_final && k + 2 == S && io->bins[S - 1]) ? io->bins[S - 1] + (size_t)first * (cfg->num_steps[S - 1] + 1) : nullptr;
            pa.w_scr = w_scr[k]; pa.bins_out = b_scr[k + 1];
            pa.dbg_bins = io->bins[k] ? io->bins[k] + (size_t)first * (pa.T + 1) : nullptr;
            pa.dbg_w = io->weights[k] ? io->weights[k] + (size_t)first * pa.T : nullptr;
            pa.dbg_sigma = io->sigmas[k] ? io->sigmas[k] + (size_t)first * pa.T : nullptr;
            pa.dbg_inds = io->inds[k + 1] ? io->inds[k + 1] + (size_t)first * (pa.Tn + 1) : nullptr;
            pa.pairs = prop_pairs[k];
            pa.skip_miss = route.use_cmp ? 1 : 0;
            {
                ProfScope ps(st, PK_PROP0 + (int)k);
                rc = launch(prop_kernel(cr.prop[k]), dim3(cr.prop[k].grid), dim3(256), 0, st, pa);
                if (rc) return rc;
            }
            SN_LAUNCH_CHECK("k_prop_stage");
        }
        if (io->skip_final) continue;
        const FinalRoute &fr = cr.fin;
        FinalArgs fa;
        fa.rc = rays; fa.g = gl_main; fa.table = cfg->grid.embeddings; fa.mlp_pack = pack;
        for (int l = 0; l < 3; ++l) { fa.w[l] = cfg->grid_mlp.weight[l]; fa.vw[l] = cfg->view_mlp.weight[l]; }
        fa.T = cfg->num_steps[S - 1];
        fa.bins_in = b_scr[S - 1]; fa.bins0_stride = io->bins0_ray_stride;
        fa.bins0_tab = (S == 1 && io->bins0_table) ? io->bins0_table + (size_t)first * fa.bins0_stride : nullptr;
        fa.sh_degree = cfg->sh_degree;
        fa.istride = io->out_stride ? io->out_stride : 3u; fa.sstride = io->out_stride ? io->out_stride : 1u;
        fa.image = io->image + (size_t)first * fa.istride; fa.depth = io->depth + (size_t)first * fa.sstride; fa.wsum = io->weights_sum + (size_t)first * fa.sstride;
        fa.dbg_bins = io->bins[S - 1] ? io->bins[S - 1] + (size_t)first * (fa.T + 1) : nullptr;
        fa.dbg_w = io->weights[S - 1] ? io->weights[S - 1] + (size_t)first * fa.T : nullptr;
        fa.dbg_sigma = io->sigmas[S - 1] ? io->sigmas[S - 1] + (size_t)first * fa.T : nullptr;
        fa.dbg_xyz = io->xyzs_last ? io->xyzs_last + (size_t)first * fa.T * 3 : nullptr;
        const uint32_t geo = route.is_any ? route.any.dg[route.any.ng] - 1u : 15u;
        fa.dbg_geo = io->geo_feat_last ? io->geo_feat_last + (size_t)first * fa.T * geo : nullptr;
        fa.fimg_stride = io->head_stride ? io->head_stride : geo + 16u;
        fa.dbg_fimg = io->f_image ? io->f_image + (size_t)first * fa.fimg_stride : nullptr;
        fa.head_rgbd = (io->head_stride && io->f_image && !route.is_any) ? fa.dbg_fimg + 31 : nullptr;
        fa.pairs = pairs;
        build_final_lv(gl_main, fr.K == 7 ? 7 : dense_prefix(gl_main), pairs, cfg->grid.embeddings, 2u * (fr.f16 ? 2u : 4u), fa.lv);
        fa.w_out = cfg->with_feat ? w_scr[S - 1] : nullptr;
        fa.stop_cum = route.stop_cum;
        {
            ProfScope ps_final(st, PK_FINAL);
            note_final(fr, &g_launch);
            rc = launch_final(fr, st, fa, route.any);
            if (rc) return rc;
            SN_LAUNCH_CHECK(fr.family == FinalRoute::ANY ? "k_final_stage_any" : "k_final_stage");
        }
        if (cfg->with_feat) {
            const GridLevels &gf = route.gl_feat;
            const FeatRoute &feat = route.feat;
            FeatArgs ft;
            ft.rc = rays; ft.g = gf; ft.table = cfg->feat_grid.embeddings; ft.T = cfg->num_steps[S - 1];
            ft.bins_in = b_scr[S - 1]; ft.bins0_stride = io->bins0_ray_stride;
            ft.bins0_tab = (S == 1 && io->bins0_table) ? io->bins0_table + (size_t)first * ft.bins0_stride : nullptr;
            ft.w_in = w_scr[S - 1];
            ft.out_stride = io->head_stride ? io->head_stride : gf.L * gf.C;
            ft.out = io->f_feat + (size_t)first * ft.out_stride;
            ProfScope ps_feat(st, PK_FEAT);
            if (feat.patch_levels) {
                ft.level0 = 0;
                rc = launch(feat_kernel(feat, true), dim3(cr.nblk, feat.patch_levels / feat.lg), dim3(256), 0, st, ft);
                if (rc) return rc;
            }
            if (feat.patch_levels < gf.L) {
                ft.level0 = feat.patch_levels;
                rc = launch(feat_kernel(feat, false), dim3(cr.nblk, (gf.L - feat.patch_levels) / feat.lg), dim3(256), 0, st, ft);
                if (rc) return rc;
            }
            SN_LAUNCH_CHECK("k_feat_stage");
        }
    }
    return SN_OK;
}

}
```

sanerf-hq_amd/raymarching/__init__.py:

```python
from .._buffers import zeros_f32
from .march import (
    composite, contract, distort_loss, generate_rays, rays_from_pixels, near_far_from_aabb, proposal_loss_stage, proposal_loss_all, sample_pdf,
    sample_positions, weights_from_sigma, ray_composite, PROPOSAL_LOSS_MAX_T, WEIGHTS_BACKWARD_MAX_T, DISTORT_LOSS_MAX_T, _host_values)
from .jitter import jitter, jitter_tables, DeviceJitter
from .mask import mask_nll, ray_pair_select, ray_pair_rgb_loss, mask_error, error_map_update, mask_output
from .meters import (
    mask_eval_accumulate, image_sqerr_accumulate, image_ssim_accumulate, ssim_record, ssim_workspace, read_ssim_record, eval_record,
    eval_workspace, read_eval_record)
from .distill import feature_distill_loss, feature_map
from .rgb_loss import rgb_loss
from .prompts import points_lift, point_store, point_store_update, points_project, prompt_overlay, reference_resize_ratio
from .collate import weighted_draw, collate_gather, COLLATE_OUTPUTS
from .heads import (
    grid_composite, mlp_forward, mlp_wide_overflow, mask_head, mask_head_fusable, mask_point_labels, mask_point_labels_fusable)
from .object import object_composite, keep_mask_of, LABEL_SKIPPED
from .mesh import lattice_points, isosurface, isosurface_counts, isosurface_emit, ISOSURFACE_MAX_VERTICES
from .mesh import mesh_components, mesh_clean, mesh_filter_counts, mesh_filter_emit
from .mesh import mesh_split, mesh_split_counts, mesh_split_emit, MESH_SPLIT_PARTS
from .mesh import mesh_simplify, mesh_simplify_counts, mesh_simplify_emit
from .mesh import mesh_smooth, mesh_vertex_normals, mesh_smooth_build, mesh_smooth_steps, mesh_smooth_emit, smooth_quantisation
from .mesh import mesh_rasterize, mesh_rasterize_clip, mesh_raster_project, mesh_raster_draw, mesh_raster_resolve, RASTER_SMALL_MAX_PIXELS, RASTER_MAX_SIDE
from .mesh import vertex_probe_points, vertex_probe_composite, PROBE_SAMPLES
from .render import RenderPlan, Tuning, tuning, last_launch_info, route_info, tile_order_info, render_rays, FP16_SPLIT_LIMIT
```

sanerf-hq_amd/raymarching/render.py:

```python
from __future__ import annotations

import ctypes as C
import warnings
from typing import Dict, List, Optional, Sequence

import numpy as np
import torch

from .. import _lib
from ._args import _f32, _flat3


class Tuning:
    FIELDS = ("mlp_mode", "per_sample_form", "densify", "linear_tile_order", "prop_sp_max_rays", "final_sp_max_rays", "feat_levels", "band_streams", "exact_early_out", "wave_tile", "prop_sp_lanes", "feat_patch", "prop_pair", "experiment")

    def __init__(self, **kw):
        for f in self.FIELDS:
            setattr(self, f, 0)
        for k, v in kw.items():
            if k not in self.FIELDS:
                raise TypeError(f"Tuning: unknown field {k!r} (fields: {', '.join(self.FIELDS)})")
            setattr(self, k, int(v))

    def write(self, ct) -> None:
        for f in self.FIELDS:
            setattr(ct, f, int(getattr(self, f)))

    def __repr__(self):
        return "Tuning(" + ", ".join(f"{f}={getattr(self, f)}" for f in self.FIELDS if getattr(self, f)) + ")"


tuning = Tuning()
FP16_SPLIT_LIMIT = 65504.0 * 0.5


def last_launch_info() -> dict:
    info = _lib.LaunchInfo()
    _lib.check(_lib.lib().sn_rm_last_launch_info(C.byref(info)), "last_launch_info")
    return dict(final_kernel=info.final_kernel.decode(), workgroups=int(info.workgroups), lds_bytes=int(info.lds_bytes),
                dense_levels=int(info.dense_levels), gathers_per_wave_sample=int(info.gathers_per_wave_sample), launches=int(info.launches))


def tile_order_info(W: int, rows: int, workgroup: int, wave_tile: int = 0, order: int = 0) -> dict:
    info = _lib.TileOrderInfo()
    _lib.check(_lib.lib().sn_rm_tile_order_info(int(W), int(rows), int(wave_tile), int(order), int(workgroup), C.byref(info)), "tile_order_info")
    return dict(workgroups=int(info.workgroups), tile_id=int(info.tile_id), tile_w=int(info.tile_w), tile_h=int(info.tile_h),
                tiles=[(int(info.x[w]), int(info.y[w])) if info.x[w] >= 0 else None for w in range(4)])


def _fill_grid(desc: _lib.GridDesc, enc, table: torch.Tensor) -> None:
    from ..gridencoder.grid import _host_offsets
    offs = _host_offsets(enc.offsets)
    desc.embeddings = table.data_ptr()
    desc.table_dtype = _lib.SN_F16 if table.dtype == torch.float16 else _lib.SN_F32
    for i, o in enumerate(offs):
        desc.offsets[i] = o
    desc.D, desc.C, desc.L = enc.input_dim, enc.level_dim, enc.num_levels
    desc.S = float(np.float32(np.log2(enc.per_level_scale)))
    desc.H = int(enc.base_resolution)
    desc.gridtype, desc.align_corners, desc.interp = enc.gridtype_id, int(enc.align_corners), enc.interp_id


def _fill_mlp(desc: _lib.MlpDesc, layers: Sequence[torch.nn.Linear], dim_in: int, keep: list) -> None:
    desc.num_layers = len(layers)
    desc.activation = 0
    desc.skip_mask = 0
    desc.dims[0] = dim_in
    for l, lin in enumerate(layers):
        w = _f32(lin.weight)
        keep.append(w)
        desc.weight[l] = w.data_ptr()
        desc.dims[l + 1] = w.shape[0]
        if lin.bias is not None:
            b = _f32(lin.bias)
            keep.append(b)
            desc.bias[l] = b.data_ptr()
        else:
            desc.bias[l] = None


class RenderPlan:

    def __init__(self, model, num_steps: Sequence[int], table_dtype=torch.float32, feat_encoder=None,
                 early_stop_eps: float = 0.0, compact_live: bool = False, tuning: Optional["Tuning"] = None, keep_packs: bool = False):
        self.keep: list = []
        self.keep_packs = bool(keep_packs)
        self._pack_key = None
        self.pack_reuses = 0
        self.tuning = tuning
        cfg = _lib.RenderCfg()
        S = len(num_steps)
        if not 1 <= S <= _lib.MAX_STAGES:
            raise RuntimeError(f"num_steps must have 1..{_lib.MAX_STAGES} entries")
        cfg.num_stages = S
        for k, t in enumerate(num_steps):
            cfg.num_steps[k] = int(t)

        self.copies: list = []

        def table_of(enc):
            src = enc.embeddings.detach()
            t = src
            if src.dtype != table_dtype or not src.is_contiguous():
                t = src.to(table_dtype).contiguous()
                self.copies.append((enc.embeddings, t))
            self.keep.append(t)
            return t

        for k in range(S - 1):
            enc = model.prop_encoders[k]
            _fill_grid(cfg.prop_grid[k], enc, table_of(enc))
            _fill_mlp(cfg.prop_mlp[k], list(model.prop_mlp[k].net), model.prop_mlp[k].dim_in, self.keep)
        _fill_grid(cfg.grid, model.grid, table_of(model.grid))
        _fill_mlp(cfg.grid_mlp, list(model.grid_mlp.net), model.grid_mlp.dim_in, self.keep)
        _fill_mlp(cfg.view_mlp, list(model.view_mlp.net), model.view_mlp.dim_in, self.keep)
        cfg.sh_degree = model.view_encoder.degree
        ab = model.aabb_infer.detach().cpu().tolist()
        for i in range(6):
            cfg.aabb[i] = ab[i]
        cfg.min_near = float(model.min_near)
        cfg.bound = float(model.bound)
        cfg.contract = int(bool(model.opt.contract))
        cfg.last_sample_opaque = int(model.opt.background == "last_sample")
        cfg.bg_color = 1.0
        self.feat_dim = 0
        if feat_encoder is not None:
            _fill_grid(cfg.feat_grid, feat_encoder, table_of(feat_encoder))
            cfg.with_feat = 1
            self.feat_dim = feat_encoder.output_dim
        cfg.early_stop_eps = float(early_stop_eps)
        cfg.compact_live = int(bool(compact_live))
        self.cfg = cfg
        self._range_model = model
        self._range_versions = None
        self.activation_bound = 0.0
        self.check_range()
        self.num_steps = [int(t) for t in num_steps]
        self.geo = int(getattr(model, "geom_feat_dim", list(model.grid_mlp.net)[-1].weight.shape[0] - 1))
        self.ncol = self.geo + model.view_encoder.output_dim
        self._ws: Optional[torch.Tensor] = None

    @torch.no_grad()
    def check_range(self) -> None:
        m = self._range_model
        tensors = [m.grid.embeddings] + [lin.weight for lin in m.grid_mlp.net]
        versions = tuple((t.data_ptr(), t._version) for t in tensors)
        if versions == self._range_versions:
            return
        self._range_versions = versions
        layers = list(m.grid_mlp.net)
        stats = [m.grid.embeddings.detach().abs().max().float()]
        stats += [lin.weight.detach().float().abs().sum(dim=1).max() for lin in layers[:-1]]
        stats += [lin.weight.detach().abs().max().float() for lin in layers]
        vals = torch.stack(stats).tolist()
        bound = worst = vals[0]
        for row_l1 in vals[1:len(layers)]:
            bound = row_l1 * bound
            worst = max(worst, bound)
        wmax = max(vals[len(layers):]) if layers else 0.0
        if any(v != v for v in vals):
            worst = float("nan")
        self.activation_bound = max(worst, wmax)
        exact = not (self.activation_bound < FP16_SPLIT_LIMIT)
        if exact and not self.cfg.mlp_exact_fp32:
            warnings.warn(f"fused render: activations of the 32-64-64-16 MLP are only bounded by {self.activation_bound:.3g} "
                          f"(>= {FP16_SPLIT_LIMIT:.0f}): using the exact fp32 matrix-core path instead of split-fp16")
        self.cfg.mlp_exact_fp32 = int(exact)

    def invalidate_range(self) -> None:
        self._range_versions = None
        self._pack_key = None

    def invalidate_packs(self) -> None:
        self._pack_key = None

    def _pack_key_of(self, io, stream: int):
        present = tuple(bool(v) for v in (io.cam_near_far, io.bins0_table, *io.u_table, io.image, *io.bins, *io.weights, *io.sigmas, *io.inds,
                                          io.xyzs_last, io.geo_feat_last, io.f_image, io.f_feat))
        shape = (io.N, io.tile_w, io.bins0_ray_stride, tuple(io.u_ray_stride), io.skip_final, io.out_stride, io.head_stride, present)
        return (bytes(self.cfg), tuple((t.data_ptr(), t._version) for t in self.keep), shape, io.workspace, io.workspace_bytes, stream)

    @torch.no_grad()
    def refresh_tables(self) -> None:
        for src, copy in self.copies:
            copy.copy_(src.detach())

    def workspace(self, N: int, tile_w: int, device) -> torch.Tensor:
        (self.tuning or tuning).write(self.cfg.tuning)
        need = int(_lib.lib().sn_rm_render_workspace_bytes(C.byref(self.cfg), N, tile_w))
        if self._ws is None or self._ws.numel() < need or self._ws.device != torch.device(device):
            self._ws = torch.empty(need, dtype=torch.uint8, device=device)
            self._pack_key = None
        return self._ws


def _fill_io(plan: RenderPlan, io, N: int, tile_w: int, want, u_tables, bins0_table, skip_final: bool, packed, head_input: bool, tuning, buf, table):
    io.N, io.tile_w = N, int(tile_w)
    if bins0_table is not None:
        b0, io.bins0_table = table(bins0_table)
        if b0.dim() == 2:
            if b0.shape != (N, plan.num_steps[0] + 1):
                raise RuntimeError(f"bins0_table: expected [{N}, {plan.num_steps[0] + 1}] per-ray bins, got {tuple(b0.shape)}")
            io.bins0_ray_stride = b0.shape[1]
    if u_tables:
        for k, u in u_tables.items():
            u, io.u_table[k] = table(u)
            if u.dim() == 2:
                if u.shape != (N, plan.num_steps[k] + 1):
                    raise RuntimeError(f"u_tables[{k}]: expected [{N}, {plan.num_steps[k] + 1}] per-ray values, got {tuple(u.shape)}")
                io.u_ray_stride[k] = u.shape[1]
    S = plan.cfg.num_stages
    want = set(want)
    if skip_final:
        if S < 2:
            raise RuntimeError("render_rays(skip_final=True) needs a schedule with proposal stages")
        io.skip_final = 1
        want = set()
        io.bins[S - 1] = buf(f"bins{S - 1}", (N, plan.num_steps[S - 1] + 1))
    else:
        plan.check_range()
        if packed is not None:
            base = packed.data_ptr()
            io.image, io.depth, io.weights_sum, io.out_stride = base, base + 12, base + 16, packed.shape[1]
        else:
            io.image = buf("image", (N, 3))
            io.depth = buf("depth", (N,))
            io.weights_sum = buf("weights_sum", (N,))
    for k in range(S):
        T = plan.num_steps[k]
        if "bins" in want or (k == S - 1 and "bins_last" in want):
            io.bins[k] = buf(f"bins{k}", (N, T + 1))
        if "weights" in want or (k == S - 1 and "weights_last" in want):
            io.weights[k] = buf(f"weights{k}", (N, T))
        if "sigmas" in want or (k == S - 1 and "sigmas_last" in want):
            io.sigmas[k] = buf(f"sigmas{k}", (N, T))
        if "inds" in want and k >= 1:
            io.inds[k] = buf(f"inds{k}", (N, T + 1), torch.int32)
    Tl = plan.num_steps[S - 1]
    if "xyzs_last" in want:
        io.xyzs_last = buf("xyzs_last", (N, Tl, 3))
    if "geo_feat_last" in want:
        io.geo_feat_last = buf("geo_feat_last", (N, Tl, plan.geo))
    if head_input and plan.cfg.with_feat and not skip_final:
        io.f_feat = buf("head_input", (N, plan.feat_dim + plan.ncol + 4))
        io.f_image, io.head_stride = io.f_feat + 4 * plan.feat_dim, plan.feat_dim + plan.ncol + 4
    else:
        if "f_image" in want:
            io.f_image = buf("f_image", (N, plan.ncol))
        if plan.cfg.with_feat and not skip_final:
            io.f_feat = buf("f_feat", (N, plan.feat_dim))
    eff = tuning or plan.tuning or globals()["tuning"]
    eff.write(plan.cfg.tuning)
    return eff


def route_info(plan: RenderPlan, N: int, tile_w: int = 0, want: Sequence[str] = (), u_tables: Optional[Dict[int, torch.Tensor]] = None,
               bins0_table: Optional[torch.Tensor] = None, skip_final: bool = False, tuning: Optional["Tuning"] = None,
               packed: Optional[torch.Tensor] = None, head_input: bool = False) -> dict:
    io = _lib.RenderIO()
    stand_in = 64
    io.rays_o = io.rays_d = stand_in
    _fill_io(plan, io, int(N), tile_w, want, u_tables, bins0_table, skip_final, packed, head_input, tuning,
             lambda name, shape, dtype=torch.float32: stand_in, lambda t: (t, stand_in))
    info = _lib.LaunchInfo()
    _lib.check(_lib.lib().sn_rm_render_route_info(C.byref(plan.cfg), C.byref(io), C.byref(info)), "route_info")
    return dict(final_kernel=info.final_kernel.decode(), workgroups=int(info.workgroups), lds_bytes=int(info.lds_bytes),
                dense_levels=int(info.dense_levels), gathers_per_wave_sample=int(info.gathers_per_wave_sample), launches=int(info.launches))


def render_rays(plan: RenderPlan, rays_o, rays_d, cam_near_far=None, bg_color: float = 1.0, tile_w: int = 0,
                want: Sequence[str] = (), u_tables: Optional[Dict[int, torch.Tensor]] = None,
                bins0_table: Optional[torch.Tensor] = None, out: Optional[Dict[str, torch.Tensor]] = None,
                skip_final: bool = False, tuning: Optional["Tuning"] = None, packed: Optional[torch.Tensor] = None,
                head_input: bool = False):
    rays_o, rays_d = _flat3(rays_o), _flat3(rays_d)
    N = rays_o.shape[0]
    device = rays_o.device
    io = _lib.RenderIO()
    res: Dict[str, torch.Tensor] = {} if out is None else out
    keep: List[torch.Tensor] = []

    def buf(name, shape, dtype=torch.float32):
        t = res.get(name)
        if t is None or tuple(t.shape) != tuple(shape) or t.dtype != dtype or t.device != device or not t.is_contiguous():
            t = torch.empty(shape, device=device, dtype=dtype)
            res[name] = t
        return _lib.dev(t, name, dtype)

    def table(t):
        t = t.to(device).contiguous().float()
        keep.append(t)
        return t, t.data_ptr()

    io.rays_o, io.rays_d = _lib.dev(rays_o, "rays_o"), _lib.dev(rays_d, "rays_d")
    if cam_near_far is not None:
        cnf = cam_near_far.float()
        if cnf.shape[0] == 1:
            cnf = cnf.expand(N, 2)
        cnf = cnf.contiguous()
        keep.append(cnf)
        io.cam_near_far = _lib.dev(cnf, "cam_near_far")
    if packed is not None and not skip_final:
        if not (packed.is_cuda and packed.dtype == torch.float32 and packed.dim() == 2 and packed.shape[0] == N and packed.shape[1] >= 5
                and packed.is_contiguous() and packed.device == device):
            raise RuntimeError(f"render_rays: packed must be a contiguous fp32 [{N}, >=5] tensor on {device}, got {tuple(packed.shape)} {packed.dtype}")
        res["image"], res["depth"], res["weights_sum"] = packed[:, :3], packed[:, 3], packed[:, 4]
    eff = _fill_io(plan, io, N, tile_w, want, u_tables, bins0_table, skip_final, packed, head_input, tuning, buf, table)
    S = plan.cfg.num_stages
    if io.head_stride:
        hb = res["head_input"]
        res["f_feat"], res["f_image"] = hb[:, :plan.feat_dim], hb[:, plan.feat_dim:plan.feat_dim + plan.ncol]
    need = int(_lib.lib().sn_rm_render_workspace_bytes(C.byref(plan.cfg), N, int(tile_w)))
    ws = plan.workspace(N, int(tile_w), device)
    if ws.numel() < need:
        plan._ws = ws = torch.empty(need, dtype=torch.uint8, device=device)
        plan._pack_key = None
    eff.write(plan.cfg.tuning)
    io.workspace, io.workspace_bytes = ws.data_ptr(), ws.numel()
    plan.cfg.bg_color = float(bg_color)
    stream = _lib.stream()
    key = plan._pack_key_of(io, stream) if plan.keep_packs else None
    reuse = key is not None and key == plan._pack_key
    io.pack_valid = _lib.PACK_VALID if reuse else 0
    plan._pack_key = None
    _lib.check(_lib.lib().sn_rm_render_rays(C.byref(plan.cfg), C.byref(io), stream), "render_rays")
    plan._pack_key = key
    plan.pack_reuses += int(reuse)
    if "weights_last" in set(want) and not skip_final:
        res["weights_last"] = res[f"weights{S - 1}"]
    return res
```

Before: 106.7 million.

## Add persistent-workgroup final stage with per-XCD atomic tile queues

Adds a persistent variant of the final render kernel: a fixed number of 512-thread workgroups stage the MLP and view weights into LDS once, then repeatedly pull 64-ray wave tiles from eight per-XCD atomic counters, stealing from other XCDs' queues once their own is empty. The per-ray body is factored into a shared device function so both the classic and persistent kernels use it. The aim is to amortise weight staging and balance uneven per-ray work (early termination) across CUs. The cost is atomic contention, an extra reset launch, and larger LDS per workgroup that may lower occupancy.

```diff
diff --git a/include/sanerf_hip.h b/include/sanerf_hip.h
--- a/include/sanerf_hip.h
+++ b/include/sanerf_hip.h
@@ -287,6 +287,8 @@
     int32_t feat_patch;
     int32_t prop_pair;
     int32_t experiment;
+    int32_t persistent_tiles;
+    int32_t persistent_wgs;
 } sn_render_tuning;
 
 typedef struct sn_render_cfg {
@@ -347,9 +349,16 @@
 typedef struct sn_launch_info {
     char     final_kernel[64];
     uint32_t workgroups, lds_bytes, dense_levels, gathers_per_wave_sample, launches;
+    uint32_t persistent_tiles, grid_workgroups;
 } sn_launch_info;
 int sn_rm_last_launch_info(sn_launch_info *info);
 int sn_rm_render_route_info(const sn_render_cfg *cfg, const sn_render_io *io, sn_launch_info *out);
+int sn_rm_render_route_info_cus(const sn_render_cfg *cfg, const sn_render_io *io, uint32_t compute_units, sn_launch_info *out);
+
+typedef struct sn_tile_queue_info {
+    uint32_t queues, wave_tiles, begin, end;
+} sn_tile_queue_info;
+int sn_rm_tile_queue_info(uint32_t units, int32_t order, int32_t wave_tile, uint32_t queue, sn_tile_queue_info *out);
 
 typedef struct sn_tile_order_info {
     uint32_t workgroups, tile_id, tile_w, tile_h;
diff --git a/sanerf-hq_amd/_lib.py b/sanerf-hq_amd/_lib.py
--- a/sanerf-hq_amd/_lib.py
+++ b/sanerf-hq_amd/_lib.py
@@ -81,12 +81,17 @@
 
 class RenderTuning(C.Structure):
     _fields_ = [("mlp_mode", C.c_int32), ("per_sample_form", C.c_int32), ("densify", C.c_int32), ("linear_tile_order", C.c_int32),
-                ("prop_sp_max_rays", C.c_int32), ("final_sp_max_rays", C.c_int32), ("feat_levels", C.c_int32), ("band_streams", C.c_int32), ("exact_early_out", C.c_int32), ("wave_tile", C.c_int32), ("prop_sp_lanes", C.c_int32), ("feat_patch", C.c_int32), ("prop_pair", C.c_int32), ("experiment", C.c_int32)]
+                ("prop_sp_max_rays", C.c_int32), ("final_sp_max_rays", C.c_int32), ("feat_levels", C.c_int32), ("band_streams", C.c_int32), ("exact_early_out", C.c_int32), ("wave_tile", C.c_int32), ("prop_sp_lanes", C.c_int32), ("feat_patch", C.c_int32), ("prop_pair", C.c_int32), ("experiment", C.c_int32),
+                ("persistent_tiles", C.c_int32), ("persistent_wgs", C.c_int32)]
 
 
 class LaunchInfo(C.Structure):
     _fields_ = [("final_kernel", C.c_char * 64), ("workgroups", C.c_uint32), ("lds_bytes", C.c_uint32), ("dense_levels", C.c_uint32),
-                ("gathers_per_wave_sample", C.c_uint32), ("launches", C.c_uint32)]
+                ("gathers_per_wave_sample", C.c_uint32), ("launches", C.c_uint32), ("persistent_tiles", C.c_uint32), ("grid_workgroups", C.c_uint32)]
+
+
+class TileQueueInfo(C.Structure):
+    _fields_ = [("queues", C.c_uint32), ("wave_tiles", C.c_uint32), ("begin", C.c_uint32), ("end", C.c_uint32)]
 
 
 class TileOrderInfo(C.Structure):
@@ -241,6 +246,8 @@
     "sn_rm_last_launch_info": (_int, [_vp]),
     "sn_rm_render_route_info": (_int, [C.POINTER(RenderCfg), C.POINTER(RenderIO), _vp]),
     "sn_rm_tile_order_info": (_int, [_u32, _u32, _i32, _i32, _u32, C.POINTER(TileOrderInfo)]),
+    "sn_rm_render_route_info_cus": (_int, [C.POINTER(RenderCfg), C.POINTER(RenderIO), _u32, _vp]),
+    "sn_rm_tile_queue_info": (_int, [_u32, _i32, _i32, _u32, C.POINTER(TileQueueInfo)]),
     "sn_debug_eval": (_int, [_int, _vp, _vp, _u32, _vp, _vp]),
 }
 
diff --git a/sanerf-hq_amd/csrc/render.hip b/sanerf-hq_amd/csrc/render.hip
--- a/sanerf-hq_amd/csrc/render.hip
+++ b/sanerf-hq_amd/csrc/render.hip
@@ -33,6 +33,13 @@
 __host__ __device__ __forceinline__ uint32_t xcd_tile_id(uint32_t b, uint32_t nwg) {
     const uint32_t xcd = b & 7u, q = nwg >> 3, r = nwg & 7u;
     return (xcd < r ? xcd * (q + 1u) : r * (q + 1u) + (xcd - r) * q) + (b >> 3);
+}
+__host__ __device__ __forceinline__ void tile_queue_range(uint32_t x, uint32_t units, int xcd, uint32_t &begin, uint32_t &end) {
+    if (!xcd) { begin = 0u; end = x == 0u ? 4u * units : 0u; return; }
+    const uint32_t q = units >> 3, r = units & 7u;
+    const uint32_t first = x < r ? x * (q + 1u) : r * (q + 1u) + (x - r) * q;
+    begin = 4u * first;
+    end = 4u * (first + q + (x < r ? 1u : 0u));
 }
 __device__ __forceinline__ uint32_t tile_id_x(const RayCommon &rc, uint32_t b, uint32_t nwg) { return rc.xcd_swizzle ? xcd_tile_id(b, nwg) : b; }
 __device__ __forceinline__ uint32_t tile_id(const RayCommon &rc) { return tile_id_x(rc, blockIdx.x, gridDim.x); }
@@ -55,13 +62,10 @@
     wy = 2u * (y0 + ry) + (g & 1u);
 }
 
-__device__ __forceinline__ bool ray_of_lane(const RayCommon &rc, uint32_t wg, uint32_t &n) {
-    const uint32_t tid = threadIdx.x;
+__device__ __forceinline__ bool ray_of_wave_tile(const RayCommon &rc, uint32_t g, uint32_t lane, uint32_t &n) {
     if (rc.W) {
         const uint32_t tlw = rc.tlw, tlh = 6u - tlw, tw = 1u << tlw, th = 1u << tlh;
         const uint32_t tx8 = (rc.W + tw - 1u) >> tlw, ty8 = (rc.rows + th - 1u) >> tlh;
-        const uint32_t wave = __builtin_amdgcn_readfirstlane(tid >> 6), lane = tid & 63u;
-        const uint32_t g = wg * 4u + wave;
         uint32_t wx, wy;
         wave_tile_of(g, tx8, ty8, rc.st_w, rc.st_h, wx, wy);
         const uint32_t py = (wy << tlh) + (lane >> tlw);
@@ -70,10 +74,15 @@
         n = ok ? py * rc.W + px : 0u;
         return ok;
     }
-    n = wg * 256u + tid;
+    n = g * 64u + lane;
     const bool ok = n < rc.N;
     if (!ok) n = 0;
     return ok;
+}
+__device__ __forceinline__ bool ray_of_lane(const RayCommon &rc, uint32_t wg, uint32_t &n) {
+    const uint32_t tid = threadIdx.x;
+    const uint32_t wave = __builtin_amdgcn_readfirstlane(tid >> 6);
+    return ray_of_wave_tile(rc, wg * 4u + wave, tid & 63u, n);
 }
 
 struct RaySetup {
@@ -1650,70 +1659,34 @@
 #define SN_FINAL_WAVES 2
 #endif
 
-template <typename TT, int L, int C, int H1, int H2, int NOUT, int VH, int MODE, int K, bool AUX = false, bool LT = false, bool L0L = false, bool EO = false, int NP = 3, bool PORD = false,
-          bool CANON = false>
-__global__ __launch_bounds__(256, MODE == MLP_VALU ? 1 : SN_FINAL_WAVES) void k_final_stage(FinalArgs a) {
-    SN_POISON_ALL();
-    static_assert(NP == 3 || (LT && !L0L && !AUX), "reduced-product MLP forms: plain linear-tail instantiations only");
-    static_assert(!LT || (MODE == MLP_F16X3 && K >= 4 && K <= 8), "linear tail: split-fp16 MLP on the FinalLv path");
-    static_assert(!L0L || (LT && sizeof(TT) == 2), "LDS-resident level 0: fp16 tables, linear-tail instantiation (80 KiB: 32 packed weights + 4 x 8 swizzled slabs + 16 level 0)");
+struct FinalLds {
+    float *lds;
+    float *fe;
+    uint32_t fstride;
+    float *actB;
+    float *lds_vw;
+    uint32_t *slab_hi, *slab_lo;
+    const uint32_t *l0tab;
+};
+
+template <typename TT, int L, int C, int H1, int H2, int NOUT, int VH, int MODE, int K, bool AUX, bool LT, bool L0L, bool EO, int NP, bool PORD, bool CANON, bool PT>
+__device__ __forceinline__ void final_stage_rays(const FinalArgs &a, const FinalLds &fl, const uint32_t g) {
     constexpr int SLAB_DW = L0L ? 16 : SLAB_STRIDE;
     constexpr bool MFMA = MODE != MLP_VALU;
     constexpr int IN = L * C;
     constexpr int GEO = NOUT - 1;
     constexpr int NSH = 16;
     constexpr int NCOL = GEO + NSH;
-    static_assert(!MFMA || (IN == 32 && H1 == 64 && H2 == 64 && NOUT == 16), "MFMA path is the 32-64-64-16 MLP");
-    extern __shared__ __attribute__((aligned(16))) float lds[];
-    float *fe;
-    uint32_t fstride;
-    float *actB = nullptr;
     constexpr int VW0 = VH * PadIn<NCOL>::value, VW1 = VH * PadIn<VH>::value;
-    float *lds_vw;
-    uint32_t *slab_hi = nullptr, *slab_lo = nullptr;
-    if constexpr (MODE == MLP_F16X3) {
-        static_assert(PACK16_U4 * 4 == PACK_FLOATS, "both packings fill the same 32 KiB");
-        for (uint32_t i = threadIdx.x; i < (uint32_t)PACK16_U4; i += 256u)
-            reinterpret_cast<uint4 *>(lds)[i] = reinterpret_cast<const uint4 *>(a.mlp_pack)[i];
-        if constexpr (LT) { __syncthreads(); stage_w3p(lds + W3P_OFFSET, a.w[2]); }
-        constexpr int WAVE_SLAB = 2 * 64 * SLAB_DW;
-        float *wave_base = lds + PACK_FLOATS + (threadIdx.x >> 6) * WAVE_SLAB;
-        slab_hi = reinterpret_cast<uint32_t *>(wave_base);
-        slab_lo = slab_hi + 64 * SLAB_DW;
-        if constexpr (L0L) {
-            uint32_t *l0w = reinterpret_cast<uint32_t *>(lds + PACK_FLOATS + 4 * WAVE_SLAB);
-            const uint32_t rows0 = a.g.res[0] * a.g.res[0] * a.g.res[0];
-            const uint32_t *src = reinterpret_cast<const uint32_t *>(a.table) + a.g.off[0];
-            for (uint32_t i = threadIdx.x; i < rows0; i += 256u) l0w[i] = src[i];
-        }
-        fe = wave_base + (threadIdx.x & 63u);
-        fstride = 64u;
-        lds_vw = lds;
-    } else if constexpr (MODE == MLP_F32) {
-        for (uint32_t i = threadIdx.x; i < (uint32_t)PACK_FLOATS / 4u; i += 256u)
-            reinterpret_cast<float4 *>(lds)[i] = reinterpret_cast<const float4 *>(a.mlp_pack)[i];
-        fe = lds + PACK_FLOATS + (threadIdx.x >> 6) * (IN * 64) + (threadIdx.x & 63u);
-        fstride = 64u;
-        lds_vw = lds;
-    } else {
-        fe = lds + threadIdx.x;
-        actB = lds + 64 * 256 + threadIdx.x;
-        fstride = 256u;
-        lds_vw = lds + 2 * 64 * 256;
-    }
-    if constexpr (!MFMA) {
-        stage_weights<NCOL, VH>(lds_vw, a.vw[0]);
-        stage_weights<VH, VH>(lds_vw + VW0, a.vw[1]);
-        stage_weights<VH, 3>(lds_vw + VW0 + VW1, a.vw[2]);
-    }
-    __syncthreads();
-    clock_probe(0);
-    const uint32_t *l0tab = reinterpret_cast<const uint32_t *>(lds + PACK_FLOATS + 4 * 2 * 64 * SLAB_DW);
+    float *const lds = fl.lds, *const fe = fl.fe, *const actB = fl.actB, *const lds_vw = fl.lds_vw;
+    const uint32_t fstride = fl.fstride;
+    uint32_t *const slab_hi = fl.slab_hi, *const slab_lo = fl.slab_lo;
+    const uint32_t *const l0tab = fl.l0tab;
+    (void)SLAB_DW; (void)MFMA; (void)actB; (void)l0tab; (void)VW0; (void)VW1;
 
     uint32_t n;
-    const uint32_t wg = tile_id(a.rc);
-    const bool ok = ray_of_lane(a.rc, wg, n);
-    const uint32_t r = wg * 256u + threadIdx.x;
+    const bool ok = ray_of_wave_tile(a.rc, g, threadIdx.x & 63u, n);
+    const uint32_t r = g * 64u + (threadIdx.x & 63u);
     const uint32_t Npad = a.rc.Npad;
     RaySetup rs;
     setup_ray(a.rc, n, rs);
@@ -1969,7 +1942,7 @@
         }
     }
 
-    clock_probe(1);
+    if constexpr (!PT) clock_probe(1);
     if constexpr (AUX) {
         if (a.w_out) for (uint32_t jj = j_stop; jj < T; ++jj) a.w_out[(size_t)jj * Npad + r] = 0.0f;
     }
@@ -1990,7 +1963,7 @@
         }
     }
     static_assert(VH <= IN && NCOL <= IN && IN * 64 <= 2 * 64 * SLAB_DW, "view MLP activations reuse the feature column / slab");
-    if constexpr (MFMA) {
+    if constexpr (MFMA && !PT) {
         __syncthreads();
         stage_weights<NCOL, VH>(lds_vw, a.vw[0]);
         stage_weights<VH, VH>(lds_vw + VW0, a.vw[1]);
@@ -2036,6 +2009,126 @@
             q[3] = dep;
         }
     }
+}
+
+template <typename TT, int L, int C, int H1, int H2, int NOUT, int VH, int MODE, int K, bool AUX = false, bool LT = false, bool L0L = false, bool EO = false, int NP = 3, bool PORD = false,
+          bool CANON = false>
+__global__ __launch_bounds__(256, MODE == MLP_VALU ? 1 : SN_FINAL_WAVES) void k_final_stage(FinalArgs a) {
+    SN_POISON_ALL();
+    static_assert(NP == 3 || (LT && !L0L && !AUX), "reduced-product MLP forms: plain linear-tail instantiations only");
+    static_assert(!LT || (MODE == MLP_F16X3 && K >= 4 && K <= 8), "linear tail: split-fp16 MLP on the FinalLv path");
+    static_assert(!L0L || (LT && sizeof(TT) == 2), "LDS-resident level 0: fp16 tables, linear-tail instantiation (80 KiB: 32 packed weights + 4 x 8 swizzled slabs + 16 level 0)");
+    constexpr int SLAB_DW = L0L ? 16 : SLAB_STRIDE;
+    constexpr bool MFMA = MODE != MLP_VALU;
+    constexpr int IN = L * C;
+    constexpr int GEO = NOUT - 1;
+    constexpr int NSH = 16;
+    constexpr int NCOL = GEO + NSH;
+    static_assert(!MFMA || (IN == 32 && H1 == 64 && H2 == 64 && NOUT == 16), "MFMA path is the 32-64-64-16 MLP");
+    extern __shared__ __attribute__((aligned(16))) float lds[];
+    float *fe;
+    uint32_t fstride;
+    float *actB = nullptr;
+    constexpr int VW0 = VH * PadIn<NCOL>::value, VW1 = VH * PadIn<VH>::value;
+    float *lds_vw;
+    uint32_t *slab_hi = nullptr, *slab_lo = nullptr;
+    if constexpr (MODE == MLP_F16X3) {
+        static_assert(PACK16_U4 * 4 == PACK_FLOATS, "both packings fill the same 32 KiB");
+        for (uint32_t i = threadIdx.x; i < (uint32_t)PACK16_U4; i += 256u)
+            reinterpret_cast<uint4 *>(lds)[i] = reinterpret_cast<const uint4 *>(a.mlp_pack)[i];
+        if constexpr (LT) { __syncthreads(); stage_w3p(lds + W3P_OFFSET, a.w[2]); }
+        constexpr int WAVE_SLAB = 2 * 64 * SLAB_DW;
+        float *wave_base = lds + PACK_FLOATS + (threadIdx.x >> 6) * WAVE_SLAB;
+        slab_hi = reinterpret_cast<uint32_t *>(wave_base);
+        slab_lo = slab_hi + 64 * SLAB_DW;
+        if constexpr (L0L) {
+            uint32_t *l0w = reinterpret_cast<uint32_t *>(lds + PACK_FLOATS + 4 * WAVE_SLAB);
+            const uint32_t rows0 = a.g.res[0] * a.g.res[0] * a.g.res[0];
+            const uint32_t *src = reinterpret_cast<const uint32_t *>(a.table) + a.g.off[0];
+            for (uint32_t i = threadIdx.x; i < rows0; i += 256u) l0w[i] = src[i];
+        }
+        fe = wave_base + (threadIdx.x & 63u);
+        fstride = 64u;
+        lds_vw = lds;
+    } else if constexpr (MODE == MLP_F32) {
+        for (uint32_t i = threadIdx.x; i < (uint32_t)PACK_FLOATS / 4u; i += 256u)
+            reinterpret_cast<float4 *>(lds)[i] = reinterpret_cast<const float4 *>(a.mlp_pack)[i];
+        fe = lds + PACK_FLOATS + (threadIdx.x >> 6) * (IN * 64) + (threadIdx.x & 63u);
+        fstride = 64u;
+        lds_vw = lds;
+    } else {
+        fe = lds + threadIdx.x;
+        actB = lds + 64 * 256 + threadIdx.x;
+        fstride = 256u;
+        lds_vw = lds + 2 * 64 * 256;
+    }
+    if constexpr (!MFMA) {
+        stage_weights<NCOL, VH>(lds_vw, a.vw[0]);
+        stage_weights<VH, VH>(lds_vw + VW0, a.vw[1]);
+        stage_weights<VH, 3>(lds_vw + VW0 + VW1, a.vw[2]);
+    }
+    __syncthreads();
+    clock_probe(0);
+    const uint32_t *l0tab = reinterpret_cast<const uint32_t *>(lds + PACK_FLOATS + 4 * 2 * 64 * SLAB_DW);
+
+    FinalLds fl;
+    fl.lds = lds; fl.fe = fe; fl.fstride = fstride; fl.actB = actB; fl.lds_vw = lds_vw; fl.slab_hi = slab_hi; fl.slab_lo = slab_lo; fl.l0tab = l0tab;
+    final_stage_rays<TT, L, C, H1, H2, NOUT, VH, MODE, K, AUX, LT, L0L, EO, NP, PORD, CANON, false>(a, fl, tile_id(a.rc) * 4u + __builtin_amdgcn_readfirstlane(threadIdx.x >> 6));
+}
+
+struct TileQueueArgs {
+    uint32_t *ctr;
+    uint32_t units;
+};
+__global__ void k_tile_queue_reset(uint32_t *ctr) {
+    if (blockIdx.x == 0 && threadIdx.x < 8u) ctr[threadIdx.x] = 0u;
+}
+template <typename TT, int K>
+__global__ __launch_bounds__(512, 2) void k_final_stage_pt(FinalArgs a, TileQueueArgs q) {
+    SN_POISON_ALL();
+    constexpr int VIEW_FLOATS = 32 * PadIn<31>::value + 32 * PadIn<32>::value + 3 * PadIn<32>::value;
+    constexpr int WAVE_SLAB = 2 * 64 * SLAB_STRIDE;
+    extern __shared__ __attribute__((aligned(16))) float lds[];
+    float *const lds_vw = lds + PACK_FLOATS + 8 * WAVE_SLAB;
+    static_assert(W3P_OFFSET % 4 == 0 && W3P_FLOATS % 4 == 0, "w3p is a whole number of 16-byte pieces of the weight image");
+    for (uint32_t i = threadIdx.x; i < (uint32_t)PACK16_U4; i += 512u)
+        if (i < (uint32_t)(W3P_OFFSET / 4) || i >= (uint32_t)((W3P_OFFSET + W3P_FLOATS) / 4)) reinterpret_cast<uint4 *>(lds)[i] = reinterpret_cast<const uint4 *>(a.mlp_pack)[i];
+    stage_w3p(lds + W3P_OFFSET, a.w[2]);
+    stage_weights<31, 32>(lds_vw, a.vw[0]);
+    stage_weights<32, 32>(lds_vw + 32 * PadIn<31>::value, a.vw[1]);
+    stage_weights<32, 3>(lds_vw + 32 * PadIn<31>::value + 32 * PadIn<32>::value, a.vw[2]);
+    static_assert(VIEW_FLOATS == 32 * 32 + 32 * 32 + 3 * 32, "the view weights' region (LDS_F16X3_PT)");
+    __syncthreads();
+    clock_probe(0);
+    const uint32_t wave = __builtin_amdgcn_readfirstlane(threadIdx.x >> 6), lane = threadIdx.x & 63u;
+    float *wave_base = lds + PACK_FLOATS + wave * WAVE_SLAB;
+    FinalLds fl;
+    fl.lds = lds; fl.fe = wave_base + lane; fl.fstride = 64u; fl.actB = nullptr; fl.lds_vw = lds_vw;
+    fl.slab_hi = reinterpret_cast<uint32_t *>(wave_base); fl.slab_lo = fl.slab_hi + 64 * SLAB_STRIDE; fl.l0tab = nullptr;
+    uint32_t ntiles;
+    if (a.rc.W) {
+        const uint32_t tlw = a.rc.tlw, tlh = 6u - tlw;
+        ntiles = ((a.rc.W + (1u << tlw) - 1u) >> tlw) * ((a.rc.rows + (1u << tlh) - 1u) >> tlh);
+    } else ntiles = (a.rc.N + 63u) >> 6;
+    const uint32_t home = blockIdx.x & 7u;
+    for (uint32_t k = 0; k < 8u;) {
+        const uint32_t x = (home + k) & 7u;
+        uint32_t begin, end;
+        tile_queue_range(x, q.units, a.rc.xcd_swizzle, begin, end);
+        if (begin >= end) { ++k; continue; }
+        uint32_t t = 0;
+        if (lane == 0u) t = atomicAdd(&q.ctr[x], 1u);
+        t = __builtin_amdgcn_readfirstlane(t);
+        if (t >= end - begin) { ++k; continue; }
+        const uint32_t g = begin + t;
+        if (g < ntiles) {
+            typedef __attribute__((address_space(4))) const FinalArgs cst_final_args;
+            cst_final_args *ap = (cst_final_args *)__builtin_amdgcn_kernarg_segment_ptr();
+            asm volatile("" : "+s"(ap));
+            final_stage_rays<TT, 16, 2, 64, 64, 16, 32, MLP_F16X3, K, false, true, false, false, 3, false, false, true>(*(const FinalArgs *)ap, fl, g);
+        }
+    }
+    clock_probe(1);
 }
 
 struct AnyShape {
@@ -3166,6 +3259,7 @@
 constexpr int VIEW_W = 32 * 32 + 32 * 32 + 3 * 32;
 static_assert(VIEW_W <= PACK_FLOATS, "view weights overlay the packed MLP weights");
 constexpr size_t LDS_F16X3 = (size_t)(PACK_FLOATS + 4 * 2 * 64 * SLAB_STRIDE) * sizeof(float);
+constexpr size_t LDS_F16X3_PT = (size_t)(PACK_FLOATS + 8 * 2 * 64 * SLAB_STRIDE + VIEW_W) * sizeof(float);
 constexpr size_t LDS_F16X3_L0 = (size_t)(PACK_FLOATS + 4 * 2 * 64 * 16 + L0_MAX_ROWS) * sizeof(float);
 constexpr size_t LDS_MFMA32 = (size_t)(PACK_FLOATS + 4 * 32 * 64) * sizeof(float);
 constexpr size_t LDS_VALU = (size_t)(2 * 64 * 256 + VIEW_W) * sizeof(float);
@@ -3179,6 +3273,7 @@
 #endif
 }
 
+constexpr uint32_t SN_TILE_QUEUES = 8;
 struct FinalRoute {
     enum Family { NONE, ANY, SP, CMP, RS, LT, LT_L0, PER_SAMPLE, MFMA32, VALU };
     Family family = NONE;
@@ -3194,6 +3289,8 @@
     int dense = 0;
     uint32_t gathers = 0;
     uint32_t lpr_log2 = 0, spl_log2 = 0;
+    bool pt = false;
+    uint32_t pt_grid = 0;
 };
 struct PropRoute {
     int K = -1;
@@ -3214,7 +3311,9 @@
     size_t pair_main = 0, pair_prop[SN_MAX_STAGES] = {};
     size_t pair_floats = 0, slot_floats = 0;
     size_t head_floats() const { return (size_t)PACK_FLOATS + pair_floats; }
-    size_t bytes() const { return ((size_t)bands.slots * slot_floats + head_floats()) * sizeof(float); }
+    size_t ctr_words() const { return (size_t)bands.slots * SN_TILE_QUEUES; }
+    size_t ctr_offset_floats() const { return (size_t)bands.slots * slot_floats + head_floats(); }
+    size_t bytes() const { return (ctr_offset_floats() + ctr_words()) * sizeof(float); }
 };
 struct RenderRoute {
     GridLevels gl_prop[SN_MAX_STAGES], gl_main, gl_feat;
@@ -3229,6 +3328,7 @@
     FinalRoute fin;
     FeatRoute feat;
     uint32_t chunks = 0;
+    uint32_t cus = 0;
     ChunkRoute full, last;
 };
 
@@ -3327,6 +3427,14 @@
     FinalRoute &f = c.fin;
     f.grid = c.nblk;
     const uint32_t T = cfg->num_steps[S - 1];
+    if (f.family == FinalRoute::LT && !f.aux && !f.eo && f.np == 3 && !f.clumped && !f.canon && cfg->tuning.persistent_tiles != 1) {
+        const uint32_t cus = r.cus ? r.cus : 256u;
+        const uint32_t wgs = cfg->tuning.persistent_wgs > 0 ? (uint32_t)cfg->tuning.persistent_wgs : cus;
+        const uint64_t slots = (uint64_t)SN_TILE_QUEUES * r.cus * (r.ws.bands.slots == 2u ? 4u : 1u);
+        if (cfg->tuning.persistent_tiles == 2 || (r.cus != 0u && (uint64_t)c.nblk * 4u > slots)) {
+            f.pt = true; f.pt_grid = wgs; f.lds = LDS_F16X3_PT;
+        }
+    }
 #ifdef SN_EXPERIMENTS
     if (f.family == FinalRoute::RS) {
         f.grid = W ? ((W + 31u) >> 5) * ((n / W + 15u) >> 4) : div_up(n, (uint32_t)(RS_PROD * 64));
@@ -3357,7 +3465,10 @@
     r->last = n_last == r->full.n ? r->full : plan_chunk(cfg, io, *r, n_last);
 }
 
-static int plan_render(const sn_render_cfg *cfg, const sn_render_io *io, RenderRoute *r) {
+static int plan_render(const sn_render_cfg *cfg, const sn_render_io *io, uint32_t cus, RenderRoute *r) {
+    r->cus = cus;
+    SN_REQUIRE(cfg->tuning.persistent_tiles >= 0 && cfg->tuning.persistent_tiles <= 2, "render_rays: tuning.persistent_tiles %d outside 0..2", cfg->tuning.persistent_tiles);
+    SN_REQUIRE(cfg->tuning.persistent_wgs >= 0 && cfg->tuning.persistent_wgs <= 65535, "render_rays: tuning.persistent_wgs %d outside 0..65535", cfg->tuning.persistent_wgs);
     SN_REQUIRE(io->out_stride == 0u || io->out_stride >= 5u, "render_rays: out_stride %u must be 0 (dense outputs) or at least 5 floats (rgb | depth | weights_sum per row)", io->out_stride);
     SN_REQUIRE(io->head_stride == 0u || (io->f_image && io->head_stride >= 31u + 4u && !io->skip_final),
                "render_rays: head_stride %u needs f_image and room for f_image | rgb | depth (>= 35 floats per row)", io->head_stride);
@@ -3472,6 +3583,7 @@
     snprintf(info->final_kernel, sizeof(info->final_kernel), "%s", f.name);
     info->workgroups = f.grid; info->lds_bytes = (uint32_t)f.lds; info->dense_levels = (uint32_t)(f.dense < 0 ? 0 : f.dense);
     info->gathers_per_wave_sample = f.gathers; info->launches += 1u;
+    info->persistent_tiles = f.pt ? 1u : 0u; info->grid_workgroups = f.pt ? f.pt_grid : f.grid;
 }
 
 template <typename... P, typename... A>
@@ -3547,8 +3659,18 @@
     }
 }
 
-static int launch_final(const FinalRoute &f, hipStream_t st, const FinalArgs &fa, const AnyShape &any) {
+static int launch_final(const FinalRoute &f, hipStream_t st, const FinalArgs &fa, const AnyShape &any, uint32_t *queue_ctr) {
     const dim3 grid(f.grid), block(f.block);
+    if (f.pt) {
+        SN_REQUIRE(queue_ctr != nullptr, "render_rays: the persistent last stage has no counters");
+        static_assert(SN_TILE_QUEUES == 8, "k_tile_queue_reset clears eight counters");
+        const int rcz = launch(k_tile_queue_reset, dim3(1), dim3(64), 0, st, queue_ctr);
+        if (rcz) return rcz;
+        const TileQueueArgs q{queue_ctr, f.grid};
+        const dim3 pgrid(f.pt_grid), pblock(512);
+        if (f.K == 7) return f.f16 ? launch(k_final_stage_pt<__half, 7>, pgrid, pblock, f.lds, st, fa, q) : launch(k_final_stage_pt<float, 7>, pgrid, pblock, f.lds, st, fa, q);
+        return f.f16 ? launch(k_final_stage_pt<__half, 5>, pgrid, pblock, f.lds, st, fa, q) : launch(k_final_stage_pt<float, 5>, pgrid, pblock, f.lds, st, fa, q);
+    }
     switch (f.family) {
         case FinalRoute::ANY:
             return f.f16 ? launch(k_final_stage_any<__half>, grid, block, f.lds, st, fa, any) : launch(k_final_stage_any<float>, grid, block, f.lds, st, fa, any);
@@ -3581,6 +3703,19 @@
         default: return ft.f16 ? feat_kernel_of<__half, 2>(ft.lg, patch) : feat_kernel_of<float, 2>(ft.lg, patch);
     }
 }
+static uint32_t device_compute_units() {
+    static std::mutex mu;
+    static std::map<int, uint32_t> known;
+    int dev = 0;
+    if (hipGetDevice(&dev) != hipSuccess) { (void)hipGetLastError(); return 0u; }
+    std::lock_guard<std::mutex> lock(mu);
+    auto it = known.find(dev);
+    if (it != known.end()) return it->second;
+    int n = 0;
+    if (hipDeviceGetAttribute(&n, hipDeviceAttributeMultiprocessorCount, dev) != hipSuccess || n < 0) { (void)hipGetLastError(); n = 0; }
+    known[dev] = (uint32_t)n;
+    return (uint32_t)n;
+}
 }
 
 extern "C" {
@@ -3590,18 +3725,31 @@
     return plan_workspace(cfg, N, tile_w).bytes();
 }
 
-int sn_rm_render_route_info(const sn_render_cfg *cfg, const sn_render_io *io, sn_launch_info *out) {
+int sn_rm_render_route_info_cus(const sn_render_cfg *cfg, const sn_render_io *io, uint32_t compute_units, sn_launch_info *out) {
     SN_REQUIRE(cfg && io && out, "render_route_info: cfg/io/out is NULL");
     *out = sn_launch_info{};
     if (io->N == 0) return SN_OK;
     int rc = check_io_pointers(cfg, io);
     if (rc) return rc;
     RenderRoute route;
-    rc = plan_render(cfg, io, &route);
+    rc = plan_render(cfg, io, compute_units, &route);
     if (rc) return rc;
     if (io->skip_final) return SN_OK;
     note_final(route.last.fin, out);
     out->launches = route.chunks;
+    return SN_OK;
+}
+int sn_rm_render_route_info(const sn_render_cfg *cfg, const sn_render_io *io, sn_launch_info *out) { return sn_rm_render_route_info_cus(cfg, io, 0u, out); }
+
+int sn_rm_tile_queue_info(uint32_t units, int32_t order, int32_t wave_tile, uint32_t queue, sn_tile_queue_info *out) {
+    SN_REQUIRE(out, "tile_queue_info: out is NULL");
+    SN_REQUIRE(queue < SN_TILE_QUEUES, "tile_queue_info: queue %u outside 0..7", queue);
+    SN_REQUIRE(units <= 0x3fffffffu, "tile_queue_info: %u workgroup tiles are more than a launch holds", units);
+    SN_REQUIRE(wave_tile >= 0 && wave_tile <= 5, "tile_queue_info: wave_tile %d outside 0..5", wave_tile);
+    const TileOrder to = tile_order_of(order, wave_tile ? (uint32_t)wave_tile : 3u);
+    *out = sn_tile_queue_info{};
+    tile_queue_range(queue, units, to.xcd, out->begin, out->end);
+    out->queues = SN_TILE_QUEUES; out->wave_tiles = 4u * units;
     return SN_OK;
 }
 
@@ -3638,7 +3786,7 @@
     int rc = check_io_pointers(cfg, io);
     if (rc) return rc;
     RenderRoute route;
-    rc = plan_render(cfg, io, &route);
+    rc = plan_render(cfg, io, device_compute_units(), &route);
     if (rc) return rc;
     SN_REQUIRE(io->workspace != nullptr, "render_rays: workspace is NULL");
     SN_REQUIRE(table_aligned(io->workspace), "render_rays: workspace must be 16-byte aligned");
@@ -3782,7 +3930,7 @@
         {
             ProfScope ps_final(st, PK_FINAL);
             note_final(fr, &g_launch);
-            rc = launch_final(fr, st, fa, route.any);
+            rc = launch_final(fr, st, fa, route.any, reinterpret_cast<uint32_t *>(pack + route.ws.ctr_offset_floats()) + (size_t)slot * SN_TILE_QUEUES);
             if (rc) return rc;
             SN_LAUNCH_CHECK(fr.family == FinalRoute::ANY ? "k_final_stage_any" : "k_final_stage");
         }
diff --git a/sanerf-hq_amd/raymarching/__init__.py b/sanerf-hq_amd/raymarching/__init__.py
--- a/sanerf-hq_amd/raymarching/__init__.py
+++ b/sanerf-hq_amd/raymarching/__init__.py
@@ -21,4 +21,4 @@
 from .mesh import mesh_smooth, mesh_vertex_normals, mesh_smooth_build, mesh_smooth_steps, mesh_smooth_emit, smooth_quantisation
 from .mesh import mesh_rasterize, mesh_rasterize_clip, mesh_raster_project, mesh_raster_draw, mesh_raster_resolve, RASTER_SMALL_MAX_PIXELS, RASTER_MAX_SIDE
 from .mesh import vertex_probe_points, vertex_probe_composite, PROBE_SAMPLES
-from .render import RenderPlan, Tuning, tuning, last_launch_info, route_info, tile_order_info, render_rays, FP16_SPLIT_LIMIT
+from .render import RenderPlan, Tuning, tuning, last_launch_info, route_info, tile_order_info, tile_queue_info, render_rays, FP16_SPLIT_LIMIT
diff --git a/sanerf-hq_amd/raymarching/render.py b/sanerf-hq_amd/raymarching/render.py
--- a/sanerf-hq_amd/raymarching/render.py
+++ b/sanerf-hq_amd/raymarching/render.py
@@ -12,7 +12,8 @@
 
 
 class Tuning:
-    FIELDS = ("mlp_mode", "per_sample_form", "densify", "linear_tile_order", "prop_sp_max_rays", "final_sp_max_rays", "feat_levels", "band_streams", "exact_early_out", "wave_tile", "prop_sp_lanes", "feat_patch", "prop_pair", "experiment")
+    FIELDS = ("mlp_mode", "per_sample_form", "densify", "linear_tile_order", "prop_sp_max_rays", "final_sp_max_rays", "feat_levels", "band_streams", "exact_early_out", "wave_tile", "prop_sp_lanes", "feat_patch", "prop_pair", "experiment",
+              "persistent_tiles", "persistent_wgs")
 
     def __init__(self, **kw):
         for f in self.FIELDS:
@@ -37,8 +38,19 @@
 def last_launch_info() -> dict:
     info = _lib.LaunchInfo()
     _lib.check(_lib.lib().sn_rm_last_launch_info(C.byref(info)), "last_launch_info")
+    return _launch_info_dict(info)
+
+
+def _launch_info_dict(info) -> dict:
     return dict(final_kernel=info.final_kernel.decode(), workgroups=int(info.workgroups), lds_bytes=int(info.lds_bytes),
-                dense_levels=int(info.dense_levels), gathers_per_wave_sample=int(info.gathers_per_wave_sample), launches=int(info.launches))
+                dense_levels=int(info.dense_levels), gathers_per_wave_sample=int(info.gathers_per_wave_sample), launches=int(info.launches),
+                persistent_tiles=int(info.persistent_tiles), grid_workgroups=int(info.grid_workgroups))
+
+
+def tile_queue_info(units: int, queue: int, order: int = 0, wave_tile: int = 0) -> dict:
+    info = _lib.TileQueueInfo()
+    _lib.check(_lib.lib().sn_rm_tile_queue_info(int(units), int(order), int(wave_tile), int(queue), C.byref(info)), "tile_queue_info")
+    return dict(queues=int(info.queues), wave_tiles=int(info.wave_tiles), begin=int(info.begin), end=int(info.end))
 
 
 def tile_order_info(W: int, rows: int, workgroup: int, wave_tile: int = 0, order: int = 0) -> dict:
@@ -256,16 +268,18 @@
 
 def route_info(plan: RenderPlan, N: int, tile_w: int = 0, want: Sequence[str] = (), u_tables: Optional[Dict[int, torch.Tensor]] = None,
                bins0_table: Optional[torch.Tensor] = None, skip_final: bool = False, tuning: Optional["Tuning"] = None,
-               packed: Optional[torch.Tensor] = None, head_input: bool = False) -> dict:
+               packed: Optional[torch.Tensor] = None, head_input: bool = False, compute_units: Optional[int] = None) -> dict:
     io = _lib.RenderIO()
     stand_in = 64
     io.rays_o = io.rays_d = stand_in
     _fill_io(plan, io, int(N), tile_w, want, u_tables, bins0_table, skip_final, packed, head_input, tuning,
              lambda name, shape, dtype=torch.float32: stand_in, lambda t: (t, stand_in))
     info = _lib.LaunchInfo()
-    _lib.check(_lib.lib().sn_rm_render_route_info(C.byref(plan.cfg), C.byref(io), C.byref(info)), "route_info")
-    return dict(final_kernel=info.final_kernel.decode(), workgroups=int(info.workgroups), lds_bytes=int(info.lds_bytes),
-                dense_levels=int(info.dense_levels), gathers_per_wave_sample=int(info.gathers_per_wave_sample), launches=int(info.launches))
+    if compute_units is None:
+        t0 = plan.keep[0] if plan.keep else None
+        compute_units = torch.cuda.get_device_properties(t0.device).multi_processor_count if t0 is not None and t0.is_cuda else 0
+    _lib.check(_lib.lib().sn_rm_render_route_info_cus(C.byref(plan.cfg), C.byref(io), int(compute_units), C.byref(info)), "route_info")
+    return _launch_info_dict(info)
 
 
 def render_rays(plan: RenderPlan, rays_o, rays_d, cam_near_far=None, bg_color: float = 1.0, tile_w: int = 0,
```

After: 110.3 million (median of 6 runs). 1.03x the previous value.
